# jxhe/vae-lagging-encoder

Measured on AMD Instinct MI355X. Metric: aggressive-loop seqs/sec, higher is better.
Workload: dtype bf16

## Files before the change

include/lvae.h:

```cpp
#ifndef LVAE_H
#define LVAE_H

#include <stdint.h>

#ifdef __cplusplus
extern "C" {
#endif

int lv_gemm_f32(int transA, int transB, int M, int N, int K, float alpha,
                const float* A, long lda, const float* B, long ldb, float* C, long ldc, int accumulate,
                const float* add1, long ld1, int mod1, const float* add2, long ld2, int mod2,
                float* ws , long ws_floats, void* stream);

int lv_gemm_bf16(int transA, int transB, int M, int N, int K, float alpha,
                 const float* A, long lda, const float* B, long ldb, float* C, long ldc, int accumulate,
                 const float* add1, long ld1, int mod1, const float* add2, long ld2, int mod2,
                 float* ws, long ws_floats, void* stream);

int lv_gemm_b16(int transA, int M, int N, int K, float alpha,
                const uint16_t* A, long lda, const uint16_t* B, long ldb, float* C, long ldc, int accumulate,
                const float* add1, long ld1, int mod1, const float* add2, long ld2, int mod2,
                float* ws, long ws_floats, void* stream);
int lv_gemm_b16_dual_supported(int M, int N, int K, long ws_floats);
int lv_gemm_b16_dual(int transA, int M, int N, int K, const uint16_t* A, long lda, const uint16_t* B, long ldb,
                     float* C1, long ldc1, int nsplit, float* C2, long ldc2, float* ws, long ws_floats, void* stream);
int lv_gemm_b16_pair_supported(int transA0, int M0, int N0, int K0, int transA1, int M1, int N1, int K1, long ws_floats);
int lv_gemm_b16_pair_pending(int* pending, void* stream);
int lv_gemm_b16_pair(int transA0, int M0, int N0, int K0, const uint16_t* A0, long lda0, const uint16_t* B0, long ldb0,
                     float* C0, long ldc0, int nsplit0, float* C0b, long ldc0b,
                     int transA1, int M1, int N1, int K1, const uint16_t* A1, long lda1, const uint16_t* B1, long ldb1,
                     float* C1, long ldc1, float* ws, long ws_floats, void* stream);
int lv_gemm_b16_keep(int M, int N, int K, const uint16_t* A, long lda, const uint16_t* B, long ldb, float* C,
                     const uint8_t* keep, float kscale, int Bsz, float* ws, long ws_floats, void* stream);
int lv_gemm_b16_sumsq_parts(int M, int N, int K, long ws_floats);
int lv_gemm_b16_sumsq(int transA, int M, int N, int K, const uint16_t* A, long lda, const uint16_t* B, long ldb, float* C, long ldc,
                      float* ws, long ws_floats, float* sq, int sq_only, void* stream);
int lv_gemm_b16_nll_parts(int N);
int lv_gemm_b16_tile(int tile, int transA, int M, int N, int K, float alpha,
                     const uint16_t* A, long lda, const uint16_t* B, long ldb, float* C, long ldc, int accumulate,
                     const float* add1, long ld1, int mod1, const float* add2, long ld2, int mod2,
                     float* ws, long ws_floats, void* stream);
int lv_gemm_b16_nll_tile(int tile, int M, int N, int K, const uint16_t* A, long lda, const uint16_t* B, long ldb, uint16_t* logits16,
                         long ldl16, const int64_t* ids, long ids_stride, int tgt_off, int Bsz, float* part, float* tgt_logit,
                         void* stream);
int lv_gemm_b16_nll(int M, int N, int K, const uint16_t* A, long lda, const uint16_t* B, long ldb, uint16_t* logits16, long ldl16,
                    const int64_t* ids, long ids_stride, int tgt_off, int Bsz, float* part, float* tgt_logit, void* stream);
int lv_softmax_nll_merge_f32(const float* part, int nparts, const float* tgt_logit, float* lse, float* nll, int R, void* stream);
int lv_softmax_nll_bwd_h16(const uint16_t* logits16, long ldl, const float* lse, const int64_t* ids, long ids_stride, int tgt_off,
                           const float* rowscale, uint16_t* dlogits, long ldo, int T, int B, int V, void* stream);
int lv_cvt_bf16_f32(const float* src, long lds, int R, int C, uint16_t* dst, long ldd, uint16_t* dstT, long ldt,
                    void* stream);
int lv_cvt_bf16_keep_f32(const float* src, long lds, int T, int Bsz, int C, const uint8_t* keep, float kscale,
                         uint16_t* dst, long ldd, uint16_t* dstT, long ldt, void* stream);
int lv_cvt_f32_bf16_scaled(const uint16_t* src, long n, float scale, float* dst, void* stream);
int lv_keep_scale_f32(float* x, const uint8_t* keep, float kscale, int T, int Bsz, int C, void* stream);

int lv_cvt_bf16_gates_f32(const float* src, long lds, int H, int C, uint16_t* dst, long ldd, uint16_t* dstT, long ldt,
                          void* stream);
int lv_cvt_bf16_lo_f32(const float* src, long lds, int R, int C, int gate_H, const int64_t* ids, long ids_stride, int Bsz, int V,
                       uint16_t* dst, long ldd, uint16_t* dstT, long ldt, void* stream);
int lv_cvt_h16_f32(const float* src, long lds, int R, int C, int gate_H, const int64_t* ids, long ids_stride, int Bsz, int V,
                   uint16_t* dst, long ldd, uint16_t* dstT, long ldt, void* stream);
int lv_gemm_h16(int M, int N, int K, float alpha, const uint16_t* A, long lda, const uint16_t* B, long ldb,
                float* C, long ldc, int accumulate, const float* add1, long ld1, int mod1,
                const float* add2, long ld2, int mod2, float* ws, long ws_floats, void* stream);
int lv_transpose_f32(const float* in, float* out, int rows, int cols, void* stream);
int lv_transpose_ld_f32(const float* in, long in_ld, float* out, long out_ld, int rows, int cols, void* stream);

int lv_lstm_fwd_f32(const float* gx, const float* whh, float* hs, float* cs, float* gates,
                    const uint8_t* dmask, float dscale, float* hdrop, float* ws, int T, int B, int H, void* stream);
int lv_lstm_fwd_bf16(const float* gx, const float* whh, float* hs, float* cs, float* gates,
                     const uint8_t* dmask, float dscale, float* hdrop, float* ws, int T, int B, int H, void* stream);
int lv_lstm_fwd_bf16_ug(const float* gx, const float* whh, float* hs, float* cs, float* gates,
                        const uint8_t* dmask, float dscale, float* hdrop, float* ws, int T, int B, int H, void* stream);
int lv_lstm_fwd_f32_ug(const float* gx, const float* whh, float* hs, float* cs, float* gates,
                       const uint8_t* dmask, float dscale, float* hdrop, float* ws, int T, int B, int H, void* stream);
long lv_lstm_persist16_wpk_floats(void);
long lv_lstm_persist16_xch_floats(void);
int lv_lstm_persist16_xch_clear(float* xch, void* stream);
long lv_lstm_persist16_saved_floats(int T, int R);
int lv_lstm_persist16_pack(const float* whh, float* wpk, int backward, int H, void* stream);
int lv_lstm_persist16_pack2(const float* whh, float* wpk_fwd, float* wpk_bwd, int H, void* stream);
int lv_lstm_persist16_pack2_h16(const float* whh, float* wpk_fwd, float* wpk_bwd, int H, void* stream);
int lv_lstm_fwd_bf16_persist16(const float* gx, const float* wpk, float* hs, float* cs, float* saved, float* xch, int* status,
                               int T, int B, int R, int flags, int H, void* stream);
int lv_lstm_bwd_bf16_persist16(const float* dh_ext, const float* dh_last, const float* wpk, const float* saved, const float* hs,
                               const float* cs, uint16_t* dG16, float* dGsum, float* xch, int* status, float* dh0, float* dc0,
                               int tanh_init, int T, int B, int R, int flags, int H, void* stream);
int lv_lstm_persist16_import_saved(const float* gates, const float* cs, float* saved, int T, int B, int R, int H, void* stream);
int lv_gate_interleave_f32(const float* a, const float* b, int R, int H, float* out, void* stream);
int lv_lstm_bwd_bf16(const float* dh_ext, const float* dh_last, const uint8_t* dmask, float dscale,
                     const float* whh, const float* gates, const float* hs, const float* cs,
                     float* dG, float* dGsum, float* ws, float* dh0, float* dc0, int tanh_init,
                     int T, int B, int H, void* stream);
int lv_lstm_bwd_bf16_img(const float* dh_ext, const float* dh_last, const uint8_t* dmask, float dscale,
                           const float* whh, const float* gates, const float* hs, const float* cs,
                           float* dG, uint16_t* dG16, float* dGsum, float* ws, float* dh0, float* dc0, int tanh_init,
                           int T, int B, int H, void* stream);
long lv_lstm_ws_floats(int B, int H);
int lv_lstm_bwd_ksplit(int H);
int lv_lstm_bwd_f32(const float* dh_ext, const float* dh_last, const uint8_t* dmask, float dscale,
                    const float* whh, const float* gates, const float* hs, const float* cs,
// ... 208 lines not shown
```

vae_lagging_encoder_amd/_lib.py:

```python
import ctypes
import os
import threading

from . import build as _build

_vp = ctypes.c_void_p
_i = ctypes.c_int
_l = ctypes.c_long
_f = ctypes.c_float
_d = ctypes.c_double
_u64 = ctypes.c_uint64

SIGNATURES = {
    "lv_gemm_f32": [_i, _i, _i, _i, _i, _f, _vp, _l, _vp, _l, _vp, _l, _i, _vp, _l, _i, _vp, _l, _i, _vp, _l, _vp],
    "lv_gemm_bf16": [_i, _i, _i, _i, _i, _f, _vp, _l, _vp, _l, _vp, _l, _i, _vp, _l, _i, _vp, _l, _i, _vp, _l, _vp],
    "lv_gemm_b16": [_i, _i, _i, _i, _f, _vp, _l, _vp, _l, _vp, _l, _i, _vp, _l, _i, _vp, _l, _i, _vp, _l, _vp],
    "lv_gemm_h16": [_i, _i, _i, _f, _vp, _l, _vp, _l, _vp, _l, _i, _vp, _l, _i, _vp, _l, _i, _vp, _l, _vp],
    "lv_gemm_b16_dual_supported": [_i, _i, _i, _l],
    "lv_gemm_b16_dual": [_i, _i, _i, _i, _vp, _l, _vp, _l, _vp, _l, _i, _vp, _l, _vp, _l, _vp],
    "lv_gemm_b16_pair_supported": [_i, _i, _i, _i, _i, _i, _i, _i, _l],
    "lv_gemm_b16_pair_pending": [_vp, _vp],
    "lv_gemm_b16_pair": [_i, _i, _i, _i, _vp, _l, _vp, _l, _vp, _l, _i, _vp, _l,
                         _i, _i, _i, _i, _vp, _l, _vp, _l, _vp, _l, _vp, _l, _vp],
    "lv_gemm_b16_keep": [_i, _i, _i, _vp, _l, _vp, _l, _vp, _vp, _f, _i, _vp, _l, _vp],
    "lv_gemm_b16_sumsq_parts": [_i, _i, _i, _l],
    "lv_gemm_b16_sumsq": [_i, _i, _i, _i, _vp, _l, _vp, _l, _vp, _l, _vp, _l, _vp, _i, _vp],
    "lv_gemm_b16_nll_parts": [_i],
    "lv_gemm_b16_tile": [_i, _i, _i, _i, _i, _f, _vp, _l, _vp, _l, _vp, _l, _i, _vp, _l, _i, _vp, _l, _i, _vp, _l, _vp],
    "lv_gemm_b16_nll_tile": [_i, _i, _i, _i, _vp, _l, _vp, _l, _vp, _l, _vp, _l, _i, _i, _vp, _vp, _vp],
    "lv_gemm_b16_nll": [_i, _i, _i, _vp, _l, _vp, _l, _vp, _l, _vp, _l, _i, _i, _vp, _vp, _vp],
    "lv_softmax_nll_merge_f32": [_vp, _i, _vp, _vp, _vp, _i, _vp],
    "lv_softmax_nll_bwd_h16": [_vp, _l, _vp, _vp, _l, _i, _vp, _vp, _l, _i, _i, _i, _vp],
    "lv_cvt_bf16_f32": [_vp, _l, _i, _i, _vp, _l, _vp, _l, _vp],
    "lv_cvt_bf16_keep_f32": [_vp, _l, _i, _i, _i, _vp, _f, _vp, _l, _vp, _l, _vp],
    "lv_cvt_f32_bf16_scaled": [_vp, _l, _f, _vp, _vp],
    "lv_keep_scale_f32": [_vp, _vp, _f, _i, _i, _i, _vp],
    "lv_cvt_bf16_gates_f32": [_vp, _l, _i, _i, _vp, _l, _vp, _l, _vp],
    "lv_cvt_bf16_lo_f32": [_vp, _l, _i, _i, _i, _vp, _l, _i, _i, _vp, _l, _vp, _l, _vp],
    "lv_cvt_h16_f32": [_vp, _l, _i, _i, _i, _vp, _l, _i, _i, _vp, _l, _vp, _l, _vp],
    "lv_gate_interleave_f32": [_vp, _vp, _i, _i, _vp, _vp],
    "lv_lstm_fwd_bf16_ug": [_vp, _vp, _vp, _vp, _vp, _vp, _f, _vp, _vp, _i, _i, _i, _vp],
    "lv_lstm_fwd_f32_ug": [_vp, _vp, _vp, _vp, _vp, _vp, _f, _vp, _vp, _i, _i, _i, _vp],
    "lv_loss_assemble_f32": [_vp, _vp, _vp, _vp, _vp, _vp, _vp, _vp, _vp, _i, _i, _vp],
    "lv_loss_assemble_rng_f32": [_vp, _vp, _vp, _vp, _vp, _vp, _vp, _vp, _vp, _i, _i, _vp, _u64, _vp],
    "lv_gx_expand_add_f32": [_vp, _vp, _vp, _i, _i, _i, _i, _vp],
    "lv_sample_sum_f32": [_vp, _vp, _i, _i, _i, _i, _vp],
    "lv_sample_sum_b16": [_vp, _l, _vp, _l, _i, _i, _i, _i, _vp],
    "lv_repeat_rows_i64": [_vp, _vp, _i, _i, _i, _vp],
    "lv_loss_assemble_ns_f32": [_vp, _vp, _vp, _vp, _vp, _vp, _vp, _vp, _vp, _i, _i, _i, _vp],
    "lv_loss_assemble_ns_rng_f32": [_vp, _vp, _vp, _vp, _vp, _vp, _vp, _vp, _vp, _i, _i, _i, _vp, _u64, _vp],
    "lv_enc_head_fwd_f32": [_vp, _vp, _vp, _vp, _vp, _vp, _i, _i, _i, _i, _vp],
    "lv_enc_head_bwd_f32": [_vp, _vp, _vp, _i, _vp, _vp, _vp, _vp, _vp, _vp, _i, _i, _i, _i, _vp],
    "lv_dec_tail_parts": [_i],
    "lv_dec_init_f32": [_vp, _vp, _vp, _l, _i, _vp, _vp, _vp, _vp, _vp, _i, _i, _i, _i, _vp],
    "lv_dec_tail_bwd_f32": [_vp, _vp, _vp, _vp, _l, _i, _vp, _vp, _l, _vp, _vp, _vp, _vp, _i, _i, _i, _vp],
    "lv_clip_norm2_f32": [_vp, _l, _vp, _l, _vp, _f, _vp, _vp, _vp, _vp],
    "lv_clip_norm2_txn_f32": [_vp, _l, _vp, _l, _vp, _f, _vp, _vp, _vp, _vp, _vp, _vp, _vp, _vp, _vp],
    "lv_clip_norm2_fold_txn_f32": [_vp, _l, _vp, _l, _vp, _vp, _i, _f, _vp, _vp, _vp, _vp, _vp, _vp, _vp, _vp, _vp],
    "lv_clip_coef_txn_f32": [_vp, _f, _vp, _vp, _vp, _vp, _vp, _vp, _vp, _vp],
    "lv_txn_guard_f32": [_vp, _vp, _vp, _vp],
    "lv_sgd_step_txn_f32": [_vp, _vp, _l, _vp, _vp, _i, _vp, _vp],
    "lv_scale_txn_f32": [_vp, _l, _vp, _vp, _vp],
    "lv_sgd_step_scale_txn_f32": [_vp, _vp, _l, _vp, _vp, _i, _vp, _l, _vp, _vp],
    "lv_rng_noise_step": [_vp, _l, _vp, _l, _f, _vp, _l, _f, _vp, _u64, _vp],
    "lv_lstm_persist16_wpk_floats": [],
    "lv_lstm_persist16_xch_floats": [],
    "lv_lstm_persist16_xch_clear": [_vp, _vp],
    "lv_lstm_persist16_saved_floats": [_i, _i],
    "lv_lstm_persist16_pack": [_vp, _vp, _i, _i, _vp],
    "lv_lstm_persist16_import_saved": [_vp, _vp, _vp, _i, _i, _i, _i, _vp],
    "lv_lstm_persist16_pack2": [_vp, _vp, _vp, _i, _vp],
    "lv_lstm_persist16_pack2_h16": [_vp, _vp, _vp, _i, _vp],
    "lv_lstm_fwd_bf16_persist16": [_vp, _vp, _vp, _vp, _vp, _vp, _vp, _i, _i, _i, _i, _i, _vp],
    "lv_lstm_bwd_bf16_persist16": [_vp, _vp, _vp, _vp, _vp, _vp, _vp, _vp, _vp, _vp, _vp, _vp, _i, _i, _i, _i, _i, _i, _vp],
    "lv_transpose_f32": [_vp, _vp, _i, _i, _vp],
    "lv_transpose_ld_f32": [_vp, _l, _vp, _l, _i, _i, _vp],
    "lv_lstm_bwd_ksplit": [_i],
    "lv_lstm_ws_floats": [_i, _i],
    "lv_lstm_fwd_f32": [_vp, _vp, _vp, _vp, _vp, _vp, _f, _vp, _vp, _i, _i, _i, _vp],
    "lv_lstm_bwd_f32": [_vp, _vp, _vp, _f, _vp, _vp, _vp, _vp, _vp, _vp, _vp, _vp, _vp, _i, _i, _i, _i, _vp],
    "lv_lstm_fwd_bf16": [_vp, _vp, _vp, _vp, _vp, _vp, _f, _vp, _vp, _i, _i, _i, _vp],
    "lv_lstm_bwd_bf16": [_vp, _vp, _vp, _f, _vp, _vp, _vp, _vp, _vp, _vp, _vp, _vp, _vp, _i, _i, _i, _i, _vp],
    "lv_lstm_bwd_bf16_img": [_vp, _vp, _vp, _f, _vp, _vp, _vp, _vp, _vp, _vp, _vp, _vp, _vp, _vp, _i, _i, _i, _i, _vp],
    "lv_embed_gather_f32": [_vp, _vp, _l, _vp, _f, _vp, _i, _i, _i, _i, _vp],
# ... 65 lines not shown
    "lv_mul_inplace_f32": [_vp, _vp, _l, _vp],
    "lv_bn_workspace_floats": [_i],
    "lv_pixelcnn_net_words": [],
    "lv_pixelcnn_block_words": [],
    "lv_pixelcnn_pixel_step_f32": [_vp, _i, _i, _i, _vp],
    "lv_conv32_tap_split": [_i],
    "lv_bn_eval_f32": [_vp, _vp, _vp, _vp, _vp, _f, _vp, _i, _vp, _vp, _vp, _l, _i, _vp],
    "lv_bn_fwd_f32": [_vp, _vp, _vp, _vp, _i, _vp, _vp, _vp, _vp, _vp, _f, _f, _vp, _l, _i, _vp],
    "lv_bn_bwd_f32": [_vp, _vp, _vp, _vp, _vp, _vp, _i, _vp, _vp, _vp, _vp, _i, _vp, _l, _i, _vp],
    "lv_bn_bwd2_f32": [_vp, _vp, _vp, _vp, _vp, _vp, _vp, _i, _vp, _vp, _vp, _vp, _i, _vp, _l, _i, _vp],
    "lv_bn_bwd4_f32": [_vp, _vp, _vp, _vp, _vp, _vp, _vp, _vp, _vp, _i, _vp, _vp, _vp, _vp, _i, _vp, _l, _i, _vp],
    "lv_sigmoid_bce_fwd_f32": [_vp, _vp, _vp, _i, _i, _f, _vp],
    "lv_sigmoid_bce_bwd_f32": [_vp, _vp, _vp, _vp, _i, _i, _f, _vp],
    "lv_dec_input_fwd_f32": [_vp, _vp, _vp, _i, _i, _i, _vp],
    "lv_dec_input_bwd_f32": [_vp, _vp, _i, _i, _i, _vp],
    "lv_dec_cond_ll_f32_supported": [_i, _i, _i, _i, _i],
    "lv_dec_cond_ll_f32_ws_floats": [_i, _i, _i, _i, _i],
    "lv_dec_cond_ll_f32": [_vp, _i, _i, _vp, _l, _i, _vp, _vp, _vp, _vp, _vp, _vp, _vp, _i, _i, _i, _i, _vp, _vp, _vp],
    "lv_grid_posterior_f32": [_vp, _vp, _l, _i, _i, _i, _vp, _vp, _vp],
    "lv_beam_supported": [_i, _i, _i],
    "lv_beam_ws_floats": [_i, _i, _i],
    "lv_beam_init_f32": [_vp, _vp, _vp, _vp, _vp, _vp, _vp, _vp, _vp, _vp, _i, _i, _i, _i, _i, _vp],
    "lv_beam_select_f32": [_vp, _l, _vp, _vp, _vp, _vp, _vp, _vp, _i, _i, _i, _vp],
    "lv_beam_advance_f32": [_vp, _vp, _vp, _vp, _vp, _vp, _vp, _vp, _vp, _vp, _vp, _vp, _vp, _i, _i, _i, _i, _i, _i, _i, _vp],
    "lv_beam_backtrace": [_vp, _vp, _vp, _vp, _vp, _vp, _vp, _vp, _i, _i, _i, _i, _vp],
}


_LONG_FNS = ("lv_lstm_ws_floats", "lv_conv1x1_wgrad_ws_floats", "lv_conv1x1_blocks", "lv_lstm_persist16_wpk_floats", "lv_lstm_persist16_xch_floats", "lv_lstm_persist16_saved_floats", "lv_conv32_wpack_floats",
             "lv_conv32_wgrad_ws_floats", "lv_dec_cond_ll_f32_ws_floats", "lv_beam_ws_floats")


class LvaeError(RuntimeError):
    pass


class Lib(object):

    def __init__(self, cdll, path):
        self.cdll = cdll
        self.path = path
        missing = []
        for name, argtypes in SIGNATURES.items():
            try:
                fn = getattr(cdll, name)
            except AttributeError:
                missing.append(name)
                continue
            fn.argtypes = argtypes
            fn.restype = ctypes.c_long if name in _LONG_FNS else ctypes.c_int
            setattr(self, "_raw_" + name, fn)
        if missing:
            raise LvaeError("%s does not export: %s" % (path, ", ".join(missing)))
        self._value_fns = {"lv_gemm_b16_dual_supported", "lv_gemm_b16_pair_supported", "lv_lstm_bwd_ksplit", "lv_dec_tail_parts", "lv_gemm_b16_nll_parts", "lv_gemm_b16_sumsq_parts", "lv_embed_scatter_sumsq_parts", "lv_conv32_wpack_floats",
                           "lv_conv32_wgrad_slabs", "lv_conv32_wgrad_ws_floats", "lv_conv32_wgrad_parts", "lv_conv1x1_wgrad_parts", "lv_conv32_blocks", "lv_conv1x1_blocks", "lv_conv1x1_wgrad_ws_floats", "lv_sumsq_workspace_floats", "lv_lstm_ws_floats", "lv_bn_workspace_floats",
                           "lv_lstm_persist16_wpk_floats", "lv_lstm_persist16_xch_floats", "lv_lstm_persist16_saved_floats",
                           "lv_pixelcnn_net_words", "lv_pixelcnn_block_words", "lv_conv32_tap_split", "lv_dec_cond_ll_f32_supported",
                           "lv_dec_cond_ll_f32_ws_floats", "lv_beam_supported", "lv_beam_ws_floats"}

    def __getattr__(self, name):
        if name.startswith("lv_"):
            raw = object.__getattribute__(self, "_raw_" + name)
            if name in object.__getattribute__(self, "_value_fns"):
                return raw

            def call(*args):
                rc = raw(*args)
                if rc != 0:
                    raise LvaeError("%s failed with status %d (%s)" % (
                        name, rc, "hipError_t" if rc > 0 else "argument check"))
            call.__name__ = name
            self.__dict__[name] = call
            return call
        raise AttributeError(name)


def bind(cdll, path="<cdll>"):
    return Lib(cdll, path)


_lock = threading.Lock()
_lib = None


def load():
    global _lib
    with _lock:
        if _lib is not None:
            return _lib
        path = _build.LIB_PATH
        if not os.path.exists(path):
            try:
                _build.build_hip()
            except Exception as e:
                raise LvaeError(
                    "HIP extension %s is missing and could not be built (%s). The MI355X path has no CPU "
                    "fallback: run `python -m vae_lagging_encoder_amd.build` where hipcc is available." % (path, e))
        try:
            cdll = ctypes.CDLL(path)
        except OSError as e:
            raise LvaeError("cannot load %s: %s" % (path, e))
        _lib = Lib(cdll, path)
        return _lib
```

vae_lagging_encoder_amd/csrc/lv_device.h:

```cpp
#pragma once

#ifdef LV_EMU
#include "hip_emu.h"
#define LV_LAUNCH(kern, grid, block, shmem, stream, ...) \
    lv_emu::launch((grid), (block), (shmem), [=]() { kern(__VA_ARGS__); })
#define LV_DYN_SHARED(name) char* name = lv_emu::dyn_smem()
static inline f32x4 lv_mfma_16x16x4(float a, float b, f32x4 c) { return lv_emu_mfma_16x16x4(a, b, c); }
static inline f32x16 lv_mfma_32x32x2(float a, float b, f32x16 c) { return lv_emu_mfma_32x32x2(a, b, c); }
#define LV_SCHED_BARRIER() do { } while (0)
static inline int lv_wave_uniform(int v) { return v; }
#define LV_LAUNCH_RESIDENT(kern, grid, block, shmem, stream, ...) \
    lv_emu::launch_concurrent((grid), (block), (shmem), [=]() { kern(__VA_ARGS__); })
#define LV_BLOCK_SHARED(T, name) T& name = *reinterpret_cast<T*>(lv_emu::block_shared(sizeof(T)))
static inline unsigned long long lv_agent_load_u64(const unsigned long long* p) {
    lv_emu::yield_all();
    return __atomic_load_n(p, __ATOMIC_RELAXED);
}
static inline void lv_agent_store_u64(unsigned long long* p, unsigned long long v) { __atomic_store_n(p, v, __ATOMIC_RELAXED); }
static inline void lv_xcd_store_u64(unsigned long long* p, unsigned long long v) { __atomic_store_n(p, v, __ATOMIC_RELAXED); }
static inline void lv_poll_backoff() { }
#define LV_WAIT_LDS() lv_emu::wave_sync()
template <class T> static inline void lv_store_nt(T v, T* p) { *p = v; }
static inline int lv_device_cus() { return 1 << 20; }
#define LV_SPIN_LIMIT (1 << 15)
static inline f32x16 lv_mfma_32x32x16_bf16(uint4 a, uint4 b, f32x16 c) { return lv_emu_mfma_32x32x16_bf16(a, b, c); }
static inline f32x4 lv_mfma_16x16x32_bf16(uint4 a, uint4 b, f32x4 c) { return lv_emu_mfma_16x16x32_bf16(a, b, c); }
static inline f32x4 lv_mfma_16x16x32_bf16_areg(uint4 a, uint4 b, f32x4 c) { return lv_emu_mfma_16x16x32_bf16(a, b, c); }
static inline f32x4 lv_mfma_16x16x32_bf16_areg_first(uint4 a, uint4 b) { return lv_emu_mfma_16x16x32_bf16(a, b, f32x4{0.f, 0.f, 0.f, 0.f}); }
#define LV_MFMA_DRAIN() do { } while (0)
static inline void LV_MFMA_RESULT(f32x4&) { }
static inline f32x4 lv_mfma_4x4x4_16b_bf16(uint2 a, uint2 b, f32x4 c) { return lv_emu_mfma_4x4x4_16b_bf16(a, b, c); }
static inline void lv_glds16(const void* g, void* lds_wave_base) { memcpy((char*)lds_wave_base + 16 * lv_emu::lane(), g, 16); }
static inline void lv_glds16_uncounted(const void* g, void* lds_wave_base) { lv_glds16(g, lds_wave_base); }
#define LV_WAIT_VMEM() do { } while (0)
#define LV_WAIT_VMEM_N(n) do { } while (0)
static inline void lv_store_wt_f4(float4* p, float4 v) { *p = v; }
static inline void lv_acquire_agent() { __atomic_thread_fence(__ATOMIC_ACQUIRE); }
static inline unsigned lv_agent_load_u32(const unsigned* p) { return __atomic_load_n(p, __ATOMIC_RELAXED); }
static inline void lv_sleep_short() { }
#define LV_ARRIVAL_POLLS 2
static inline unsigned atomicExch(unsigned* p, unsigned v) { return __atomic_exchange_n(p, v, __ATOMIC_RELAXED); }
#define LV_S_BARRIER() __syncthreads()
#define LV_SETPRIO(n) do { } while (0)
static inline uint2 lv_ds_read_tr16_b64(const void* lds_ptr) {
    auto& w = lv_emu::my_wave();
    const int l = lv_emu::lane();
    uint64_t blk;
    memcpy(&blk, lds_ptr, 8);
    w.u[l] = blk;
    lv_emu::wave_sync();
    uint16_t o[4];
    for (int j = 0; j < 4; ++j) {
        const uint64_t b = w.u[(l & ~15) + 4 * j + ((l & 15) >> 2)];
        o[j] = (uint16_t)(b >> (16 * (l & 3)));
    }
    lv_emu::wave_sync();
    uint2 r;
    memcpy(&r, o, 8);
    return r;
}
template <int SHIFT, int BANK> static inline float lv_row_shr_into(float old, float src) {
    auto& w = lv_emu::my_wave();
    const int l = lv_emu::lane();
    uint32_t b;
    memcpy(&b, &src, 4);
    w.u[l] = b;
    lv_emu::wave_sync();
    float out = old;
    if (((l & 15) >> 2) == BANK && (l & 15) >= SHIFT) { const uint32_t v = (uint32_t)w.u[l - SHIFT]; memcpy(&out, &v, 4); }
    lv_emu::wave_sync();
    return out;
}
static inline float lv_sat_f16(float x) { return x != x ? x : fminf(fmaxf(x, -65504.f), 65504.f); }
static inline uint16_t lv_f32_to_f16_bits(float x) {
    uint32_t u;
    memcpy(&u, &x, 4);
    const uint32_t sign = (u >> 16) & 0x8000u;
    u &= 0x7FFFFFFFu;
    if (u >= 0x7F800000u) return (uint16_t)(sign | (u > 0x7F800000u ? 0x7E00u : 0x7C00u));
    if (u >= 0x477FF000u) return (uint16_t)(sign | 0x7C00u);
    if (u < 0x33000001u) return (uint16_t)sign;
    if (u < 0x38800000u) {
        const int shift = 126 - (int)(u >> 23);
        const uint32_t mant = (u & 0x7FFFFFu) | 0x800000u;
        uint32_t h = mant >> shift;
        const uint32_t rem = mant & ((1u << shift) - 1u), half = 1u << (shift - 1);
        if (rem > half || (rem == half && (h & 1u))) ++h;
        return (uint16_t)(sign | h);
    }
    uint32_t h = ((u - 0x38000000u) >> 13);
    const uint32_t rem = u & 0x1FFFu;
    if (rem > 0x1000u || (rem == 0x1000u && (h & 1u))) ++h;
    return (uint16_t)(sign | h);
}
// ... 439 lines not shown
```

vae_lagging_encoder_amd/csrc/lv_gemm_b16.hip:

```cpp
#ifndef LV_B16_T256_DMA
#define LV_B16_T256_DMA 1
#endif
#if defined(LV_TRACE)
#define lv_trace_buf lv_trace_buf_gemm
#endif
#include "lv_device.h"
#if defined(LV_TRACE) && !defined(LV_EMU)
__device__ unsigned long long* lv_trace_buf = nullptr;
extern "C" int lv_trace_set_gemm(void* p) { return (int)hipMemcpyToSymbol(HIP_SYMBOL(lv_trace_buf), &p, sizeof(p)); }
#endif
#include <type_traits>

namespace {

#ifndef LV_B16_ABL
#define LV_B16_ABL 0
#endif
#ifndef LV_B16_SPLIT_TARGET
#define LV_B16_SPLIT_TARGET 512
#endif

constexpr int BK = 64;
constexpr int BT = 128;
constexpr int NCH = BK / 8;

#ifndef LV_NLL_ABL
#define LV_NLL_ABL 0
#endif
struct GemmQ {
    const uint16_t* A; const uint16_t* B; float* C;
    int M, N, K;
    long lda, ldb, ldc;
    float alpha;
    int accumulate;
    const float* add1; long ld1; int mod1;
    const float* add2; long ld2; int mod2;
    int tilesM, tilesN;
    int splits, kt_per_split;
    float* ws;
    uint16_t* C16; long ldc16;
    const int64_t* ids; long ids_stride; int tgt_off; int Bsz;
    float2* part; int nparts;
    float* tgt;
    const uint8_t* keep; float kscale; int keepT;
    float* sq; int sq_only;
    float* C2; long ldc2; int nsplit;
};

__device__ __forceinline__ uint4 load_chunk(const uint16_t* __restrict__ p, int valid) {
    if (valid >= 8) return *reinterpret_cast<const uint4*>(p);
    uint32_t h[8];
#pragma unroll
    for (int e = 0; e < 8; ++e) h[e] = e < valid ? (uint32_t)p[e] : 0u;
    uint4 q;
    q.x = h[0] | (h[1] << 16); q.y = h[2] | (h[3] << 16); q.z = h[4] | (h[5] << 16); q.w = h[6] | (h[7] << 16);
    return q;
}


struct KcPtr { const uint16_t* p[4]; };

__device__ __forceinline__ KcPtr kc_setup(const uint16_t* __restrict__ P, long ld, int rows, int r0, int t) {
    KcPtr q;
#pragma unroll
    for (int i = 0; i < 4; ++i) {
        const int f = t + 256 * i;
        int row = r0 + (f >> 3);
        if (row > rows - 1) row = rows - 1;
        q.p[i] = P + (long)row * ld + 8 * (f & 7);
    }
    return q;
}

template <bool FULL>
__device__ __forceinline__ void kc_load(const KcPtr& q, int k0, int K, int t, uint4 (&reg)[4]) {
#pragma unroll
    for (int i = 0; i < 4; ++i) {
        if (FULL) {
            reg[i] = *reinterpret_cast<const uint4*>(q.p[i] + k0);
        } else {
            const int k = k0 + 8 * ((t + 256 * i) & 7);
            reg[i] = k < K ? load_chunk(q.p[i] + k0, K - k) : make_uint4(0u, 0u, 0u, 0u);
        }
    }
}

__device__ __forceinline__ void store_kc(uint4 (*S)[BT], int t, const uint4 (&reg)[4]) {
#pragma unroll
    for (int i = 0; i < 4; ++i) {
        const int f = t + 256 * i;
        const int m = f >> 3, c = f & 7;
        S[c][m ^ (2 * c)] = reg[i];
    }
}

struct McPtr { const uint16_t* p; long ld; };

__device__ __forceinline__ McPtr mc_setup(const uint16_t* __restrict__ P, long ld, int r0, int t) {
    long col = r0 + 8 * (t & 15);
// ... 525 lines not shown
    for (int i = 0; i < 2; ++i)
#pragma unroll
        for (int j = 0; j < 2; ++j)
            store_frag_f32(p, acc[i][j], m0 + wm * 64 + i * 32 + 4 * (l >> 5), n0 + wn * 64 + j * 32 + (l & 31));
}

constexpr int BT2 = 256;
typedef uint4 LdsTile2[BT2][NCH];

struct Tail256 {
    int full;
    int tail;
    int tail_s;
    int kt_per_piece;
};

#ifndef LV_T256_G
#define LV_T256_G 4
#endif
__device__ __forceinline__ void t256_tile_of(const GemmQ& p, int s, int& tm, int& tn) {
    const int G = LV_T256_G;
    const int nig = G * p.tilesN;
    const int group = s / nig;
    const int first_m = group * G;
    const int gsz = (p.tilesM - first_m) < G ? (p.tilesM - first_m) : G;
    tm = first_m + (s % nig) % gsz;
    tn = (s % nig) / gsz;
}

struct T256Pick { int tile, kt0, kt1, piece, tm, tn; };
__device__ __forceinline__ T256Pick t256_pick(const GemmQ& p, const Tail256& q, int bid) {
    T256Pick k;
    const int nk_all = (p.K + BK - 1) / BK;
    k.piece = -1;
    if (bid < q.full) {
        const int xcd = bid % 8, per = q.full / 8;
        k.tile = xcd * per + bid / 8;
        k.kt0 = 0; k.kt1 = nk_all;
    } else {
        const int r = bid - q.full, nw = q.tail * q.tail_s;
        const int xcd = r % 8, qq = nw / 8, rem = nw % 8;
        const int idx = (xcd < rem ? xcd * (qq + 1) : rem * (qq + 1) + (xcd - rem) * qq) + r / 8;
        k.tile = q.full + idx % q.tail;
        k.piece = idx / q.tail;
        k.kt0 = k.piece * q.kt_per_piece;
        k.kt1 = k.kt0 + q.kt_per_piece;
        if (k.kt1 > nk_all) k.kt1 = nk_all;
        if (q.tail_s == 1) k.piece = -1;
    }
    t256_tile_of(p, k.tile, k.tm, k.tn);
    return k;
}

template <bool NLL>
__device__ __forceinline__ void t256_epilogue(const GemmQ& p, const Tail256& q, f32x16 (&acc)[4][2], LdsTile2& As0, LdsTile2& Bs0,
                                              LdsTile2& As1, LdsTile2& Bs1, int tile, int piece, int tn, int m0, int n0, int t, int l,
                                              int wm, int wn, int lh) {
    constexpr int NJ = 2;
    if constexpr (NLL) {
#if LV_NLL_ABL & 4
        return;
#endif
        auto rowptr = [&](int rr) -> char* {
            const int b = rr >> 6;
            char* base = b == 0 ? reinterpret_cast<char*>(&As0[0][0]) : b == 1 ? reinterpret_cast<char*>(&Bs0[0][0])
                       : b == 2 ? reinterpret_cast<char*>(&As1[0][0]) : reinterpret_cast<char*>(&Bs1[0][0]);
            return base + (rr & 63) * 512;
        };
        const int odd = l & 1;
#pragma unroll
        for (int i2 = 0; i2 < 4; ++i2) {
            char* const bufp = rowptr(wm * 128 + i2 * 32);
#pragma unroll
            for (int j = 0; j < 2; ++j) {
                const int clp = (wn * 64 + j * 32 + (l & 31)) & ~1;
                const int lane_off = (4 * lh + odd) * 512 + ((((clp >> 3) ^ (4 * lh) ^ odd) << 4) | ((clp & 7) << 1));
#pragma unroll
                for (int e = 0; e < 16; e += 2) {
                    const float mine0 = acc[i2][j][e], mine1 = acc[i2][j][e + 1];
                    const float got = lv_lane_xor1(odd ? mine0 : mine1);
                    const uint32_t pk = odd ? lv_pack_f16x2(got, mine1) : lv_pack_f16x2(mine0, got);
                    const int key = (e & 3) | (8 * ((e >> 2) & 1));
                    const int roff = ((e & 3) + 8 * (e >> 2)) * 512;
                    *reinterpret_cast<uint32_t*>(bufp + roff + (lane_off ^ (key << 4))) = pk;
                }
            }
        }
        __syncthreads();
#if !(LV_NLL_ABL & 1)
        {
            const int c = l & 31;
#pragma unroll 4
            for (int s16 = 0; s16 < 16; ++s16) {
                const int r2 = 16 * s16 + 2 * (t >> 6) + (l >> 5);
                const uint4 qv = *reinterpret_cast<const uint4*>(rowptr(r2) + ((c ^ (r2 & 15)) << 4));
                const int col0 = n0 + 8 * c;
                if (m0 + r2 < p.M && col0 + 8 <= p.ldc16) *reinterpret_cast<uint4*>(p.C16 + (long)(m0 + r2) * p.ldc16 + col0) = qv;
            }
        }
#endif
        const int rr = t & 255, half = t >> 8;
        const int row = m0 + rr;
        if (row < p.M) {
            const char* rowp = rowptr(rr);
            const int tt = row / p.Bsz, bb = row % p.Bsz;
            long tg = p.ids[(long)bb * p.ids_stride + tt + p.tgt_off];
            if (tg < 0) tg = 0;
            if (tg >= p.N) tg = p.N - 1;
#pragma unroll 1
            for (int pc = 0; pc < 2; ++pc) {
                const int cb = 128 * half + 64 * pc;
                const int c0 = n0 + cb;
                uint4 qv[8];
#pragma unroll
                for (int k = 0; k < 8; ++k) qv[k] = *reinterpret_cast<const uint4*>(rowp + ((((cb >> 3) + k) ^ (rr & 15)) << 4));
#if LV_NLL_ABL & 2
                if (qv[0].x == 0x12345678u) p.tgt[row] = 1.f;
                continue;
#endif
                float v[64];
#pragma unroll
                for (int k = 0; k < 8; ++k) {
                    const uint32_t wv[4] = {qv[k].x, qv[k].y, qv[k].z, qv[k].w};
#pragma unroll
                    for (int h2 = 0; h2 < 4; ++h2) {
                        v[8 * k + 2 * h2] = lv_f16_bits_to_f32((uint16_t)(wv[h2] & 0xFFFFu));
                        v[8 * k + 2 * h2 + 1] = lv_f16_bits_to_f32((uint16_t)(wv[h2] >> 16));
                    }
                }
                float mx, sm;
                nll_piece_stats(v, p.N - c0, mx, sm);
                p.part[(long)row * p.nparts + 4 * tn + 2 * half + pc] = make_float2(mx, sm);
                const int tl = (int)tg - c0;
                if (tl >= 0 && tl < 64) {
                    const int cl = cb + tl;
                    p.tgt[row] = lv_f16_bits_to_f32(*reinterpret_cast<const uint16_t*>(rowp + ((((cl >> 3) ^ (rr & 15)) << 4) | ((cl & 7) << 1))));
                }
            }
        }
        return;
    }
    if (piece >= 0) {
        if (p.sq && piece == 0 && l == 0) p.sq[tile * 8 + (t >> 6)] = 0.f;
        float* slab = p.ws + ((long)(tile - q.full) * q.tail_s + piece) * (BT2 * BT2);
#pragma unroll
        for (int i2 = 0; i2 < 4; ++i2)
#pragma unroll
            for (int j = 0; j < NJ; ++j) {
                const int col = wn * (32 * NJ) + j * 32 + (l & 31);
#pragma unroll
                for (int e = 0; e < 16; ++e) {
                    const int rr = wm * 128 + i2 * 32 + (e & 3) + 8 * (e >> 2) + 4 * (l >> 5);
                    slab[rr * BT2 + col] = acc[i2][j][e];
                }
            }
        return;
    }
    if (p.sq) {
        float ss = 0.f;
#pragma unroll
        for (int i2 = 0; i2 < 4; ++i2)
#pragma unroll
            for (int j = 0; j < NJ; ++j) {
                const int rbase = m0 + wm * 128 + i2 * 32 + 4 * (l >> 5), col = n0 + wn * (32 * NJ) + j * 32 + (l & 31);
#pragma unroll
                for (int e = 0; e < 16; ++e) {
                    const float v = p.alpha * acc[i2][j][e];
                    if (col < p.N && rbase + (e & 3) + 8 * (e >> 2) < p.M) ss += v * v;
                }
            }
        ss = lv_wave_sum(ss);
        if (l == 0) p.sq[tile * 8 + (t >> 6)] = ss;
        if (p.sq_only) return;
    }
#pragma unroll
    for (int i2 = 0; i2 < 4; ++i2)
#pragma unroll
        for (int j = 0; j < NJ; ++j)
            store_frag_f32(p, acc[i2][j], m0 + wm * 128 + i2 * 32 + 4 * (l >> 5), n0 + wn * (32 * NJ) + j * 32 + (l & 31));
}

template <bool NLL, bool TN, bool PP = false>
__global__ __launch_bounds__(512) void lv_gemm_b16_t256_kernel(GemmQ p, Tail256 q) {
    constexpr int WN = 4;
    constexpr int NJ = 2;
    constexpr int UN = 4;
    __shared__ __attribute__((aligned(1024))) LdsTile2 As0, Bs0;
    __shared__ __attribute__((aligned(1024))) LdsTile2 As1, Bs1;

    const int t = (int)threadIdx.x;
    const int l = t & 63, w = lv_wave_uniform(t >> 6);
    const int wm = w / WN, wn = w % WN;
    const int li = l & 31, lh = l >> 5;
    const int nfull = p.K / BK;

    const T256Pick pk = t256_pick(p, q, (int)blockIdx.x);
    const int kt0 = pk.kt0, kt1 = pk.kt1;
    const int m0 = pk.tm * BT2, n0 = pk.tn * BT2;

    f32x16 acc[4][NJ];
#pragma unroll
    for (int i = 0; i < 4; ++i)
#pragma unroll
        for (int j = 0; j < NJ; ++j)
#pragma unroll
            for (int e = 0; e < 16; ++e) acc[i][j][e] = 0.f;

    uint32_t oa[UN], ob[UN];
    int kch[UN];
#pragma unroll
    for (int i = 0; i < UN; ++i) {
        const int u = UN * w + i;
        const int row = 8 * u + (l >> 3);
#if LV_B16_PP_ABL & 128
        const int c = (l & 7);
#else
        const int c = (l & 7) ^ ((row >> 1) & 7);
#endif
        kch[i] = 8 * c;
#if LV_B16_PP_ABL & 64
        int ra = row, rb = row;
#else
        int ra = m0 + row, rb = n0 + row;
#endif
        if (ra > p.M - 1) ra = p.M - 1;
        if (rb > p.N - 1) rb = p.N - 1;
        oa[i] = (uint32_t)((long)ra * p.lda + kch[i]);
        ob[i] = (uint32_t)((long)rb * p.ldb + kch[i]);
        if constexpr (TN) {
            const int krow = 2 * u + (l >> 5);
            long mc = m0 / 8 + ((l & 31) ^ (4 * (krow & 3)));
            if (mc > p.lda / 8 - 1) mc = p.lda / 8 - 1;
            oa[i] = (uint32_t)((long)krow * p.lda + 8 * mc);
        }
    }
// ... 344 lines not shown
        mfma_close(true);
#pragma unroll
        for (int ks = 0; ks < 4; ++ks) { fa[ks][0] = a_frag(Ac, ks, 2); fa[ks][1] = a_frag(Ac, ks, 3); }
        LV_SCHED_BARRIER();
        stage_half(kn2, 2, Ac, Bc);
        seg_close(false);
        mma_quadrant(fa, fb1, 1, 1);
        mfma_close(false);
        stage_half(kn2, 3, Ac, Bc);
        seg_close(true);
        mma_quadrant(fa, fb0, 1, 0);
        mfma_close(true);
    };

    const int nmain = (kt1 < nfull ? kt1 : nfull) - kt0;
    if (kt1 > kt0 + nmain) {
        stage_ragged(kt1 - 1, As0, Bs0);
        __syncthreads();
#pragma unroll
        for (int ks = 0; ks < 4; ++ks) {
            uint4 ra[4], rb[2];
#pragma unroll
            for (int i2 = 0; i2 < 4; ++i2) ra[i2] = a_frag(As0, ks, i2);
#pragma unroll
            for (int j = 0; j < 2; ++j) rb[j] = b_frag(Bs0, ks, j);
#pragma unroll
            for (int i2 = 0; i2 < 4; ++i2)
#pragma unroll
                for (int j = 0; j < 2; ++j) acc[i2][j] = lv_mfma_32x32x16_bf16(ra[i2], rb[j], acc[i2][j]);
        }
        __syncthreads();
    }
    if (nmain > 0) {
        const int klast = kt0 + nmain - 1;
        auto tile_at = [&](int i) { return kt0 + i < klast ? kt0 + i : klast; };
        stage_half(tile_at(0), 0, As0, Bs0); stage_half(tile_at(0), 2, As0, Bs0); stage_half(tile_at(0), 3, As0, Bs0);
        stage_half(tile_at(0), 1, As0, Bs0);
        stage_half(tile_at(1), 0, As1, Bs1); stage_half(tile_at(1), 2, As1, Bs1); stage_half(tile_at(1), 3, As1, Bs1);
        LV_Q_WAIT();
        __syncthreads();
        if (wm == 1) LV_S_BARRIER();
        for (int i = 0; i < nmain; i += 2) {
            q_tile(As0, Bs0, As1, Bs1, tile_at(i + 1), tile_at(i + 2));
            if (i + 1 >= nmain) break;
            q_tile(As1, Bs1, As0, Bs0, tile_at(i + 2), tile_at(i + 3));
        }
        if (wm == 0) LV_S_BARRIER();
        LV_WAIT_VMEM();
        __syncthreads();
    }
#undef LV_Q_WAIT
}

template <bool NLL, bool TN>
__global__ __launch_bounds__(512) void lv_gemm_b16_t256q_kernel(GemmQ p, Tail256 q) {
    __shared__ __attribute__((aligned(1024))) LdsTile2 As0, Bs0;
    __shared__ __attribute__((aligned(1024))) LdsTile2 As1, Bs1;

    const T256Pick pk = t256_pick(p, q, (int)blockIdx.x);
    const int m0 = pk.tm * BT2, n0 = pk.tn * BT2;
    const int t = (int)threadIdx.x;
    const int l = t & 63, w = lv_wave_uniform(t >> 6);

    f32x16 acc[4][2];
    t256q_run<TN>(p, m0, n0, pk.kt0, pk.kt1, acc, As0, Bs0, As1, Bs1, l, w);
    t256_epilogue<NLL>(p, q, acc, As0, Bs0, As1, Bs1, pk.tile, pk.piece, pk.tn, m0, n0, t, l, w >> 2, w & 3, l >> 5);
}

#ifndef LV_SK_ABL
#define LV_SK_ABL 0
#endif
#ifndef LV_SK_SPIN
#define LV_SK_SPIN LV_ARRIVAL_POLLS
#endif
#ifndef LV_SK_SKEW
#define LV_SK_SKEW 3
#endif
#ifndef LV_SK_ROWS0
#define LV_SK_ROWS0 0
#endif
constexpr int SK_SLOTS = 32;
constexpr int SK_TILES = 1024;
__device__ unsigned lv_sk_arrivals[SK_SLOTS * SK_TILES];

struct SkProb {
    GemmQ q;
    int rows;
    int nk;
    long units;
    float* slabs;
    int cnt0;
    int skew, pieces, plen;
};
struct GemmG { SkProb pr[2]; };

__device__ __forceinline__ long sk_start(const SkProb& P, int nwg, int s) {
    const long b = (long)s * P.units / nwg;
    return (P.skew > 0 && s % P.pieces != 0) ? b - P.skew : b;
}
__device__ __forceinline__ int sk_owner(const SkProb& P, int nwg, long u) {
    if (P.skew > 0) {
        const int tile = (int)(u / P.nk), k = (int)(u - (long)tile * P.nk);
        int j = k / P.plen;
        if (j + 1 < P.pieces && k >= (j + 1) * P.plen - P.skew) ++j;
        return tile * P.pieces + j;
    }
    return (int)(((u + 1) * nwg - 1) / P.units);
// ... 115 lines not shown
                    sk_add_slab(acc, reinterpret_cast<const float4*>(P.slabs + (2L * c + (tile != (int)(cu0 / P.nk))) * (BT2 * BT2)) + t);
                }
            }
            done = summed;
        }
#if LV_SK_ABL & 2
        if (done && acc[0][0][0] == 1.2345e-30f) sk_store_tile(P.q, acc, m0, n0, l, w);
#else
        if (done) sk_store_tile(P.q, acc, m0, n0, l, w);
#endif
    }
}

__global__ __launch_bounds__(256) void sk_pending_kernel(int* out) {
    int n = 0;
    for (int i = (int)threadIdx.x; i < SK_SLOTS * SK_TILES; i += 256) n += lv_sk_arrivals[i] != 0u;
    n = lv_wave_sum(n);
    __shared__ int part[4];
    if ((threadIdx.x & 63) == 0) part[threadIdx.x >> 6] = n;
    __syncthreads();
    if (threadIdx.x == 0) *out = part[0] + part[1] + part[2] + part[3];
}

template <bool TN0, bool TN1>
__global__ __launch_bounds__(512) void lv_gemm_b16_t256g_kernel(GemmG g) {
    __shared__ __attribute__((aligned(1024))) LdsTile2 As0, Bs0;
    __shared__ __attribute__((aligned(1024))) LdsTile2 As1, Bs1;
    const int t = (int)threadIdx.x;
    const int l = t & 63, w = lv_wave_uniform(t >> 6);
    const int bid = (int)blockIdx.x, xcd = bid % 8, row = bid / 8;
    if (row < g.pr[0].rows) sk_work<TN0>(g.pr[0], xcd * g.pr[0].rows + row, As0, Bs0, As1, Bs1, t, l, w);
    else sk_work<TN1>(g.pr[1], xcd * g.pr[1].rows + (row - g.pr[0].rows), As0, Bs0, As1, Bs1, t, l, w);
}

#ifndef LV_TR_ROWS
#define LV_TR_ROWS 8
#endif
constexpr int TR_ROWS = LV_TR_ROWS, TR_WGS = BT2 / TR_ROWS;
__global__ __launch_bounds__(256) void tail_reduce_t256_kernel(GemmQ p, Tail256 q) {
    const int tile = q.full + (int)blockIdx.x / TR_WGS;
    int tm, tn;
    t256_tile_of(p, tile, tm, tn);
    const float* slab = p.ws + (long)(tile - q.full) * q.tail_s * (BT2 * BT2);
    const int t = (int)threadIdx.x;
    const int c4 = (t & 63) * 4;
    float ss = 0.f;
    const bool fast = !p.add1 && !p.add2 && !p.accumulate && p.ldc % 4 == 0 && p.N % 4 == 0 && (((uintptr_t)p.C) & 15) == 0 &&
                      (((uintptr_t)p.keep) & 3) == 0;
#pragma unroll
    for (int it = 0; it < TR_ROWS / 4; ++it) {
        const int rr = ((int)blockIdx.x % TR_WGS) * TR_ROWS + 4 * it + (t >> 6);
        const int row = tm * BT2 + rr;
        if (row >= p.M) continue;
        float4 sacc = make_float4(0.f, 0.f, 0.f, 0.f);
        for (int k0 = 0; k0 < q.tail_s; k0 += 4) {
            float4 pv[4];
#pragma unroll
            for (int u = 0; u < 4; ++u)
                pv[u] = *reinterpret_cast<const float4*>(slab + (long)(k0 + u < q.tail_s ? k0 + u : k0) * (BT2 * BT2) + rr * BT2 + c4);
#pragma unroll
            for (int u = 0; u < 4; ++u)
                if (k0 + u < q.tail_s) { sacc.x += pv[u].x; sacc.y += pv[u].y; sacc.z += pv[u].z; sacc.w += pv[u].w; }
        }
        const float sv[4] = {sacc.x, sacc.y, sacc.z, sacc.w};
        if (fast && tn * BT2 + c4 + 3 < p.N) {
            const int col = tn * BT2 + c4;
            float4 o = make_float4(p.alpha * sv[0], p.alpha * sv[1], p.alpha * sv[2], p.alpha * sv[3]);
            if (p.keep) {
                const uint32_t mk = *reinterpret_cast<const uint32_t*>(p.keep + ((long)(row % p.Bsz) * p.keepT + row / p.Bsz) * p.N + col);
                o.x = (mk & 0xFFu) ? o.x * p.kscale : 0.f;
                o.y = (mk & 0xFF00u) ? o.y * p.kscale : 0.f;
                o.z = (mk & 0xFF0000u) ? o.z * p.kscale : 0.f;
                o.w = (mk & 0xFF000000u) ? o.w * p.kscale : 0.f;
            }
            ss += (o.x * o.x + o.y * o.y) + (o.z * o.z + o.w * o.w);
            if (!p.sq_only) *reinterpret_cast<float4*>(p.C + (long)row * p.ldc + col) = o;
            continue;
        }
#pragma unroll
        for (int e = 0; e < 4; ++e) {
            const int col = tn * BT2 + c4 + e;
            if (col >= p.N) continue;
            float v = p.alpha * sv[e];
            if (p.add1) v += p.add1[(long)(row % p.mod1) * p.ld1 + col];
            if (p.add2) v += p.add2[(long)(row % p.mod2) * p.ld2 + col];
            float* c = p.C + (long)row * p.ldc + col;
            if (p.accumulate) v += *c;
            if (p.keep) v *= p.keep[((long)(row % p.Bsz) * p.keepT + row / p.Bsz) * p.N + col] ? p.kscale : 0.f;
            ss += v * v;
            if (!p.sq_only) *c = v;
        }
    }
    if (p.sq) {
        ss = lv_wave_sum(ss);
        if ((t & 63) == 0) p.sq[(long)p.tilesM * p.tilesN * 8 + (long)blockIdx.x * 4 + (t >> 6)] = ss;
    }
}

template <int NF>
__device__ __forceinline__ float sum_pieces(const float* first, long stride, int n) {
    float s = 0.f;
    for (int k0 = 0; k0 < n; k0 += NF) {
        float pv[NF];
#pragma unroll
        for (int u = 0; u < NF; ++u) pv[u] = first[(long)(k0 + u < n ? k0 + u : 0) * stride];
#pragma unroll
        for (int u = 0; u < NF; ++u)
            if (k0 + u < n) s += pv[u];
    }
    return s;
}

__global__ __launch_bounds__(256) void splitk_reduce_b16_v4_kernel(GemmQ p) {
    const long idx = ((long)blockIdx.x * 256 + threadIdx.x) * 4;
    const long MN = (long)p.M * p.N;
    if (idx >= MN) return;
    const int row = (int)(idx / p.N), col = (int)(idx % p.N);
    float4 s = make_float4(0.f, 0.f, 0.f, 0.f);
    for (int k0 = 0; k0 < p.splits; k0 += 4) {
        float4 pv[4];
#pragma unroll
        for (int u = 0; u < 4; ++u) pv[u] = *reinterpret_cast<const float4*>(p.ws + (long)(k0 + u < p.splits ? k0 + u : k0) * MN + idx);
#pragma unroll
        for (int u = 0; u < 4; ++u)
            if (k0 + u < p.splits) { s.x += pv[u].x; s.y += pv[u].y; s.z += pv[u].z; s.w += pv[u].w; }
    }
    float4 o = make_float4(p.alpha * s.x, p.alpha * s.y, p.alpha * s.z, p.alpha * s.w);
    if (p.keep) {
        const uint32_t mk = *reinterpret_cast<const uint32_t*>(p.keep + ((long)(row % p.Bsz) * p.keepT + row / p.Bsz) * p.N + col);
        o.x = (mk & 0xFFu) ? o.x * p.kscale : 0.f;
        o.y = (mk & 0xFF00u) ? o.y * p.kscale : 0.f;
        o.z = (mk & 0xFF0000u) ? o.z * p.kscale : 0.f;
        o.w = (mk & 0xFF000000u) ? o.w * p.kscale : 0.f;
    }
    if (p.nsplit > 0 && col >= p.nsplit) *reinterpret_cast<float4*>(p.C2 + (long)row * p.ldc2 + (col - p.nsplit)) = o;
    else *reinterpret_cast<float4*>(p.C + (long)row * p.ldc + col) = o;
}

__global__ __launch_bounds__(256) void splitk_reduce_b16_kernel(GemmQ p) {
    const long idx = (long)blockIdx.x * 256 + threadIdx.x;
    const long MN = (long)p.M * p.N;
    if (idx >= MN) return;
    const int row = (int)(idx / p.N), col = (int)(idx % p.N);
    float s = 0.f;
    if (p.splits <= 2) s = sum_pieces<2>(p.ws + idx, MN, p.splits);
    else if (p.splits <= 4) s = sum_pieces<4>(p.ws + idx, MN, p.splits);
    else s = sum_pieces<8>(p.ws + idx, MN, p.splits);
    float v = p.alpha * s;
    if (p.add1) v += p.add1[(long)(row % p.mod1) * p.ld1 + col];
    if (p.add2) v += p.add2[(long)(row % p.mod2) * p.ld2 + col];
    float* c = (p.nsplit > 0 && col >= p.nsplit) ? p.C2 + (long)row * p.ldc2 + (col - p.nsplit) : p.C + (long)row * p.ldc + col;
    if (p.accumulate) v += *c;
    if (p.keep) v *= p.keep[((long)(row % p.Bsz) * p.keepT + row / p.Bsz) * p.N + col] ? p.kscale : 0.f;
    *c = v;
}

__global__ __launch_bounds__(256) void cvt_b16_kernel(const float* __restrict__ src, long lds_, int R, int C,
                                                      uint16_t* __restrict__ dst, long ldd, uint16_t* __restrict__ dstT, long ldt,
                                                      int gate_H, const uint8_t* __restrict__ keep, float kscale, int Bsz,
                                                      const int64_t* __restrict__ gids, long gstride, int gV, int lo) {
    __shared__ uint16_t tile[64][66];
    const int t = (int)threadIdx.x;
    const int r0 = (int)blockIdx.y * 64, c0 = (int)blockIdx.x * 64;
    const int lane = t & 63, q = t >> 6;
    const bool tb = keep || gids;
    const int Tt = tb ? R / Bsz : 1;
    int bb = tb ? (r0 + q) % Bsz : 0, tt = tb ? (r0 + q) / Bsz : 0;
    const int gc = c0 + lane, gcc = gc < C ? gc : C - 1;
#pragma unroll
    for (int i0 = 0; i0 < 16; i0 += 8) {
        int grs[8], bbs[8], tts[8];
        long sr[8];
#pragma unroll
        for (int u = 0; u < 8; ++u) {
            grs[u] = r0 + q + 4 * (i0 + u);
            bbs[u] = bb; tts[u] = tt;
            if (tb) {
                bb += 4;
                while (bb >= Bsz) { bb -= Bsz; ++tt; }
            }
            sr[u] = grs[u] < R ? grs[u] : R - 1;
        }
        if (gids) {
#pragma unroll
            for (int u = 0; u < 8; ++u) sr[u] = gids[(long)bbs[u] * gstride + (grs[u] < R ? tts[u] : 0)];
#pragma unroll
            for (int u = 0; u < 8; ++u) sr[u] = sr[u] < 0 ? 0 : (sr[u] >= gV ? gV - 1 : sr[u]);
        }
        float v[8];
        uint8_t kp[8];
#pragma unroll
        for (int u = 0; u < 8; ++u) v[u] = src[sr[u] * lds_ + gcc];
        if (keep) {
#pragma unroll
            for (int u = 0; u < 8; ++u) kp[u] = keep[((long)bbs[u] * Tt + (grs[u] < R ? tts[u] : 0)) * C + gcc];
        }
#pragma unroll
        for (int u = 0; u < 8; ++u) {
            const int gr = grs[u];
            uint16_t b = 0;
            if (gr < R && gc < C) {
                float x = v[u];
                if (keep) {
                    if (gids) x = kp[u] ? x * kscale : 0.f;
                    else x *= kp[u] ? kscale : 0.f;
                }
                b = (uint16_t)lv_f32_to_bf16_bits(x);
                if (lo == 1) b = (uint16_t)lv_f32_to_bf16_bits(x - lv_bf16_bits_to_f32(b));
                if (dst) {
                    const long dr = gate_H > 0 ? (long)(gr % gate_H) * 4 + gr / gate_H : gr;
                    dst[dr * ldd + gc] = lo == 2 ? lv_f32_to_f16_bits(lv_sat_f16(x)) : b;
                }
            }
            tile[q + 4 * (i0 + u)][lane] = b;
        }
    }
    if (!dstT) return;
    __syncthreads();
#pragma unroll 4
    for (int i = 0; i < 16; ++i) {
        const int c = q + 4 * i;
        const int gc = c0 + c, gr = r0 + lane;
        if (gc < C && gr < R) dstT[(long)gc * ldt + gr] = tile[lane][c];
    }
}


__global__ __launch_bounds__(256) void cvt_b16_v4_kernel(const float* __restrict__ src, long lds_, int R, int C,
                                                         uint16_t* __restrict__ dst, long ldd, uint16_t* __restrict__ dstT, long ldt,
                                                         int gate_H, const uint8_t* __restrict__ keep, float kscale, int Bsz,
                                                         const int64_t* __restrict__ gids, long gstride, int gV, int lo) {
    __shared__ __attribute__((aligned(8))) uint16_t tile[64][68];
    const int t = (int)threadIdx.x;
    const int r0 = (int)blockIdx.y * 64, c0 = (int)blockIdx.x * 64;
    const int q = t >> 4, cl = t & 15;
    const bool tb = keep || gids;
    const int Tt = tb ? R / Bsz : 1;
    int bb = tb ? (r0 + q) % Bsz : 0, tt = tb ? (r0 + q) / Bsz : 0;
    const int gc = c0 + 4 * cl;
    const int gcc = gc < C ? gc : C - 4;
    int grs[4], bbs[4], tts[4];
    long sr[4];
#pragma unroll
    for (int u = 0; u < 4; ++u) {
        grs[u] = r0 + q + 16 * u;
        bbs[u] = bb; tts[u] = tt;
        if (tb) {
            bb += 16;
            while (bb >= Bsz) { bb -= Bsz; ++tt; }
        }
        sr[u] = grs[u] < R ? grs[u] : R - 1;
    }
    if (gids) {
#pragma unroll
        for (int u = 0; u < 4; ++u) sr[u] = gids[(long)bbs[u] * gstride + (grs[u] < R ? tts[u] : 0)];
#pragma unroll
        for (int u = 0; u < 4; ++u) sr[u] = sr[u] < 0 ? 0 : (sr[u] >= gV ? gV - 1 : sr[u]);
    }
    float4 v[4];
    uint32_t kp[4] = {0u, 0u, 0u, 0u};
#pragma unroll
    for (int u = 0; u < 4; ++u) v[u] = *reinterpret_cast<const float4*>(src + sr[u] * lds_ + gcc);
    if (keep) {
#pragma unroll
        for (int u = 0; u < 4; ++u)
            kp[u] = *reinterpret_cast<const uint32_t*>(keep + ((long)bbs[u] * Tt + (grs[u] < R ? tts[u] : 0)) * C + gcc);
    }
#pragma unroll
    for (int u = 0; u < 4; ++u) {
        const int gr = grs[u];
        uint16_t b[4] = {0, 0, 0, 0}, d[4] = {0, 0, 0, 0};
        const bool in = gr < R && gc < C;
        if (in) {
            const float xs[4] = {v[u].x, v[u].y, v[u].z, v[u].w};
#pragma unroll
            for (int e = 0; e < 4; ++e) {
                float x = xs[e];
                if (keep) {
                    const bool k = (kp[u] >> (8 * e)) & 0xFFu;
                    if (gids) x = k ? x * kscale : 0.f;
                    else x *= k ? kscale : 0.f;
                }
                b[e] = (uint16_t)lv_f32_to_bf16_bits(x);
                if (lo == 1) b[e] = (uint16_t)lv_f32_to_bf16_bits(x - lv_bf16_bits_to_f32(b[e]));
                d[e] = lo == 2 ? lv_f32_to_f16_bits(lv_sat_f16(x)) : b[e];
            }
            if (dst) {
                const long dr = gate_H > 0 ? (long)(gr % gate_H) * 4 + gr / gate_H : gr;
                *reinterpret_cast<uint2*>(dst + dr * ldd + gc) = make_uint2((uint32_t)d[0] | ((uint32_t)d[1] << 16), (uint32_t)d[2] | ((uint32_t)d[3] << 16));
            }
        }
        *reinterpret_cast<uint2*>(&tile[q + 16 * u][4 * cl]) = make_uint2((uint32_t)b[0] | ((uint32_t)b[1] << 16), (uint32_t)b[2] | ((uint32_t)b[3] << 16));
    }
    if (!dstT) return;
    __syncthreads();
    const int rl = t & 15, gr = r0 + 4 * rl;
#pragma unroll
    for (int i = 0; i < 4; ++i) {
        const int c = q + 16 * i, gct = c0 + c;
        const uint16_t e0 = tile[4 * rl][c], e1 = tile[4 * rl + 1][c], e2 = tile[4 * rl + 2][c], e3 = tile[4 * rl + 3][c];
        if (gct < C) {
            uint16_t* o = dstT + (long)gct * ldt + gr;
            if (gr + 3 < R) *reinterpret_cast<uint2*>(o) = make_uint2((uint32_t)e0 | ((uint32_t)e1 << 16), (uint32_t)e2 | ((uint32_t)e3 << 16));
            else {
                if (gr < R) o[0] = e0;
                if (gr + 1 < R) o[1] = e1;
                if (gr + 2 < R) o[2] = e2;
            }
        }
    }
}

static void cvt_launch(void* stream, const float* src, long lds, int R, int C, uint16_t* dst, long ldd, uint16_t* dstT, long ldt, int gate_H,
                       const uint8_t* keep, float kscale, int Bsz, const int64_t* gids, long gstride, int gV, int lo) {
    const dim3 grid((unsigned)lv_cdiv(C, 64), (unsigned)lv_cdiv(R, 64)), block(256);
    const bool v4 = C >= 4 && C % 4 == 0 && lds % 4 == 0 && (((uintptr_t)src) & 15) == 0 &&
                    (!dst || (ldd % 4 == 0 && (((uintptr_t)dst) & 7) == 0)) && (!dstT || (ldt % 4 == 0 && (((uintptr_t)dstT) & 7) == 0)) &&
                    (!keep || (((uintptr_t)keep) & 3) == 0);
    if (v4) LV_LAUNCH(cvt_b16_v4_kernel, grid, block, 0, stream, src, lds, R, C, dst, ldd, dstT, ldt, gate_H, keep, kscale, Bsz, gids, gstride, gV, lo);
    else LV_LAUNCH(cvt_b16_kernel, grid, block, 0, stream, src, lds, R, C, dst, ldd, dstT, ldt, gate_H, keep, kscale, Bsz, gids, gstride, gV, lo);
}

}

static bool t256_wanted(int tile, int M, int N, int K) {
    if (tile) return tile >= 256;
    return 2.0 * M * N * K >= 1.0e11 && M >= 1024 && N >= 1024 && K >= 1024;
}
#ifndef LV_B16_SCHED_DEFAULT
#define LV_B16_SCHED_DEFAULT -1
#endif
static int t256_sched(int tile, int kt_per_wg) {
    if (tile >= 256) return tile - 256;
    return LV_B16_SCHED_DEFAULT >= 0 ? LV_B16_SCHED_DEFAULT : (kt_per_wg >= 24 ? 2 : 1);
}

static Tail256 t256_plan(long tiles, int nk, long ws_floats) {
    Tail256 q;
    q.full = (int)(tiles / 256 * 256);
    q.tail_s = 1;
    q.kt_per_piece = nk;
    const long tail = tiles - q.full;
    q.tail = (int)tail;
    if (tail == 0) return q;
    double best = (double)nk * 2.0;
    for (int s = 2; s <= 16; ++s) {
        if (nk / s < 4 || tail * s * (long)(BT2 * BT2) > ws_floats) break;
        const double cost = (double)lv_cdiv(tail * s, 256) * lv_cdiv(nk, s) * 2.0 + (s + 1) * tail * 0.058;
        if (cost < best) { best = cost; q.tail_s = s; }
    }
    q.kt_per_piece = lv_cdiv(nk, q.tail_s);
    q.tail_s = lv_cdiv(nk, q.kt_per_piece);
    return q;
}

extern "C" int lv_keep_scale_f32(float* x, const uint8_t* keep, float kscale, int T, int Bsz, int C, void* stream);

static int gemm_b16_launch(int tile, int transA, int M, int N, int K, float alpha,
                           const uint16_t* A, long lda, const uint16_t* B, long ldb,
                           float* C, long ldc, int accumulate,
                           const float* add1, long ld1, int mod1,
                           const float* add2, long ld2, int mod2,
                           float* ws, long ws_floats, void* stream, const uint8_t* keep, float kscale, int Bsz,
                           float* sq = nullptr, int sq_only = 0, int f16 = 0, float* C2 = nullptr, long ldc2 = 0, int nsplit = 0) {
    if (tile != 0 && tile != 128 && (tile < 256 || tile > 258)) return LV_ERR_ARG;
    if (f16) {
        if (transA || keep || sq || !LV_B16_GLDS) return LV_ERR_UNSUPPORTED;
        tile = 128;
    }
    if (M < 0 || N < 0 || K < 0) return LV_ERR_SHAPE;
    if (M == 0 || N == 0) return LV_OK;
    if (!A || !B || !C) return LV_ERR_ARG;
    if ((add1 && mod1 <= 0) || (add2 && mod2 <= 0)) return LV_ERR_ARG;
    if (lda < (transA ? M : K) || ldb < K || ldc < (C2 && nsplit > 0 ? nsplit : N)) return LV_ERR_SHAPE;
    if (ldb % 8 != 0 || (((uintptr_t)B) & 15) != 0) return LV_ERR_ALIGN;
    if (lda % 8 != 0 || (((uintptr_t)A) & 15) != 0) return LV_ERR_ALIGN;
    GemmQ p{};
    p.A = A; p.B = B; p.C = C; p.M = M; p.N = N; p.K = K;
    p.lda = lda; p.ldb = ldb; p.ldc = ldc; p.alpha = alpha; p.accumulate = accumulate;
    p.add1 = add1; p.ld1 = ld1; p.mod1 = mod1 > 0 ? mod1 : 1;
    p.add2 = add2; p.ld2 = ld2; p.mod2 = mod2 > 0 ? mod2 : 1;
    p.ws = ws;
    p.keep = nullptr; p.kscale = 1.f; p.keepT = 1; p.Bsz = Bsz > 0 ? Bsz : 1;
    p.sq = sq; p.sq_only = sq ? sq_only : 0;
    p.C2 = C2; p.ldc2 = ldc2; p.nsplit = C2 ? nsplit : 0;
    if (p.nsplit > 0) {
        if (p.nsplit >= N || ldc < p.nsplit || ldc2 < N - p.nsplit || add1 || add2 || accumulate || keep || sq || f16) return LV_ERR_ARG;
        if (t256_wanted(tile, M, N, K) || !ws) return LV_ERR_UNSUPPORTED;
    }
    if (sq && (!t256_wanted(tile, M, N, K) || accumulate || add1 || add2 || keep)) return LV_ERR_ARG;
    bool keep_pending = keep != nullptr;
    const int nk = lv_cdiv(K > 0 ? K : 1, BK);
    if (t256_wanted(tile, M, N, K)) {
        p.tilesM = lv_cdiv(M, BT2); p.tilesN = lv_cdiv(N, BT2);
        p.splits = 1; p.kt_per_split = nk;
        const Tail256 q = t256_plan((long)p.tilesM * p.tilesN, nk, ws ? ws_floats : 0);
        const long tail = (long)p.tilesM * p.tilesN - q.full;
        if (keep && q.full == 0 && q.tail_s > 1) { p.keep = keep; p.kscale = kscale; p.keepT = M / p.Bsz; keep_pending = false; }
        dim3 grid((unsigned)(q.full + tail * q.tail_s)), block(512);
        const int sched = t256_sched(tile, q.tail_s > 1 && q.full == 0 ? q.kt_per_piece : nk);
        if (sched == 2) {
            if (transA) LV_LAUNCH((lv_gemm_b16_t256q_kernel<false, true>), grid, block, 0, stream, p, q);
            else LV_LAUNCH((lv_gemm_b16_t256q_kernel<false, false>), grid, block, 0, stream, p, q);
        } else if (sched == 1) {
            if (transA) LV_LAUNCH((lv_gemm_b16_t256_kernel<false, true, true>), grid, block, 0, stream, p, q);
            else LV_LAUNCH((lv_gemm_b16_t256_kernel<false, false, true>), grid, block, 0, stream, p, q);
        } else if (transA) LV_LAUNCH((lv_gemm_b16_t256_kernel<false, true>), grid, block, 0, stream, p, q);
        else LV_LAUNCH((lv_gemm_b16_t256_kernel<false, false>), grid, block, 0, stream, p, q);
        if (q.tail_s > 1) LV_LAUNCH(tail_reduce_t256_kernel, dim3((unsigned)(tail * TR_WGS)), dim3(256), 0, stream, p, q);
        LV_CHECK_LAUNCH();
        if (keep_pending) return lv_keep_scale_f32(C, keep, kscale, M / p.Bsz, p.Bsz, N, stream);
        return LV_OK;
    }
    p.tilesM = lv_cdiv(M, BT); p.tilesN = lv_cdiv(N, BT);
    const long tiles = (long)p.tilesM * p.tilesN;
    int splits = 1;
    if (ws && tiles < 512 && nk >= 8) {
        long sp = lv_cdiv(LV_B16_SPLIT_TARGET, tiles);
        if (sp > nk / 4) sp = nk / 4;
        if (sp > 64) sp = 64;
        const long cap = ws_floats / ((long)M * N);
        if (sp > cap) sp = cap;
        if (sp > 1) splits = (int)sp;
    }
    if (p.nsplit > 0 && splits < 2) {
        if (nk < 2 || ws_floats < 2L * M * N) return LV_ERR_UNSUPPORTED;
        splits = 2;
    }
    if (p.nsplit > 0) {
        while (lv_cdiv(nk, splits) > 32 && splits < 64 && ws_floats >= (long)(splits + 1) * M * N) ++splits;
    }
    p.kt_per_split = lv_cdiv(nk, splits);
    splits = lv_cdiv(nk, p.kt_per_split);
    p.splits = splits;
    if (keep && splits > 1) { p.keep = keep; p.kscale = kscale; p.keepT = M / p.Bsz; keep_pending = false; }
    dim3 grid((unsigned)tiles, (unsigned)splits), block(256);
    if (transA && LV_B16_GLDS == 1 && p.kt_per_split > 32) LV_LAUNCH((lv_gemm_b16_nt_glds_kernel<false, false, true>), grid, block, 0, stream, p);
    else if (transA && LV_B16_GLDS) LV_LAUNCH((lv_gemm_b16_nt_glds_kernel<true, false, true>), grid, block, 0, stream, p);
    else if (transA) LV_LAUNCH((lv_gemm_b16_kernel<false>), grid, block, 0, stream, p);
    else if (f16 && p.kt_per_split > 32) LV_LAUNCH((lv_gemm_b16_nt_glds_kernel<false, false, false, true>), grid, block, 0, stream, p);
    else if (f16) LV_LAUNCH((lv_gemm_b16_nt_glds_kernel<true, false, false, true>), grid, block, 0, stream, p);
    else if (LV_B16_GLDS == 1 && p.kt_per_split > 32) LV_LAUNCH(lv_gemm_b16_nt_glds_kernel<false>, grid, block, 0, stream, p);
    else if (LV_B16_GLDS) LV_LAUNCH(lv_gemm_b16_nt_glds_kernel<true>, grid, block, 0, stream, p);
    else LV_LAUNCH((lv_gemm_b16_kernel<true>), grid, block, 0, stream, p);
    if (splits > 1) {
        const bool v4 = !add1 && !add2 && !accumulate && N % 4 == 0 && ldc % 4 == 0 && (((uintptr_t)C | (uintptr_t)ws) & 15) == 0 &&
                        (((uintptr_t)p.keep) & 3) == 0 &&
                        (p.nsplit == 0 || (p.nsplit % 4 == 0 && ldc2 % 4 == 0 && (((uintptr_t)C2) & 15) == 0));
        if (v4) LV_LAUNCH(splitk_reduce_b16_v4_kernel, dim3((unsigned)lv_cdiv((long)M * N / 4, 256)), dim3(256), 0, stream, p);
        else LV_LAUNCH(splitk_reduce_b16_kernel, dim3((unsigned)lv_cdiv((long)M * N, 256)), dim3(256), 0, stream, p);
    }
    LV_CHECK_LAUNCH();
    if (keep_pending) return lv_keep_scale_f32(C, keep, kscale, M / p.Bsz, p.Bsz, N, stream);
    return LV_OK;
}

static int sk_rows0(long U0, int nk0, long U1) {
    if (U1 <= 0) return 32;
    int best = 0;
    double bestc = 0.;
    for (int r0 = 1; r0 < 32; ++r0) {
        const long n0 = 8L * r0, n1 = 8L * (32 - r0);
        const long L0 = lv_cdiv(U0, n0), L1 = lv_cdiv(U1, n1);
        double c = (double)(L0 > L1 ? L0 : L1);
        if (U0 % n0 != 0 || nk0 % L0 != 0) c *= 1.1;
        if (!best || c < bestc) { best = r0; bestc = c; }
    }
    return best;
}
static bool sk_fits32(int transA, int M, int N, int K, long lda, long ldb) {
    const long ea = (long)(transA ? K : M) * lda + 64, eb = (long)N * ldb + 64;
    return ea < (1L << 32) && eb < (1L << 32) && (transA ? K : M) < (1 << 30);
}
static long sk_ws_floats() { return 2L * 256 * BT2 * BT2; }

static bool sk_possible(int transA1, int M0, int N0, int K0, int M1, int N1, int K1, long ws_floats) {
    if (!LV_B16_GLDS) return false;
    if (M0 <= 0 || N0 <= 0 || K0 <= 0 || M1 < 0 || N1 < 0 || K1 < 0) return false;
    const bool two = M1 > 0 && N1 > 0 && K1 > 0;
    if (transA1 != 0 && two) return false;
    const long t0 = (long)lv_cdiv(M0, BT2) * lv_cdiv(N0, BT2), t1 = two ? (long)lv_cdiv(M1, BT2) * lv_cdiv(N1, BT2) : 0;
    return t0 + t1 <= SK_TILES && ws_floats >= sk_ws_floats();
}
extern "C" int lv_gemm_b16_pair_supported(int transA0, int M0, int N0, int K0, int transA1, int M1, int N1, int K1, long ws_floats) {
    (void)transA0;
    if (!sk_possible(transA1, M0, N0, K0, M1, N1, K1, ws_floats) || M1 <= 0 || N1 <= 0 || K1 <= 0) return 0;
    const long U = (long)lv_cdiv(M0, BT2) * lv_cdiv(N0, BT2) * lv_cdiv(K0, BK) + (long)lv_cdiv(M1, BT2) * lv_cdiv(N1, BT2) * lv_cdiv(K1, BK);
    return U >= 256L * 12;
}

extern "C" int lv_gemm_b16_pair(int transA0, int M0, int N0, int K0, const uint16_t* A0, long lda0, const uint16_t* B0, long ldb0,
                                float* C0, long ldc0, int nsplit0, float* C0b, long ldc0b,
                                int transA1, int M1, int N1, int K1, const uint16_t* A1, long lda1, const uint16_t* B1, long ldb1,
                                float* C1, long ldc1, float* ws, long ws_floats, void* stream) {
    if (!sk_possible(transA1, M0, N0, K0, M1, N1, K1, ws_floats)) return LV_ERR_UNSUPPORTED;
    const bool two = M1 > 0 && N1 > 0 && K1 > 0;
    if (!A0 || !B0 || !C0 || !ws || (two && (!A1 || !B1 || !C1))) return LV_ERR_ARG;
    if (nsplit0 < 0 || (nsplit0 > 0 && (!C0b || nsplit0 >= N0 || ldc0b < N0 - nsplit0))) return LV_ERR_ARG;
    if (lda0 < (transA0 ? M0 : K0) || ldb0 < K0 || ldc0 < (nsplit0 > 0 ? nsplit0 : N0)) return LV_ERR_SHAPE;
    if (two && (lda1 < K1 || ldb1 < K1 || ldc1 < N1)) return LV_ERR_SHAPE;
    if (lda0 % 8 != 0 || ldb0 % 8 != 0 || ((((uintptr_t)A0) | ((uintptr_t)B0)) & 15) != 0) return LV_ERR_ALIGN;
    if (two && (lda1 % 8 != 0 || ldb1 % 8 != 0 || ((((uintptr_t)A1) | ((uintptr_t)B1)) & 15) != 0)) return LV_ERR_ALIGN;
    if ((((uintptr_t)ws) & 15) != 0) return LV_ERR_ALIGN;
    if (!sk_fits32(transA0, M0, N0, K0, lda0, ldb0) || (two && !sk_fits32(0, M1, N1, K1, lda1, ldb1))) return LV_ERR_UNSUPPORTED;
    static unsigned next_slot = 0;
// ... 14 lines not shown
    for (int j = 0; j < 2; ++j) {
        SkProb& P = g.pr[j];
        const long n = 8L * P.rows;
        if (LV_SK_SKEW <= 0 || n == 0 || P.units % n != 0) continue;
        const long L = P.units / n;
        if (L < 8 || P.nk % L != 0 || P.nk / L < 2) continue;
        P.pieces = (int)(P.nk / L); P.plen = (int)L;
        P.skew = LV_SK_SKEW < L / 8 ? LV_SK_SKEW : (int)(L / 8);
    }
    g.pr[0].slabs = ws;
    g.pr[1].slabs = ws + 2L * 8 * g.pr[0].rows * (BT2 * BT2);
    g.pr[0].cnt0 = (int)(slot * SK_TILES);
    g.pr[1].cnt0 = g.pr[0].cnt0 + g.pr[0].q.tilesM * g.pr[0].q.tilesN;
    if (transA0) LV_LAUNCH((lv_gemm_b16_t256g_kernel<true, false>), dim3(256), dim3(512), 0, stream, g);
    else LV_LAUNCH((lv_gemm_b16_t256g_kernel<false, false>), dim3(256), dim3(512), 0, stream, g);
    LV_CHECK_LAUNCH();
    return LV_OK;
}

extern "C" int lv_gemm_b16_pair_pending(int* pending, void* stream) {
    if (!pending) return LV_ERR_ARG;
    LV_LAUNCH(sk_pending_kernel, dim3(1), dim3(256), 0, stream, pending);
    LV_CHECK_LAUNCH();
    return LV_OK;
}

extern "C" int lv_gemm_b16_tile(int tile, int transA, int M, int N, int K, float alpha,
                                const uint16_t* A, long lda, const uint16_t* B, long ldb,
                                float* C, long ldc, int accumulate,
                                const float* add1, long ld1, int mod1,
                                const float* add2, long ld2, int mod2,
                                float* ws, long ws_floats, void* stream) {
    return gemm_b16_launch(tile, transA, M, N, K, alpha, A, lda, B, ldb, C, ldc, accumulate, add1, ld1, mod1, add2, ld2, mod2, ws, ws_floats,
                           stream, nullptr, 1.f, 1);
}

extern "C" int lv_gemm_b16_dual_supported(int M, int N, int K, long ws_floats) {
    if (M <= 0 || N <= 0 || K <= 0 || t256_wanted(0, M, N, K)) return 0;
    return lv_cdiv(K, BK) >= 2 && ws_floats >= 2L * M * N;
}
extern "C" int lv_gemm_b16_dual(int transA, int M, int N, int K, const uint16_t* A, long lda, const uint16_t* B, long ldb,
                                float* C1, long ldc1, int nsplit, float* C2, long ldc2, float* ws, long ws_floats, void* stream) {
    if (!C2 || nsplit <= 0) return LV_ERR_ARG;
    return gemm_b16_launch(0, transA, M, N, K, 1.f, A, lda, B, ldb, C1, ldc1, 0, nullptr, 0, 1, nullptr, 0, 1, ws, ws_floats, stream,
                           nullptr, 1.f, 1, nullptr, 0, 0, C2, ldc2, nsplit);
}

extern "C" int lv_gemm_b16_keep(int M, int N, int K, const uint16_t* A, long lda, const uint16_t* B, long ldb, float* C,
                                const uint8_t* keep, float kscale, int Bsz, float* ws, long ws_floats, void* stream) {
    if (!keep || Bsz <= 0 || M % Bsz != 0) return LV_ERR_ARG;
    return gemm_b16_launch(0, 0, M, N, K, 1.f, A, lda, B, ldb, C, N, 0, nullptr, 0, 1, nullptr, 0, 1, ws, ws_floats, stream, keep, kscale, Bsz);
}

extern "C" int lv_gemm_b16_sumsq_parts(int M, int N, int K, long ws_floats) {
    if (M <= 0 || N <= 0 || K <= 0 || !t256_wanted(0, M, N, K)) return 0;
    const long tiles = (long)lv_cdiv(M, BT2) * lv_cdiv(N, BT2);
    const Tail256 q = t256_plan(tiles, lv_cdiv(K, BK), ws_floats);
    return (int)(tiles * 8 + (q.tail_s > 1 ? (long)q.tail * TR_WGS * 4 : 0));
}

extern "C" int lv_gemm_b16_sumsq(int transA, int M, int N, int K, const uint16_t* A, long lda, const uint16_t* B, long ldb,
                                 float* C, long ldc, float* ws, long ws_floats, float* sq, int sq_only, void* stream) {
    if (!sq || (!ws && ws_floats > 0)) return LV_ERR_ARG;
    return gemm_b16_launch(0, transA, M, N, K, 1.f, A, lda, B, ldb, C, ldc, 0, nullptr, 0, 1, nullptr, 0, 1, ws, ws_floats, stream,
                           nullptr, 1.f, 1, sq, sq_only);
}

extern "C" int lv_gemm_b16(int transA, int M, int N, int K, float alpha,
                           const uint16_t* A, long lda, const uint16_t* B, long ldb,
                           float* C, long ldc, int accumulate,
                           const float* add1, long ld1, int mod1,
                           const float* add2, long ld2, int mod2,
                           float* ws, long ws_floats, void* stream) {
    return lv_gemm_b16_tile(0, transA, M, N, K, alpha, A, lda, B, ldb, C, ldc, accumulate, add1, ld1, mod1, add2, ld2, mod2, ws,
                            ws_floats, stream);
}

extern "C" int lv_gemm_h16(int M, int N, int K, float alpha, const uint16_t* A, long lda, const uint16_t* B, long ldb,
                           float* C, long ldc, int accumulate, const float* add1, long ld1, int mod1,
                           const float* add2, long ld2, int mod2, float* ws, long ws_floats, void* stream) {
    return gemm_b16_launch(128, 0, M, N, K, alpha, A, lda, B, ldb, C, ldc, accumulate, add1, ld1, mod1, add2, ld2, mod2, ws, ws_floats,
                           stream, nullptr, 1.f, 1, nullptr, 0, 1);
}

extern "C" int lv_cvt_bf16_f32(const float* src, long lds, int R, int C, uint16_t* dst, long ldd, uint16_t* dstT, long ldt,
                               void* stream) {
    if (!src || (!dst && !dstT)) return LV_ERR_ARG;
    if (R < 0 || C < 0 || lds < C || (dst && ldd < C) || (dstT && ldt < R)) return LV_ERR_SHAPE;
    if (R == 0 || C == 0) return LV_OK;
    cvt_launch(stream, src, lds, R, C,
              dst, ldd, dstT, ldt, 0, (const uint8_t*)nullptr, 1.f, 1, (const int64_t*)nullptr, 0L, 0, 0);
    LV_CHECK_LAUNCH();
    return LV_OK;
}

extern "C" int lv_cvt_bf16_keep_f32(const float* src, long lds, int T, int Bsz, int C, const uint8_t* keep, float kscale,
                                    uint16_t* dst, long ldd, uint16_t* dstT, long ldt, void* stream) {
    if (!src || !keep || (!dst && !dstT)) return LV_ERR_ARG;
    const long R = (long)T * Bsz;
    if (T < 0 || Bsz <= 0 || C < 0 || lds < C || (dst && ldd < C) || (dstT && ldt < R)) return LV_ERR_SHAPE;
    if (R == 0 || C == 0) return LV_OK;
    cvt_launch(stream, src, lds, (int)R, C,
              dst, ldd, dstT, ldt, 0, keep, kscale, Bsz, (const int64_t*)nullptr, 0L, 0, 0);
    LV_CHECK_LAUNCH();
    return LV_OK;
}

extern "C" int lv_embed_gather_b16(const float* emb, const int64_t* ids, long ids_stride, const uint8_t* keep, float kscale,
                                   int T, int Bsz, int C, int V, uint16_t* dst, long ldd, uint16_t* dstT, long ldt, void* stream) {
    if (!emb || !ids || (!dst && !dstT)) return LV_ERR_ARG;
    const long R = (long)T * Bsz;
    if (T < 0 || Bsz <= 0 || C < 0 || V <= 0 || (dst && ldd < C) || (dstT && ldt < R)) return LV_ERR_SHAPE;
    if (R == 0 || C == 0) return LV_OK;
    cvt_launch(stream, emb, (long)C, (int)R, C,
              dst, ldd, dstT, ldt, 0, keep, kscale, Bsz, ids, ids_stride, V, 0);
    LV_CHECK_LAUNCH();
    return LV_OK;
}

extern "C" int lv_cvt_bf16_gates_f32(const float* src, long lds, int H, int C, uint16_t* dst, long ldd, uint16_t* dstT, long ldt,
                                     void* stream) {
    if (!src || (!dst && !dstT)) return LV_ERR_ARG;
    if (H <= 0 || C < 0 || lds < C || (dst && ldd < C) || (dstT && ldt < 4 * H)) return LV_ERR_SHAPE;
    if (C == 0) return LV_OK;
    cvt_launch(stream, src, lds, 4 * H, C,
              dst, ldd, dstT, ldt, H, (const uint8_t*)nullptr, 1.f, 1, (const int64_t*)nullptr, 0L, 0, 0);
    LV_CHECK_LAUNCH();
    return LV_OK;
}


extern "C" int lv_cvt_bf16_lo_f32(const float* src, long lds, int R, int C, int gate_H, const int64_t* ids, long ids_stride, int Bsz,
                                  int V, uint16_t* dst, long ldd, uint16_t* dstT, long ldt, void* stream) {
    if (!src || (!dst && !dstT)) return LV_ERR_ARG;
    if (R < 0 || C < 0 || lds < C || (dst && ldd < C) || (dstT && ldt < R)) return LV_ERR_SHAPE;
    if (gate_H > 0 && (R != 4 * gate_H || ids)) return LV_ERR_ARG;
    if (ids && (Bsz <= 0 || V <= 0 || R % Bsz != 0)) return LV_ERR_SHAPE;
    if (R == 0 || C == 0) return LV_OK;
    cvt_launch(stream, src, lds, R, C,
              dst, ldd, dstT, ldt, gate_H > 0 ? gate_H : 0, (const uint8_t*)nullptr, 1.f, ids ? Bsz : 1, ids, ids_stride, ids ? V : 0, 1);
    LV_CHECK_LAUNCH();
    return LV_OK;
}

extern "C" int lv_cvt_h16_f32(const float* src, long lds, int R, int C, int gate_H, const int64_t* ids, long ids_stride, int Bsz,
                              int V, uint16_t* dst, long ldd, uint16_t* dstT, long ldt, void* stream) {
    if (!src || (!dst && !dstT)) return LV_ERR_ARG;
    if (R < 0 || C < 0 || lds < C || (dst && ldd < C) || (dstT && ldt < R)) return LV_ERR_SHAPE;
    if (gate_H > 0 && (R != 4 * gate_H || ids)) return LV_ERR_ARG;
    if (ids && (Bsz <= 0 || V <= 0 || R % Bsz != 0)) return LV_ERR_SHAPE;
    if (R == 0 || C == 0) return LV_OK;
    cvt_launch(stream, src, lds, R, C,
              dst, ldd, dstT, ldt, gate_H > 0 ? gate_H : 0, (const uint8_t*)nullptr, 1.f, ids ? Bsz : 1, ids, ids_stride, ids ? V : 0, 2);
    LV_CHECK_LAUNCH();
    return LV_OK;
}

extern "C" int lv_gemm_b16_nll_parts(int N) { return 4 * lv_cdiv(N, BT2); }

extern "C" int lv_gemm_b16_nll_tile(int tile, int M, int N, int K, const uint16_t* A, long lda, const uint16_t* B, long ldb,
                                    uint16_t* logits16, long ldl16, const int64_t* ids, long ids_stride, int tgt_off, int Bsz,
                                    float* part, float* tgt_logit, void* stream) {
    if (tile != 0 && tile != 128 && (tile < 256 || tile > 258)) return LV_ERR_ARG;
    if (M < 0 || N <= 0 || K <= 0 || Bsz <= 0) return LV_ERR_SHAPE;
    if (M == 0) return LV_OK;
    if (!A || !B || !logits16 || !ids || !part || !tgt_logit) return LV_ERR_ARG;
    if (lda < K || ldb < K || ldl16 < N) return LV_ERR_SHAPE;
    if (lda % 8 != 0 || ldb % 8 != 0 || ldl16 % 8 != 0 || (((uintptr_t)A) & 15) != 0 || (((uintptr_t)B) & 15) != 0 ||
        (((uintptr_t)logits16) & 15) != 0 || (((uintptr_t)part) & 7) != 0)
        return LV_ERR_ALIGN;
    GemmQ p{};
    p.A = A; p.B = B; p.C = nullptr; p.M = M; p.N = N; p.K = K;
    p.lda = lda; p.ldb = ldb; p.ldc = 0; p.alpha = 1.f; p.accumulate = 0;
    p.add1 = nullptr; p.add2 = nullptr; p.mod1 = p.mod2 = 1; p.ws = nullptr;
    p.splits = 1; p.kt_per_split = lv_cdiv(K, BK);
    p.C16 = logits16; p.ldc16 = ldl16; p.ids = ids; p.ids_stride = ids_stride; p.tgt_off = tgt_off; p.Bsz = Bsz;
    p.part = reinterpret_cast<float2*>(part); p.nparts = lv_gemm_b16_nll_parts(N); p.tgt = tgt_logit;
    if (t256_wanted(tile, M, N, K)) {
        p.tilesM = lv_cdiv(M, BT2); p.tilesN = lv_cdiv(N, BT2);
        Tail256 q;
        const long tiles = (long)p.tilesM * p.tilesN;
        q.full = (int)(tiles / 256 * 256); q.tail = (int)(tiles - q.full); q.tail_s = 1; q.kt_per_piece = p.kt_per_split;
        const int sched = t256_sched(tile, p.kt_per_split);
        if (sched == 2) LV_LAUNCH((lv_gemm_b16_t256q_kernel<true, false>), dim3((unsigned)tiles), dim3(512), 0, stream, p, q);
        else if (sched == 1) LV_LAUNCH((lv_gemm_b16_t256_kernel<true, false, true>), dim3((unsigned)tiles), dim3(512), 0, stream, p, q);
        else LV_LAUNCH((lv_gemm_b16_t256_kernel<true, false>), dim3((unsigned)tiles), dim3(512), 0, stream, p, q);
        LV_CHECK_LAUNCH();
        return LV_OK;
    }
    p.tilesM = lv_cdiv(M, BT); p.tilesN = lv_cdiv(N, BT);
    dim3 grid((unsigned)((long)p.tilesM * p.tilesN), 1), block(256);
    LV_LAUNCH((lv_gemm_b16_nt_glds_kernel<true, true>), grid, block, 0, stream, p);
    LV_CHECK_LAUNCH();
    return LV_OK;
}

extern "C" int lv_gemm_b16_nll(int M, int N, int K, const uint16_t* A, long lda, const uint16_t* B, long ldb,
                               uint16_t* logits16, long ldl16, const int64_t* ids, long ids_stride, int tgt_off, int Bsz,
                               float* part, float* tgt_logit, void* stream) {
    return lv_gemm_b16_nll_tile(0, M, N, K, A, lda, B, ldb, logits16, ldl16, ids, ids_stride, tgt_off, Bsz, part, tgt_logit, stream);
}
```

vae_lagging_encoder_amd/csrc/lv_loss.hip:

```cpp
#include "lv_device.h"

namespace {

template <int G>
__global__ __launch_bounds__(256) void reparam_kl_fwd_kernel(const float* __restrict__ mulv, const float* __restrict__ eps,
                                                             float* __restrict__ z, float* __restrict__ kl,
                                                             int B, int ns, int nz) {
    const int tid = (int)threadIdx.x;
    const int row = ((int)blockIdx.x * 256 + tid) / G;
    const int j0 = tid % G;
    const bool ok = row < B;
    const float* mu = mulv + (long)(ok ? row : 0) * 2 * nz;
    const float* lv = mu + nz;
    float part = 0.f;
    for (int j = j0; j < nz; j += G) {
        if (!ok) break;
        const float m = mu[j], l = lv[j];
        const float sd = expf(0.5f * l);
        part += (m * m + expf(l)) - l - 1.f;
        for (int s = 0; s < ns; ++s) {
            const long zi = ((long)row * ns + s) * nz + j;
            z[zi] = m + eps[zi] * sd;
        }
    }
// ... 111 lines not shown
    uint16_t* orow = out + (long)r * ldo;
    const int t = r / B, b = r % B;
    long tg = ids[(long)b * ids_stride + t + tgt_off];
    if (tg < 0) tg = 0;
    if (tg >= V) tg = V - 1;
    const float L = lse[r], sc = rowscale[b];
    const bool vec = (ldl % 4 == 0) && ((((uintptr_t)logits) & 15) == 0) && (ldo % 4 == 0) && ((((uintptr_t)out) & 7) == 0);
    const int itg = (int)tg;
    int done = 0;
    if (vec) {
        const int V4 = V & ~3;
        for (int k = tid * 4; k < V4; k += 1024) {
            const float4 v = *reinterpret_cast<const float4*>(row + k);
            const float g0 = (expf(v.x - L) - (k == itg ? 1.f : 0.f)) * sc;
            const float g1 = (expf(v.y - L) - (k + 1 == itg ? 1.f : 0.f)) * sc;
            const float g2 = (expf(v.z - L) - (k + 2 == itg ? 1.f : 0.f)) * sc;
            const float g3 = (expf(v.w - L) - (k + 3 == itg ? 1.f : 0.f)) * sc;
            *reinterpret_cast<uint2*>(orow + k) = make_uint2(lv_pack_bf16x2(g0, g1), lv_pack_bf16x2(g2, g3));
        }
        done = V4;
    }
    for (int k = done + tid; k < V; k += 256)
        orow[k] = (uint16_t)lv_f32_to_bf16_bits((expf(row[k] - L) - (k == itg ? 1.f : 0.f)) * sc);
    for (long k = V + tid; k < ldo; k += 256) orow[k] = 0;
}

__global__ __launch_bounds__(256) void softmax_nll_merge_kernel(const float2* __restrict__ part, int nparts,
                                                                const float* __restrict__ tgt, float* __restrict__ lse,
                                                                float* __restrict__ nll, int R) {
    const int r = (int)blockIdx.x * 4 + ((int)threadIdx.x >> 6);
    const int l = (int)threadIdx.x & 63;
    if (r >= R) return;
    float m = -INFINITY, s = 0.f;
    for (int i0 = l; i0 < nparts; i0 += 512) {
        float2 q[8];
#pragma unroll
        for (int u = 0; u < 8; ++u) q[u] = part[(long)r * nparts + (i0 + 64 * u < nparts ? i0 + 64 * u : nparts - 1)];
#pragma unroll
        for (int u = 0; u < 8; ++u)
            if (i0 + 64 * u < nparts) ms_merge(m, s, q[u].x, q[u].y);
    }
#pragma unroll
    for (int d = 32; d >= 1; d >>= 1) {
        const float m2 = __shfl_xor(m, d, 64), s2 = __shfl_xor(s, d, 64);
        ms_merge(m, s, m2, s2);
    }
    if (l == 0) {
        const float L = m + logf(s);
        lse[r] = L;
        nll[r] = L - tgt[r];
    }
}

__global__ __launch_bounds__(256) void softmax_nll_bwd_h16_kernel(const uint16_t* __restrict__ logits16, long ldl,
                                                                  const float* __restrict__ lse, const int64_t* __restrict__ ids,
                                                                  long ids_stride, int tgt_off, const float* __restrict__ rowscale,
                                                                  uint16_t* __restrict__ out, long ldo, int T, int B, int V) {
    const int r = (int)blockIdx.x;
    const int tid = (int)threadIdx.x;
    const uint16_t* row = logits16 + (long)r * ldl;
    uint16_t* orow = out + (long)r * ldo;
    const int t = r / B, b = r % B;
    long tg = ids[(long)b * ids_stride + t + tgt_off];
    if (tg < 0) tg = 0;
    if (tg >= V) tg = V - 1;
    const float L = lse[r], sc = rowscale[b];
    const int itg = (int)tg;
    const bool vec = (ldl % 8 == 0) && ((((uintptr_t)logits16) & 15) == 0) && (ldo % 8 == 0) && ((((uintptr_t)out) & 15) == 0);
    int done = 0;
    if (vec) {
        const int V8 = V & ~7;
        for (int k = tid * 8; k < V8; k += 2048) {
            const uint4 q = *reinterpret_cast<const uint4*>(row + k);
            const uint32_t wv[4] = {q.x, q.y, q.z, q.w};
            uint32_t o[4];
#pragma unroll
            for (int h = 0; h < 4; ++h) {
                const float x0 = lv_f16_bits_to_f32((uint16_t)(wv[h] & 0xFFFFu)), x1 = lv_f16_bits_to_f32((uint16_t)(wv[h] >> 16));
                const float g0 = (lv_exp_fast(x0 - L) - (k + 2 * h == itg ? 1.f : 0.f)) * sc;
                const float g1 = (lv_exp_fast(x1 - L) - (k + 2 * h + 1 == itg ? 1.f : 0.f)) * sc;
                o[h] = lv_pack_bf16x2(g0, g1);
            }
            *reinterpret_cast<uint4*>(orow + k) = make_uint4(o[0], o[1], o[2], o[3]);
        }
        done = V8;
    }
    for (int k = done + tid; k < V; k += 256)
        orow[k] = (uint16_t)lv_f32_to_bf16_bits((lv_exp_fast(lv_f16_bits_to_f32(row[k]) - L) - (k == itg ? 1.f : 0.f)) * sc);
    for (long k = V + tid; k < ldo; k += 256) orow[k] = 0;
}

__global__ __launch_bounds__(256) void vae_loss_kernel(const float* __restrict__ nll, const float* __restrict__ kl,
                                                       const float* __restrict__ klw, float* __restrict__ loss,
                                                       float* __restrict__ rec, int T, int B) {
    const int b = (int)blockIdx.x * 4 + ((int)threadIdx.x >> 6);
    const int l = (int)threadIdx.x & 63;
    if (b >= B) return;
    float s = 0.f;
    for (int t = l; t < T; t += 64) s += nll[(long)t * B + b];
    s = lv_wave_sum(s);
    if (l == 0) {
        rec[b] = s;
        loss[b] = s + klw[0] * kl[b];
    }
}

// ... 163 lines not shown
extern "C" int lv_colsum_f32(const float* in, long ld, int R, int C, float* out, float* out2, void* stream) {
    if (!in || !out || R < 0 || C <= 0 || ld < C) return LV_ERR_ARG;
    LV_LAUNCH(colsum_kernel, dim3((unsigned)lv_cdiv(C, 256)), dim3(256), 0, stream, in, ld, R, C, out, out2);
    LV_CHECK_LAUNCH();
    return LV_OK;
}

extern "C" int lv_add_f32(const float* a, const float* b, float* out, long n, void* stream) {
    if (!a || !b || !out || n < 0) return LV_ERR_ARG;
    if (n == 0) return LV_OK;
    if ((n & 3) == 0 && ((((uintptr_t)a) | ((uintptr_t)b) | ((uintptr_t)out)) & 15) == 0) {
        LV_LAUNCH(add_v4_kernel, dim3((unsigned)lv_cdiv(n / 4, 256)), dim3(256), 0, stream, a, b, out, n / 4);
        LV_CHECK_LAUNCH();
        return LV_OK;
    }
    LV_LAUNCH(add_kernel, dim3((unsigned)lv_cdiv(n, 256)), dim3(256), 0, stream, a, b, out, n);
    LV_CHECK_LAUNCH();
    return LV_OK;
}

extern "C" int lv_loss_assemble_f32(const float* nll, const float* kl, const float* kl_weight_dev, const float* g_loss,
                                    float* loss, float* rec, float* rowscale, float* dkl, float* acc, int T, int B,
                                    void* stream) {
    if (!nll || !kl || !kl_weight_dev || !g_loss || !loss || !rec || !rowscale || !dkl || !acc) return LV_ERR_ARG;
    if (T < 0 || B <= 0) return LV_ERR_SHAPE;
    LV_LAUNCH(loss_assemble_kernel, dim3(1), dim3(64 * LA_WAVES), 0, stream, nll, kl, kl_weight_dev, g_loss, loss, rec, rowscale,
              dkl, acc, T, B, (unsigned long long*)nullptr, 0ULL);
    LV_CHECK_LAUNCH();
    return LV_OK;
}

extern "C" int lv_loss_assemble_rng_f32(const float* nll, const float* kl, const float* kl_weight_dev, const float* g_loss,
                                        float* loss, float* rec, float* rowscale, float* dkl, float* acc, int T, int B,
                                        uint64_t* rng_state, uint64_t rng_inc, void* stream) {
    if (!nll || !kl || !kl_weight_dev || !g_loss || !loss || !rec || !rowscale || !dkl || !acc || !rng_state) return LV_ERR_ARG;
    if (T < 0 || B <= 0) return LV_ERR_SHAPE;
    LV_LAUNCH(loss_assemble_kernel, dim3(1), dim3(64 * LA_WAVES), 0, stream, nll, kl, kl_weight_dev, g_loss, loss, rec, rowscale,
              dkl, acc, T, B, reinterpret_cast<unsigned long long*>(rng_state), (unsigned long long)rng_inc);
    LV_CHECK_LAUNCH();
    return LV_OK;
}

extern "C" int lv_softmax_nll_merge_f32(const float* part, int nparts, const float* tgt_logit, float* lse, float* nll, int R,
                                        void* stream) {
    if (!part || !tgt_logit || !lse || !nll) return LV_ERR_ARG;
    if (R < 0 || nparts <= 0) return LV_ERR_SHAPE;
    if (R == 0) return LV_OK;
    LV_LAUNCH(softmax_nll_merge_kernel, dim3((unsigned)lv_cdiv(R, 4)), dim3(256), 0, stream, reinterpret_cast<const float2*>(part),
              nparts, tgt_logit, lse, nll, R);
    LV_CHECK_LAUNCH();
    return LV_OK;
}

extern "C" int lv_softmax_nll_bwd_h16(const uint16_t* logits16, long ldl, const float* lse, const int64_t* ids, long ids_stride,
                                      int tgt_off, const float* rowscale, uint16_t* dlogits, long ldo, int T, int B, int V,
                                      void* stream) {
    if (!logits16 || !ids || !lse || !rowscale || !dlogits) return LV_ERR_ARG;
    if (T < 0 || B <= 0 || V <= 0 || ldl < V || ldo < V) return LV_ERR_SHAPE;
    if (T == 0) return LV_OK;
    LV_LAUNCH(softmax_nll_bwd_h16_kernel, dim3((unsigned)(T * B)), dim3(256), 0, stream, logits16, ldl, lse, ids, ids_stride,
              tgt_off, rowscale, dlogits, ldo, T, B, V);
    LV_CHECK_LAUNCH();
    return LV_OK;
}
```

vae_lagging_encoder_amd/engine.py:

```python
import ctypes
import os

import torch

from . import _lib

def backend_for(device):
    device = torch.device(device)
    if device.type == "cuda":
        return _lib.load()
    raise _lib.LvaeError(
        "vae_lagging_encoder_amd runs on MI355X (ROCm 'cuda' tensors) through its HIP extension; got a %s tensor. "
        "There is no CPU fallback." % device.type)


def stream_ptr(device):
    device = torch.device(device)
    if device.type == "cuda":
        return ctypes.c_void_p(torch.cuda.current_stream(device).cuda_stream)
    return None


def P(t, offset_elems=0):
    if t is None:
# ... 123 lines not shown
                budget_bytes = 8 << 30
        self.budget = budget_bytes

    def get(self, key, builder):
        ws = self.cache.get(key)
        if ws is not None:
            self.cache.move_to_end(key)
            self.hits += 1
            return ws
        self.misses += 1
        ws = builder()
        nb = _tensor_bytes(ws)
        self.cache[key] = ws
        self.nbytes[key] = nb
        self.total += nb
        self._trim(key)
        return ws

    def grew(self, key, nbytes):
        if key in self.nbytes:
            self.nbytes[key] += nbytes
            self.total += nbytes
            self._trim(key)

    def _trim(self, key):
        if not self.evictable:
            return
        told = False
        while self.total > self.budget and len(self.cache) > 8:
            k = next(iter(self.cache))
            if k == key:
                break
            if not told and self.before_evict is not None:
                self.before_evict()
                told = True
            del self.cache[k]
            self.total -= self.nbytes.pop(k)
            self.evictions += 1

    def f32(self, *shape):
        return torch.empty(*shape, dtype=torch.float32, device=self.device)

    def i16(self, *shape):
        return torch.empty(*shape, dtype=torch.int16, device=self.device)

    def i32(self, *shape):
        return torch.empty(*shape, dtype=torch.int32, device=self.device)


class _NS(object):
    pass


class _DecWS(_NS):

    @property
    def logits(self):
        if self._logits is None:
            self._logits = self._alloc()
            self._grew(self._logits.numel() * self._logits.element_size())
        return self._logits


PROFILE = None
PROFILE_PREFIX = None


class _prof(object):
    def __init__(self, name, work, launches=1):
        self.name, self.work, self.launches = name, work, launches
        self.on = PROFILE is not None and (PROFILE_PREFIX is None or name.startswith(PROFILE_PREFIX))

    def __enter__(self):
        if self.on:
            self.e0 = torch.cuda.Event(enable_timing=True)
            self.e1 = torch.cuda.Event(enable_timing=True)
            self.e0.record()

    def __exit__(self, *a):
        if self.on:
            self.e1.record()
            PROFILE.setdefault(self.name, []).append((self.e0, self.e1, self.work, self.launches))


_GEMM_WS = {}
_PERSISTENT_DEFAULT = True


def _gemm_ws(lib, s):
    dev = torch.device("cuda", torch.cuda.current_device()) if s is not None else torch.device("cpu")
    ws = _GEMM_WS.get(dev)
    if ws is None:
        ws = torch.empty(1 << 26 if dev.type == "cuda" else 1 << 20, dtype=torch.float32, device=dev)
        _GEMM_WS[dev] = ws
    return ws


def _gemm(lib, s, tA, tB, M, N, K, A, lda, B, ldb, C, ldc, alpha=1.0, acc=0, add1=None, ld1=0, mod1=1,
          add2=None, ld2=0, mod2=1, prec="f32", ws=None):
    if ws is None:
        ws = _gemm_ws(lib, s)
    fn = lib.lv_gemm_bf16 if prec == "bf16" else lib.lv_gemm_f32
    with _prof("gemm_" + prec, 2.0 * M * N * K):
        fn(tA, tB, M, N, K, alpha, A, lda, B, ldb, C, ldc, acc, add1, ld1, mod1, add2, ld2, mod2, P(ws), ws.numel(), s)


# ... 25 lines not shown
            t.record_stream(self.stream)
        with torch.cuda.stream(self.stream):
            fn(self.stream.cuda_stream)
            self.done = torch.cuda.Event()
            self.done.record(self.stream)

    def join(self, device):
        if self.done is not None:
            torch.cuda.current_stream(torch.device(device)).wait_event(self.done)
            self.done = None


class _TokenSortCache(object):
    LIMIT = 8192

    def __init__(self):
        import collections
        self.map = collections.OrderedDict()

    def _entries(self, key_tensor, create):
        i = id(key_tensor)
        ent = self.map.get(i)
        if ent is not None and ent[0]() is key_tensor:
            self.map.move_to_end(i)
            return ent[1]
        if not create:
            return None
        import weakref
        while len(self.map) >= self.LIMIT:
            self.map.popitem(last=False)
        self.map[i] = (weakref.ref(key_tensor, lambda _r, i=i, m=self.map: m.pop(i, None)), {})
        return self.map[i][1]

    def get(self, key_tensor, tag):
        ent = self._entries(key_tensor, False)
        hit = ent.get(tag) if ent is not None else None
        return hit[1:] if hit is not None and hit[0] == key_tensor._version else None

    def put(self, key_tensor, tag, srows, stok):
        self._entries(key_tensor, True)[tag] = (key_tensor._version, srows, stok)

    def invalidate(self, key_tensor=None):
        if key_tensor is None:
            self.map.clear()
        else:
            self.map.pop(id(key_tensor), None)


def reset_persistent_status(eng):
    if eng.status is not None:
        eng.status.zero_()


PERSIST_RUNGS = ("persistent, XCD-local hand-off", "persistent, write-through hand-off", "launch-per-timestep kernels")


def persist_rung(eng):
    if not eng.persistent:
        return 2
    return 0 if (eng.persist_flags & 1) else 1


def demote_persistent(eng):
    r = persist_rung(eng)
    if r == 0:
        eng.persist_flags &= ~1
    elif r == 1:
        eng.persistent = False
    else:
        raise _lib.LvaeError("a persistent-launch timeout was reported although the engine runs the launch-per-timestep kernels")
    reset_persistent_status(eng)
    eng.ladder_gen = getattr(eng, "ladder_gen", 0) + 1
    return r + 1


def status_ptr(eng):
    return P(eng.status) if eng.status is not None else None


_PERSIST_H = 1024
_PERSIST_MAX_B = 128


def _persist_rows(eng, B):
    rows = getattr(eng, "persist_rows", None)
    if rows is not None and 8 * rows >= B and 1 <= rows <= 16:
        return int(rows)
    return (B + 7) // 8


def _saved_floats(eng, T, B, H):
    n = T * B * 4 * H
    if H == _PERSIST_H and eng.precision == "bf16" and eng.persistent and B <= _PERSIST_MAX_B:
        n = max(n, eng.lib.lv_lstm_persist16_saved_floats(T, _persist_rows(eng, B)))
    return n


def _persistent_ok(eng, img, B, H, device, max_b):
    return (eng.precision == "bf16" and img is not None and eng.persistent and H == _PERSIST_H and B <= max_b
            and torch.device(device).type == "cuda" and torch.cuda.get_device_properties(device).multi_processor_count >= 256)


def weights_version(eng):
    return (sum(p._version for p in eng.flat.params), eng.wgen)


# ... 494 lines not shown
            _gemm(lib, s, 1, 0, nz2, H, B, P(w.dmulv), nz2, P(w.hs, T * B * H), H, P(gv["linear.weight"]), H)
        elif head is not None:
            eps, dz, parts, dkl = head
            lib.lv_enc_head_bwd_f32(P(w.mulv), P(eps), P(dz), parts, P(dkl), P(w.hs, T * B * H), P(v["linear.weight"]), P(w.dmulv),
                                    P(w.dhT), P(gv["linear.weight"]), B, H, eps.shape[1], nz2 // 2, s)
        else:
            dmulv = dmulv.contiguous()
            _gemm(lib, s, 0, 0, B, H, nz2, P(dmulv), nz2, P(v["linear.weight"]), H, P(w.dhT), H)
            _gemm(lib, s, 1, 0, nz2, H, B, P(dmulv), nz2, P(w.hs, T * B * H), H, P(gv["linear.weight"]), H)
        img = self._b16(B, T)
        with _prof("lstm_bwd_enc", float(T), 1 if _persistent_ok(self, img, B, H, x.device, _PERSIST_BWD_MAX_B) else 2 * T):
            _lstm_backward(self, lib, s, img, w, None, P(w.dhT), None, 1.0, P(v["lstm.weight_hh_l0"]), None, None, 0, T, B, H, x.device)
        if after_bptt is not None:
            after_bptt()
        def embed_grad():
            self._aux.join(x.device)
            if self.fold and "embed" in self.fold:
                sq, only = self.fold["embed"]
                lib.lv_embed_scatter_full_sumsq_f32(P(w.dX), None, 1.0, P(self._sort[0]), P(self._sort[1]), T, B, P(gv["embed.weight"]), ni,
                                                    V, -1, P(sq), int(only), s)
            else:
                lib.lv_embed_scatter_full_f32(P(w.dX), None, 1.0, P(self._sort[0]), P(self._sort[1]), T, B, P(gv["embed.weight"]), ni, V, -1, s)
            if after_embed is not None:
                after_embed()
        if img is not None:
            img.backward(lib, s, None, P(w.hs), P(self._wimg.WT), P(w.dX), P(gv["lstm.weight_ih_l0"]), ni, P(gv["lstm.weight_hh_l0"]),
                         between=embed_grad)
        else:
            _gemm(lib, s, 0, 0, T * B, ni, 4 * H, P(w.dG), 4 * H, P(v["lstm.weight_ih_l0"]), ni, P(w.dX), ni, prec=self.precision)
            embed_grad()
            _wgrad(lib, s, 4 * H, ni, T * B, P(w.dG), 4 * H, P(w.X), ni, P(gv["lstm.weight_ih_l0"]), ni, self.precision)
            _wgrad(lib, s, 4 * H, H, T * B, P(w.dG), 4 * H, P(w.hs), H, P(gv["lstm.weight_hh_l0"]), H, self.precision)
        lib.lv_colsum_f32(P(w.dGsum), 4 * H, B, 4 * H, P(gv["lstm.bias_ih_l0"]), P(gv["lstm.bias_hh_l0"]), s)


class LSTMDecoderEngine(object):

    def __init__(self, module):
        self.m = module
        self.flat = None
        self.wsc = None
        self.ws_evictable = True
        self.gen = 0
        self.precision = "f32"
        self.overlap = None
        self.native16 = True
        self.persistent = _PERSISTENT_DEFAULT
        self.persist_rows = None
        self.persist_flags = 1
        self.status = None
        self.fold = None
        self.cache_weight_images = True
        self.fused_nll = True
        self.wgen = 0
        self._wimg = None
        self._side = None
        self._side_ws = None
        self._pending = None
        self._aux = _AuxStream()
        self._sorts = _TokenSortCache()

    def _quiesce_side_streams(self):
        dev = self.flat.device if self.flat is not None else None
        if dev is not None and dev.type == "cuda":
            for st in (self._aux.stream, self._side):
                if st is not None:
                    torch.cuda.current_stream(dev).wait_stream(st)

    def _fork(self, device):
        import contextlib
        if not (torch.device(device).type == "cuda" and self._overlap_on()):
            return contextlib.nullcontext(), None
        if self._side is None:
            self._side = torch.cuda.Stream(device)
            self._side_ws = torch.empty(1 << 26, dtype=torch.float32, device=device)
        ev = torch.cuda.Event()
        ev.record(torch.cuda.current_stream(device))
        self._side.wait_event(ev)
        return torch.cuda.stream(self._side), self._side_ws

    def _overlap_on(self):
        if self.overlap is not None:
            return bool(self.overlap)
        return self.precision == "f32"

    def _mark_pending(self, device):
        if self._side is not None and torch.device(device).type == "cuda" and self._overlap_on():
            ev = torch.cuda.Event()
            ev.record(self._side)
            self._pending = ev

    def join(self):
        if self._pending is not None:
            torch.cuda.current_stream().wait_event(self._pending)
            self._pending = None

    def ensure(self, device):
        device = torch.device(device)
        if self.flat is None or self.flat.device != device or not self.flat.bound():
            m = self.m
            named = [("embed.weight", m.embed.weight), ("trans_linear.weight", m.trans_linear.weight),
                     ("lstm.weight_ih_l0", m.lstm.weight_ih_l0), ("lstm.weight_hh_l0", m.lstm.weight_hh_l0),
                     ("lstm.bias_ih_l0", m.lstm.bias_ih_l0), ("lstm.bias_hh_l0", m.lstm.bias_hh_l0),
                     ("pred_linear.weight", m.pred_linear.weight)]
            self.flat = FlatBuffer(named, device)
            self.flat.flat_grads = getattr(self, "_flat_grads_pref", True)
# ... 28 lines not shown
            w._grew = lambda nb: c.grew(key, nb)
            w.X = c.f32(Td * Bs, ni)
            if ns > 1:
                w.Gxw = c.f32(Td * Bs, 4 * H)
                w.dGs = c.f32(Td * Bs, 4 * H)
                w.x_rep = torch.empty(Bd, Td + 1, dtype=torch.int64, device=c.device)
                w.Zp_um = c.f32(Bd, 4 * H)
            w.Zp = c.f32(Bd, 4 * H)
            w.Gx = c.f32(Td * Bd, 4 * H)
            w.hs = c.f32(Td + 1, Bd, H)
            w.cs = c.f32(Td + 1, Bd, H)
            w.gates = c.f32(_saved_floats(self, Td, Bd, H))
            w.O = c.f32(Td * Bd, H)
            w._logits = None
            w.lse = c.f32(Td * Bd)
            w.nll = c.f32(Td * Bd)
            w.rec = c.f32(Bd)
            w.dO = c.f32(Td * Bd, H)
            w.dG = c.f32(Td * Bd, 4 * H)
            w.dGsum = c.f32(Bd, 4 * H)
            w.lstm_ws = c.f32(self.lib.lv_lstm_ws_floats(Bd, H))
            w.dc0 = c.f32(Bd, H)
            w.dX = c.f32(Td * Bs, ni)
            w.dz = c.f32(Bd, nz)
            w.dz_parts = self.lib.lv_dec_tail_parts(H)
            w.dzp = c.f32(w.dz_parts, Bd, nz)
            w.srows = c.i32(Td * Bs)
            w.stok = c.i32(Td * Bs)
            w.stmp = c.i32(2 * Td * Bs)
            w.zero1 = torch.zeros(1, dtype=torch.float32, device=c.device)
            w.klz = torch.zeros(Bd, dtype=torch.float32, device=c.device)
            w.loss = c.f32(Bd)
            return w
        return c.get(key, build)

    def fold_parts(self, B, Td, ns=1):
        out = {"embed": self.lib.lv_embed_scatter_sumsq_parts(Td, B)}
        V, ni, H, nz = self.dims()
        if self._b16(B * ns, Td, ns) is not None:
            dev = self.flat.device
            on_side = torch.device(dev).type == "cuda" and self._overlap_on()
            ws_n = (1 << 26) if on_side else _gemm_ws(self.lib, stream_ptr(dev)).numel()
            n = self.lib.lv_gemm_b16_sumsq_parts(V, H, Td * B * ns, ws_n)
            if n > 0:
                out["pred"] = n
        return out

    def _b16(self, Bd, Td, ns=1):
        V, ni, H, nz = self.dims()
        if self.precision != "bf16" or not self.native16 or H % 8 != 0:
            return None
        c = self.wsc

        def build():
            b = _NS()
            b.ldr = _round_up(Td * Bd, 8)
            b.ldv = _round_up(V, 32)
            b.O = c.i16(Td * Bd, H)
            b.OT = c.i16(H, b.ldr)
            b.dl = c.i16(Td * Bd, b.ldv)
            b.l16 = c.i16(Td * Bd, b.ldv)
            b.nparts = self.lib.lv_gemm_b16_nll_parts(V)
            b.part = c.f32(Td * Bd, 2 * b.nparts)
            b.tgt = c.f32(Td * Bd)
            return b
        return c.get(("b16", Bd, Td) if ns == 1 else ("b16", Bd // ns, ns, Td), build)

    def refresh_weight_images(self, B, device):
        V, ni, H, nz = self.dims()
        use_pred = self.precision == "bf16" and self.native16 and H % 8 == 0
        use_lstm = _LstmImages.usable(self.precision, self.native16, ni, H)
        if not (use_pred or use_lstm):
            return None
        self.ensure(device)
        persist = use_lstm and self.persistent and H == _PERSIST_H and B <= _PERSIST_MAX_B and \
            torch.device(device).type == "cuda" and torch.cuda.get_device_properties(device).multi_processor_count >= 256
        return _weight_images(self, self.lib, stream_ptr(device), device, persist, lstm=use_lstm, pred=use_pred)

    def _lstm_images(self, Bd, Td, ns=1):
        V, ni, H, nz = self.dims()
        if not _LstmImages.usable(self.precision, self.native16, ni, H):
            return None
        if ns > 1:
            return self.wsc.get(("b16lstm", Bd // ns, ns, Td), lambda: _LstmImagesMS(self.wsc, Td, Bd // ns, ns, ni, H))
        return self.wsc.get(("b16lstm", Bd, Td), lambda: _LstmImages(self.wsc, Td * Bd, ni, H, key=("b16lstm", Bd, Td)))

    def forward(self, x, z, mask_in, mask_out, p_in, p_out, want_rec=True, x_key=None):
        assert x.dtype == torch.int64 and x.dim() == 2
        x = x.contiguous()
        B, T = x.shape
        Td = T - 1
        if z.dim() != 3 or z.shape[0] != B or z.shape[1] < 1:
            raise _lib.LvaeError("the HIP decoder path takes z of shape [B, nsamples, nz]; got %s for a batch of %d" % (tuple(z.shape), B))
        ns = int(z.shape[1])
        Bd = B * ns
        z2 = z.reshape(Bd, -1).contiguous()
        f = self.ensure(x.device)
        lib, s = self.lib, stream_ptr(x.device)
        V, ni, H, nz = self.dims()
        w = self._ws(Bd, Td, ns)
        v = f.views
        sc_in = 1.0 / (1.0 - p_in) if mask_in is not None else 1.0
        sc_out = 1.0 / (1.0 - p_out) if mask_out is not None else 1.0
        if mask_in is not None:
            assert mask_in.dtype == torch.uint8 and tuple(mask_in.shape) == (B, Td, ni) and mask_in.is_contiguous()
        if mask_out is not None:
            assert mask_out.dtype == torch.uint8 and tuple(mask_out.shape) == (Bd, Td, H) and mask_out.is_contiguous()
        gather = (P(v["embed.weight"]), P(x), T, P(mask_in), sc_in, Td, B, V)
        img = self._lstm_images(Bd, Td, ns)
        if img is None:
            lib.lv_embed_gather_f32(P(v["embed.weight"]), P(x), T, P(mask_in), sc_in, P(w.X), Td, B, ni, V, s)
        self._sort = _sorted_tokens(self, lib, s, x, x_key, T, Td, B, V, w)
        ids = x
        if ns > 1:
            lib.lv_repeat_rows_i64(P(x), P(w.x_rep), B, T, ns, s)
            ids = w.x_rep
        wih = v["lstm.weight_ih_l0"]
        fused = fused_ends_ok(Bd, nz)
        if fused:
            lib.lv_dec_init_f32(P(z2), P(v["trans_linear.weight"]), P(wih), ni + nz, ni, P(v["lstm.bias_ih_l0"]),
                                P(v["lstm.bias_hh_l0"]), P(w.cs), P(w.hs), P(w.Zp), 1 if img is not None else 0, Bd, H, nz, s)
        else:
            _gemm(lib, s, 0, 1, Bd, H, nz, P(z2), nz, P(v["trans_linear.weight"]), nz, P(w.cs), H)
            lib.lv_tanh_f32(P(w.cs), P(w.hs), Bd * H, s)
            _gemm(lib, s, 0, 1, Bd, 4 * H, nz, P(z2), nz, P(wih, ni), ni + nz, P(w.Zp), 4 * H,
                  add1=P(v["lstm.bias_ih_l0"]), ld1=0, mod1=1, add2=P(v["lstm.bias_hh_l0"]), ld2=0, mod2=1)
        if ns > 1:
            zp = w.Zp
            if img is not None and not fused:
                lib.lv_gate_interleave_f32(P(w.Zp), None, Bd, H, P(w.Zp_um), s)
                zp = w.Zp_um
            if img is not None:
                wi = self.refresh_weight_images(Bd, x.device)
                img.forward(lib, s, P(wi.W), P(w.Gxw), gather)
            else:
                _gemm(lib, s, 0, 1, Td * B, 4 * H, ni, P(w.X), ni, P(wih), ni + nz, P(w.Gxw), 4 * H, prec=self.precision)
            lib.lv_gx_expand_add_f32(P(w.Gxw), P(zp), P(w.Gx), Td, B, ns, 4 * H, s)
        elif img is not None:
            wi = self.refresh_weight_images(B, x.device)
            if fused:
                img.forward(lib, s, None, P(wi.W), P(w.Gx), None, None, B, self.wsc, addend_um=P(w.Zp), gather=gather)
            else:
                img.forward(lib, s, None, P(wi.W), P(w.Gx), P(w.Zp), None, B, self.wsc, gather=gather)
        else:
            _gemm(lib, s, 0, 1, Td * B, 4 * H, ni, P(w.X), ni, P(wih), ni + nz, P(w.Gx), 4 * H,
                  add1=P(w.Zp), ld1=4 * H, mod1=B, prec=self.precision)
        b16 = self._b16(Bd, Td, ns)
        late_mask = b16 is not None and _persistent_ok(self, img, Bd, H, x.device, _PERSIST_MAX_B)
        with _prof("lstm_fwd_dec", float(Td), 1 if _persistent_ok(self, img, Bd, H, x.device, _PERSIST_MAX_B) else Td):
            if late_mask:
                _lstm_forward(self, lib, s, img, w, P(w.Gx), P(v["lstm.weight_hh_l0"]), None, 1.0, None, Td, Bd, H, x.device)
            else:
                _lstm_forward(self, lib, s, img, w, P(w.Gx), P(v["lstm.weight_hh_l0"]), P(mask_out), sc_out, P(w.O), Td, Bd, H, x.device)
        if b16 is not None:
            if late_mask and mask_out is not None:
                lib.lv_cvt_bf16_keep_f32(P(w.hs, Bd * H), H, Td, Bd, H, P(mask_out), sc_out, P(b16.O), H, P(b16.OT), b16.ldr, s)
            elif late_mask:
                lib.lv_cvt_bf16_f32(P(w.hs, Bd * H), H, Td * Bd, H, P(b16.O), H, P(b16.OT), b16.ldr, s)
            else:
                lib.lv_cvt_bf16_f32(P(w.O), H, Td * Bd, H, P(b16.O), H, P(b16.OT), b16.ldr, s)
            wi = self.refresh_weight_images(Bd, x.device)
            if self.fused_nll:
                with _prof("gemm_bf16", 2.0 * Td * Bd * V * H):
                    lib.lv_gemm_b16_nll(Td * Bd, V, H, P(b16.O), H, P(wi.pred), H, P(b16.l16), b16.ldv, P(ids), T, 1, Bd,
                                        P(b16.part), P(b16.tgt), s)
                lib.lv_softmax_nll_merge_f32(P(b16.part), b16.nparts, P(b16.tgt), P(w.lse), P(w.nll), Td * Bd, s)
            else:
                _gemm16(lib, s, 0, Td * Bd, V, H, P(b16.O), H, P(wi.pred), H, P(w.logits), w.ldl)
        else:
            _gemm(lib, s, 0, 1, Td * Bd, V, H, P(w.O), H, P(v["pred_linear.weight"]), H, P(w.logits), w.ldl, prec=self.precision)
        if not (b16 is not None and self.fused_nll):
            lib.lv_softmax_nll_fwd_f32(P(w.logits), w.ldl, P(ids), T, 1, P(w.lse), P(w.nll), Td, Bd, V, s)
        if want_rec:
            lib.lv_vae_loss_f32(P(w.nll), P(w.klz), P(w.zero1), P(w.loss), P(w.rec), Td, Bd, s)
        self.gen += 1
        self.last = (x, z2, mask_in, mask_out, sc_in, sc_out, B, T, self.gen)
        self.last_ns = ns
        return w.rec

    def cond_ll_supported(self, T):
        V, ni, H, nz = self.dims()
        return bool(self.lib.lv_dec_cond_ll_f32_supported(V, ni, H, nz, int(T)))

    def cond_ll(self, x, z):
        device = x.device
        if z.device != device:
            raise _lib.LvaeError("cond_ll: z is on %s, x on %s" % (z.device, device))
        self.ensure(device)
        V, ni, H, nz = self.dims()
        v = self.flat.views
        B, T = x.shape
        if x.dtype != torch.int64 or z.dim() not in (2, 3) or z.shape[-1] != nz or (z.dim() == 3 and z.shape[0] != B):
            raise ValueError("cond_ll: x int64 [B][T] and z [K][%d] or [B][K][%d] expected, got %s %s and %s"
                             % (nz, nz, x.dtype, tuple(x.shape), tuple(z.shape)))
        x = x.contiguous()
        z = z.contiguous().float()
        K = z.shape[-2]
        z_stride = 0 if z.dim() == 2 else K * nz
        ws = torch.empty(self.lib.lv_dec_cond_ll_f32_ws_floats(V, H, nz, B, T), dtype=torch.float32, device=device)
        out = torch.empty(B, K, dtype=torch.float32, device=device)
        self.lib.lv_dec_cond_ll_f32(P(x), B, T, P(z), z_stride, K, P(v["embed.weight"]), P(v["trans_linear.weight"]),
                                    P(v["lstm.weight_ih_l0"]), P(v["lstm.weight_hh_l0"]), P(v["lstm.bias_ih_l0"]),
                                    P(v["lstm.bias_hh_l0"]), P(v["pred_linear.weight"]), V, ni, H, nz, P(ws), P(out),
                                    stream_ptr(device))
        return out

    def backward(self, drec, gen=None, partial_dz=False):
        x, z2, mask_in, mask_out, sc_in, sc_out, B, T, g = self.last
        if gen is not None and gen != g:
            raise _lib.LvaeError("decoder activations were overwritten by a later forward(); the HIP engine keeps "
                                 "one in-flight step per module")
        ns = self.last_ns
        Bd, Td = B * ns, T - 1
        f = self.flat
        lib, s = self.lib, stream_ptr(x.device)
        V, ni, H, nz = self.dims()
        w = self._ws(Bd, Td, ns)
        v, gv = f.views, f.gviews
        drec = drec.contiguous()
        if drec.numel() != Bd:
            raise _lib.LvaeError("backward takes drec per decoder row (%d values for %d samples per sentence), got %d" % (Bd, ns, drec.numel()))
        ids = x if ns == 1 else w.x_rep
        wih = v["lstm.weight_ih_l0"]
        gwih = gv["lstm.weight_ih_l0"]
        dev = x.device
        b16 = self._b16(Bd, Td, ns)
        if b16 is not None and self.fused_nll:
            lib.lv_softmax_nll_bwd_h16(P(b16.l16), b16.ldv, P(w.lse), P(ids), T, 1, P(drec), P(b16.dl), b16.ldv, Td, Bd, V, s)
        elif b16 is not None:
            lib.lv_softmax_nll_bwd_b16(P(w.logits), w.ldl, P(w.lse), P(ids), T, 1, P(drec), P(b16.dl), b16.ldv, Td, Bd, V, s)
        else:
            lib.lv_softmax_nll_bwd_f32(P(w.logits), w.ldl, P(w.lse), P(ids), T, 1, P(drec), Td, Bd, V, s)
        ctx, sws = self._fork(dev)
        with ctx:
            if b16 is not None and self.fold and "pred" in self.fold:
                sq, only = self.fold["pred"]
                gws = sws if sws is not None else _gemm_ws(lib, s)
                if lib.lv_gemm_b16_sumsq_parts(V, H, Td * Bd, gws.numel()) != sq.numel():
                    raise RuntimeError("norm folding: the plan's partial count does not match this launch's tile plan")
                with _prof("gemm_bf16", 2.0 * V * H * Td * Bd):
                    lib.lv_gemm_b16_sumsq(1, V, H, Td * Bd, P(b16.dl), b16.ldv, P(b16.OT), b16.ldr, P(gv["pred_linear.weight"]), H,
                                          P(gws), gws.numel(), P(sq), int(only), stream_ptr(dev))
            elif b16 is not None:
                _gemm16(lib, stream_ptr(dev), 1, V, H, Td * Bd, P(b16.dl), b16.ldv, P(b16.OT), b16.ldr,
                        P(gv["pred_linear.weight"]), H, ws=sws)
            else:
                _wgrad(lib, stream_ptr(dev), V, H, Td * Bd, P(w.logits), w.ldl, P(w.O), H, P(gv["pred_linear.weight"]), H,
                       self.precision, ws=sws)
        img = self._lstm_images(Bd, Td, ns)
        late_mask = _persistent_ok(self, img, Bd, H, dev, _PERSIST_BWD_MAX_B)
        if b16 is not None and late_mask and mask_out is not None:
            gws = _gemm_ws(lib, s)
            with _prof("gemm_bf16", 2.0 * Td * Bd * H * V):
                lib.lv_gemm_b16_keep(Td * Bd, H, V, P(b16.dl), b16.ldv, P(self._wimg.predT), b16.ldv, P(w.dO), P(mask_out), sc_out, Bd,
                                     P(gws), gws.numel(), s)
        else:
            if b16 is not None:
                _gemm16(lib, s, 0, Td * Bd, H, V, P(b16.dl), b16.ldv, P(self._wimg.predT), b16.ldv, P(w.dO), H)
            else:
                _gemm(lib, s, 0, 0, Td * Bd, H, V, P(w.logits), w.ldl, P(v["pred_linear.weight"]), H, P(w.dO), H, prec=self.precision)
            if late_mask and mask_out is not None:
                lib.lv_keep_scale_f32(P(w.dO), P(mask_out), sc_out, Td, Bd, H, s)
        with _prof("lstm_bwd_dec", float(Td), 1 if late_mask else 2 * Td):
            _lstm_backward(self, lib, s, img, w, P(w.dO), None, None if late_mask else P(mask_out), 1.0 if late_mask else sc_out,
                           P(v["lstm.weight_hh_l0"]), None, P(w.dc0), 1, Td, Bd, H, dev)
        ctx, sws = self._fork(dev)
        with ctx:
            s2 = stream_ptr(dev)
            if img is not None:
                img.backward(lib, s2, None, P(w.hs), P(self._wimg.WT), P(w.dX), P(gwih), ni + nz, P(gv["lstm.weight_hh_l0"]), ws=sws)
            else:
                dG = w.dG
                if ns > 1:
                    lib.lv_sample_sum_f32(P(w.dG), P(w.dGs), Td, B, ns, 4 * H, s2)
                    dG = w.dGs
                _gemm(lib, s2, 0, 0, Td * B, ni, 4 * H, P(dG), 4 * H, P(wih), ni + nz, P(w.dX), ni, prec=self.precision, ws=sws)
                _wgrad(lib, s2, 4 * H, ni, Td * B, P(dG), 4 * H, P(w.X), ni, P(gwih), ni + nz, self.precision, ws=sws)
                _wgrad(lib, s2, 4 * H, H, Td * Bd, P(w.dG), 4 * H, P(w.hs), H, P(gv["lstm.weight_hh_l0"]), H,
                       self.precision, ws=sws)
            self._aux.join(dev)
            if self.fold and "embed" in self.fold:
                sq, only = self.fold["embed"]
                lib.lv_embed_scatter_full_sumsq_f32(P(w.dX), P(mask_in), sc_in, P(self._sort[0]), P(self._sort[1]), Td, B,
                                                    P(gv["embed.weight"]), ni, V, V - 1, P(sq), int(only), s2)
            else:
                lib.lv_embed_scatter_full_f32(P(w.dX), P(mask_in), sc_in, P(self._sort[0]), P(self._sort[1]), Td, B, P(gv["embed.weight"]), ni,
                                              V, V - 1, s2)
        self._mark_pending(dev)
        if not fused_ends_ok(Bd, nz):
            _gemm(lib, s, 1, 0, 4 * H, nz, Bd, P(w.dGsum), 4 * H, P(z2), nz, P(gwih, ni), ni + nz)
            lib.lv_colsum_f32(P(w.dGsum), 4 * H, Bd, 4 * H, P(gv["lstm.bias_ih_l0"]), P(gv["lstm.bias_hh_l0"]), s)
            _gemm(lib, s, 0, 0, Bd, nz, 4 * H, P(w.dGsum), 4 * H, P(wih, ni), ni + nz, P(w.dz), nz)
            _gemm(lib, s, 0, 0, Bd, nz, H, P(w.dc0), H, P(v["trans_linear.weight"]), nz, P(w.dz), nz, acc=1)
            _gemm(lib, s, 1, 0, H, nz, Bd, P(w.dc0), H, P(z2), nz, P(gv["trans_linear.weight"]), nz)
            return (w.dz, 1) if partial_dz else w.dz
        lib.lv_dec_tail_bwd_f32(P(w.dGsum), P(w.dc0), P(z2), P(wih), ni + nz, ni, P(v["trans_linear.weight"]), P(gwih), ni + nz,
                                P(gv["trans_linear.weight"]), P(gv["lstm.bias_ih_l0"]), P(gv["lstm.bias_hh_l0"]), P(w.dzp),
                                Bd, H, nz, s)
        if partial_dz:
            return w.dzp, w.dz_parts
        lib.lv_colsum_f32(P(w.dzp), Bd * nz, w.dz_parts, Bd * nz, P(w.dz), None, s)
        return w.dz


# ... 244 lines not shown
```

vae_lagging_encoder_amd/trainer.py:

```python
import collections
import ctypes

import numpy as np
import contextlib
import gc
import torch

from . import engine as _eng
from .engine import P



@contextlib.contextmanager
def _capture_graph(graph, stream):
    was_enabled = gc.isenabled()
    gc.disable()
    try:
        with torch.cuda.graph(graph, stream=stream):
            yield
    finally:
        if was_enabled:
            gc.enable()

class _Static(object):
# ... 85 lines not shown
        self._klw_host = 0.0
        self._journal = []
        self._committed_base = 0.0
        self.on_demote = _log_demotion
        self.recoveries = 0
        self.norm_ws = torch.empty(self.lib.lv_sumsq_workspace_floats(), dtype=torch.float32, device=d)
        self.rng_state = torch.tensor([_rank_seed(seed, grad_sync), 0], dtype=torch.int64, device=d)
        self.static = collections.OrderedDict()
        for e in (self.enc, self.dec):
            e.ws_evictable = e.ws_evictable and not self.use_graph
            if e.wsc is not None:
                e.wsc.evictable = e.ws_evictable

    def _s(self, i):
        return P(self.scal, i)

    def set_lr(self, lr):
        self.scal[1] = lr

    ADAM_STEP = {"enc": 13, "dec": 14}

    def reset_optimizer(self, lr, betas=None):
        self.commit()
        self.scal[1] = lr
        if self.optimizer != "adam":
            return
        if betas is not None and (float(betas[0]), float(betas[1])) != self.betas:
            self.betas = (float(betas[0]), float(betas[1]))
            for st in self.static.values():
                st.graphs = {}
        self.scal[13:15] = 0
        for k in ("enc", "dec"):
            self.adam_m[k].zero_()
            self.adam_v[k].zero_()

    def adam_steps(self):
        v = self.scal[13:15].cpu().tolist()
        return int(v[0]), int(v[1])

    JOURNAL_MAX = 64

    def read_stats(self):
        v = self._settle(self.scal.cpu().tolist())
        return dict(loss_sum=v[5], rec_sum=v[6], kl_sum=v[7], norm=v[4], coef=v[3])

    def commit(self):
        self._settle(self.scal.cpu().tolist())
        return max(_eng.persist_rung(self.enc), _eng.persist_rung(self.dec))

    def _settle(self, v):
        while v[8] != 0.0:
            done = int(round(v[9] - self._committed_base))
            redo = self._journal[done:]
            if all(_eng.persist_rung(e) == 2 for e in (self.enc, self.dec)):
                raise _eng._lib.LvaeError("a step was voided although both engines run the launch-per-timestep kernels (status words "
                                          "%s / %s)" % (self.enc.status.tolist(), self.dec.status.tolist()))
            for e in (self.enc, self.dec):
                if _eng.persist_rung(e) < 2:
                    _eng.demote_persistent(e)
                else:
                    _eng.reset_persistent_status(e)
            self.recoveries += 1
            for st in self.static.values():
                st.graphs = {}
            self.scal[8:13] = 0
            self._committed_base = 0.0
            self._journal = []
            if self.on_demote is not None:
                self.on_demote(max(_eng.persist_rung(self.enc), _eng.persist_rung(self.dec)))
            for x, klw, noise, update in redo:
                self._queue_step(x, klw, noise, update)
                self._journal.append((x, klw, noise, update))
            v = self.scal.cpu().tolist()
        self._committed_base = v[9]
        self._journal = []
        if v[9] >= 4194304.0:
            self.scal[9] = 0
            self._committed_base = 0.0
        return v

    def reset_stats(self):
        self.scal[5:8] = 0

    def prepare_batches(self, batches):
        if self.use_graph:
            return
        lib = self.lib
        for x in batches:
            if not (x.is_contiguous() and x.device == self.device and x.dtype == torch.int64 and x.dim() == 2):
                continue
            B, T = x.shape
            s = _eng.stream_ptr(self.device)
            for eng, Tu in ((self.enc, T), (self.dec, T - 1)):
                if Tu <= 0 or eng._sorts.get(x, (Tu, B)) is not None:
                    continue
                V = eng.dims()[0]
                srows, stok = eng.wsc.i32(Tu * B), eng.wsc.i32(Tu * B)
                tmp = eng.wsc.i32(2 * Tu * B)
                lib.lv_token_sort(P(x), T, Tu, B, V, P(srows), P(stok), P(tmp), s)
                eng._sorts.put(x, (Tu, B), srows, stok)

    def enable_row_exchange(self, batches, mode="auto"):
        gs = self.grad_sync
        if gs is None or not gs.active:
            return False
        if self.micro_batches != 1 or self.use_graph:
            raise ValueError("the row-list exchange runs with micro_batches = 1 in eager mode")
        self.prepare_batches(batches)
        V, ni = self.enc.dims()[:2]
        uniq = []
        self._row_index = {}
        for j, x in enumerate(batches):
            B, T = x.shape
            _, stok = self.enc._sorts.get(x, (T, B))
            uniq.append(torch.unique_consecutive(stok).to(torch.int64))
            self._row_index[id(x)] = j
        self._row_keep = list(batches)
        ef = self.enc.flat
        return gs.prepare_rows(uniq, V, ni, ef.offsets[ef.names[1]], mode=mode)

    def invalidate_batch(self, x=None):
        self.enc._sorts.invalidate(x)
        self.dec._sorts.invalidate(x)

    def _static_for(self, B, T, parts=1):
        key = (B, T) if parts == 1 else (B, T, parts)
        st = self.static.get(key)
        if st is not None:
            self.static.move_to_end(key)
        else:
            d = self.device
            V, ni, H, nz = self.dec.dims()
# ... 237 lines not shown
                df.use_slot(i)
                if gs is not None:
                    gs.set_slot(i)
                self._fwd_bwd(st, draw)
                if dp:
                    gs.sync_issue(ef, df, update)
            dec_ss = None
            if dp:
                for i in range(m):
                    ef.use_slot(i)
                    df.use_slot(i)
                    gs.set_slot(i)
                    gs.sync_collect(ef, df, update)
                dec_ss = gs.sync_norm(df, update, tuple(range(m)))
        finally:
            ef.use_slot(0)
            df.use_slot(0)
            if gs is not None:
                gs.set_slot(0)
        for f in (ef, df):
            for i in range(1, m):
                lib.lv_add_f32(P(f._slots[0][0]), P(f._slots[i][0]), P(f._slots[0][0]), f._slots[0][0].numel(), s)
        self._clip_and_step(update, dec_ss)
        if update in ("encoder", "both"):
            self.enc.wgen += 1
        if update in ("decoder", "both"):
            self.dec.wgen += 1

    def _queue_step(self, x, kl_weight, noise, update):
        if self.micro_batches > 1:
            return self._queue_micro(x, kl_weight, noise, update, self.micro_batches)
        B, T = x.shape
        for e in (self.enc, self.dec):
            if e.flat.detached:
                e.flat.attach_grads()
        st = self._static_for(B, T)
        if self.use_graph or not (x.is_contiguous() and x.device == self.device and x.dtype == torch.int64):
            st.x.copy_(x)
            st.xin = st.x
        else:
            st.xin = x
        st.x_key = x
        if self._klw_host != float(kl_weight):
            self.scal[0] = float(kl_weight)
            self._klw_host = float(kl_weight)
        draw = noise is None
        if not draw:
            eps, m_in, m_out = noise
            st.eps.copy_(eps.reshape(st.eps.shape))
            if m_in is not None:
                st.m_in.copy_(m_in)
            if m_out is not None:
                st.m_out.copy_(m_out)
        try:
            if not self.use_graph:
                self._run(st, update, draw)
                return
            self.enc.refresh_weight_images(B, self.device)
            self.dec.refresh_weight_images(B, self.device)
            gens = (getattr(self.enc, "ladder_gen", 0), getattr(self.dec, "ladder_gen", 0))
            key = (update, draw, self.vae.training) + gens
            g = st.graphs.get(key)
            if g is None:
                for k in [k for k in st.graphs if k[3:] != gens]:
                    del st.graphs[k]
                self._run(st, update, draw)
                torch.cuda.synchronize(self.device)
                g = self._capture(st, update, draw)
                st.graphs[key] = g
                return
            for part in g:
                part()
        finally:
            if update in ("encoder", "both"):
                self.enc.wgen += 1
            if update in ("decoder", "both"):
                self.dec.wgen += 1

    def _check_noise(self, x, noise):
        B, T = x.shape
        V, ni, H, nz = self.dec.dims()
        ns = self.nsamples
        want = ((B, ns, nz), (B, T - 1, ni), (B * ns, T - 1, H))
        for name, got, shape in zip(("eps", "mask_in", "mask_out"), noise, want):
            if got is not None and tuple(got.shape) != shape:
                raise ValueError("nsamples = %d: %s must have shape %s, got %s" % (ns, name, shape, tuple(got.shape)))

    def _capture(self, st, update, draw):
        parts = []
        self._update = update
        self._plan_fold(st, update)
        stream = torch.cuda.Stream(self.device)
        stream.wait_stream(torch.cuda.current_stream(self.device))

        def cap(fn):
            gr = torch.cuda.CUDAGraph()
            self._capturing = True
            try:
                with _capture_graph(gr, stream):
                    fn()
            finally:
                self._capturing = False
            return gr.replay
        if self.grad_sync is None:
            parts.append(cap(lambda: (self._fwd_bwd(st, draw), self._clip_and_step(update))))
        else:
            self._update = update
            parts.append(cap(lambda: self._fwd_bwd(st, draw)))
            ss = self.grad_sync.ss_handle(self.dec.flat, update)
            parts.append(lambda: self.grad_sync.sync(self.enc.flat, self.dec.flat, update))
            parts.append(cap(lambda: self._clip_and_step(update, ss)))
        return parts

    def inner_loop(self, batches, first, kl_weight, np_rng=None, max_iter=100, window=15, fixed_k=None, noise_fn=None, next_batch=None):
        rng = np_rng if np_rng is not None else np.random
        sub_iter = 1
        x = first
        burn_num_words = 0
        burn_pre_loss = 1e4
        self.reset_stats()
        steps = 0
        while sub_iter < max_iter:
            B, T = x.shape
            burn_num_words += (T - 1) * B
            self.step(x, kl_weight, noise=None if noise_fn is None else noise_fn(x), update="encoder")
            steps += 1
# ... 198 lines not shown
```

Before: 11340.

## Add exp-image NLL route folding softmax rescale into backward GEMM

Adds a new fused NLL path. The logits GEMM epilogue stores exp(logits) as bf16 and accumulates row sums, instead of storing fp16 logits and running a separate softmax backward. The merge kernel computes lse and the per-row scale factors kappa, rz and corr. The backward dlogits GEMM then applies the row scale and subtracts the target-weight correction in its tail, and the OT conversion is folded into a rescaled transpose, which removes the separate softmax-backward pass over the V-wide logits. The trade-offs are possible exp overflow, handled through a status word that falls back to the logits route and replays the step, and extra host-side routing logic.

```diff
diff --git a/include/lvae.h b/include/lvae.h
--- a/include/lvae.h
+++ b/include/lvae.h
@@ -48,6 +48,24 @@
 int lv_softmax_nll_merge_f32(const float* part, int nparts, const float* tgt_logit, float* lse, float* nll, int R, void* stream);
 int lv_softmax_nll_bwd_h16(const uint16_t* logits16, long ldl, const float* lse, const int64_t* ids, long ids_stride, int tgt_off,
                            const float* rowscale, uint16_t* dlogits, long ldo, int T, int B, int V, void* stream);
+int lv_gemm_b16_nll_exp_supported(int M, int N, int K);
+int lv_gemm_b16_nll_exp_tile(int tile, int M, int N, int K, const uint16_t* A, long lda, const uint16_t* B, long ldb, uint16_t* expimg,
+                             long lde, float* part, void* stream);
+int lv_gemm_b16_nll_exp(int M, int N, int K, const uint16_t* A, long lda, const uint16_t* B, long ldb, uint16_t* expimg, long lde,
+                        float* part, void* stream);
+int lv_softmax_nll_merge_exp_f32(const float* part, int nparts, const uint16_t* A, long lda, const uint16_t* W, long ldw, int K,
+                                 const int64_t* ids, long ids_stride, int tgt_off, int Bsz, uint16_t* expimg, long lde, int V,
+                                 float* lse, float* nll, float* kappa, float* rz, float* corr, int* status, int R, void* stream);
+int lv_gemm_b16_keep_rs(int M, int N, int K, const uint16_t* A, long lda, const uint16_t* B, long ldb, float* C,
+                        const uint8_t* keep, float kscale, int Bsz, const float* rz, const float* drec, const float* corr,
+                        const float* W, long ldw, const int64_t* ids, long ids_stride, int tgt_off,
+                        float* ws, long ws_floats, void* stream);
+int lv_gemm_b16_keep_rs_tile(int tile, int M, int N, int K, const uint16_t* A, long lda, const uint16_t* B, long ldb, float* C,
+                             const uint8_t* keep, float kscale, int Bsz, const float* rz, const float* drec, const float* corr,
+                             const float* W, long ldw, const int64_t* ids, long ids_stride, int tgt_off,
+                             float* ws, long ws_floats, void* stream);
+int lv_cvt_bf16_keep_rs_f32(const float* src, long lds, int T, int Bsz, int C, const uint8_t* keep, float kscale,
+                            const float* kappa, const float* drec, uint16_t* dstT, long ldt, void* stream);
 int lv_cvt_bf16_f32(const float* src, long lds, int R, int C, uint16_t* dst, long ldd, uint16_t* dstT, long ldt,
                     void* stream);
 int lv_cvt_bf16_keep_f32(const float* src, long lds, int T, int Bsz, int C, const uint8_t* keep, float kscale,
diff --git a/vae_lagging_encoder_amd/_lib.py b/vae_lagging_encoder_amd/_lib.py
--- a/vae_lagging_encoder_amd/_lib.py
+++ b/vae_lagging_encoder_amd/_lib.py
@@ -30,6 +30,13 @@
     "lv_gemm_b16_nll_tile": [_i, _i, _i, _i, _vp, _l, _vp, _l, _vp, _l, _vp, _l, _i, _i, _vp, _vp, _vp],
     "lv_gemm_b16_nll": [_i, _i, _i, _vp, _l, _vp, _l, _vp, _l, _vp, _l, _i, _i, _vp, _vp, _vp],
     "lv_softmax_nll_merge_f32": [_vp, _i, _vp, _vp, _vp, _i, _vp],
+    "lv_gemm_b16_nll_exp_supported": [_i, _i, _i],
+    "lv_gemm_b16_nll_exp_tile": [_i, _i, _i, _i, _vp, _l, _vp, _l, _vp, _l, _vp, _vp],
+    "lv_gemm_b16_nll_exp": [_i, _i, _i, _vp, _l, _vp, _l, _vp, _l, _vp, _vp],
+    "lv_softmax_nll_merge_exp_f32": [_vp, _i, _vp, _l, _vp, _l, _i, _vp, _l, _i, _i, _vp, _l, _i, _vp, _vp, _vp, _vp, _vp, _vp, _i, _vp],
+    "lv_gemm_b16_keep_rs": [_i, _i, _i, _vp, _l, _vp, _l, _vp, _vp, _f, _i, _vp, _vp, _vp, _vp, _l, _vp, _l, _i, _vp, _l, _vp],
+    "lv_gemm_b16_keep_rs_tile": [_i, _i, _i, _i, _vp, _l, _vp, _l, _vp, _vp, _f, _i, _vp, _vp, _vp, _vp, _l, _vp, _l, _i, _vp, _l, _vp],
+    "lv_cvt_bf16_keep_rs_f32": [_vp, _l, _i, _i, _i, _vp, _f, _vp, _vp, _vp, _l, _vp],
     "lv_softmax_nll_bwd_h16": [_vp, _l, _vp, _vp, _l, _i, _vp, _vp, _l, _i, _i, _i, _vp],
     "lv_cvt_bf16_f32": [_vp, _l, _i, _i, _vp, _l, _vp, _l, _vp],
     "lv_cvt_bf16_keep_f32": [_vp, _l, _i, _i, _i, _vp, _f, _vp, _l, _vp, _l, _vp],
@@ -201,7 +208,7 @@
             setattr(self, "_raw_" + name, fn)
         if missing:
             raise LvaeError("%s does not export: %s" % (path, ", ".join(missing)))
-        self._value_fns = {"lv_gemm_b16_dual_supported", "lv_gemm_b16_pair_supported", "lv_lstm_bwd_ksplit", "lv_dec_tail_parts", "lv_gemm_b16_nll_parts", "lv_gemm_b16_sumsq_parts", "lv_embed_scatter_sumsq_parts", "lv_conv32_wpack_floats",
+        self._value_fns = {"lv_gemm_b16_dual_supported", "lv_gemm_b16_nll_exp_supported", "lv_gemm_b16_pair_supported", "lv_lstm_bwd_ksplit", "lv_dec_tail_parts", "lv_gemm_b16_nll_parts", "lv_gemm_b16_sumsq_parts", "lv_embed_scatter_sumsq_parts", "lv_conv32_wpack_floats",
                            "lv_conv32_wgrad_slabs", "lv_conv32_wgrad_ws_floats", "lv_conv32_wgrad_parts", "lv_conv1x1_wgrad_parts", "lv_conv32_blocks", "lv_conv1x1_blocks", "lv_conv1x1_wgrad_ws_floats", "lv_sumsq_workspace_floats", "lv_lstm_ws_floats", "lv_bn_workspace_floats",
                            "lv_lstm_persist16_wpk_floats", "lv_lstm_persist16_xch_floats", "lv_lstm_persist16_saved_floats",
                            "lv_pixelcnn_net_words", "lv_pixelcnn_block_words", "lv_conv32_tap_split", "lv_dec_cond_ll_f32_supported",
diff --git a/vae_lagging_encoder_amd/csrc/lv_device.h b/vae_lagging_encoder_amd/csrc/lv_device.h
--- a/vae_lagging_encoder_amd/csrc/lv_device.h
+++ b/vae_lagging_encoder_amd/csrc/lv_device.h
@@ -40,6 +40,7 @@
 static inline void lv_sleep_short() { }
 #define LV_ARRIVAL_POLLS 2
 static inline unsigned atomicExch(unsigned* p, unsigned v) { return __atomic_exchange_n(p, v, __ATOMIC_RELAXED); }
+static inline int atomicCAS(int* p, int cmp, int v) { __atomic_compare_exchange_n(p, &cmp, v, false, __ATOMIC_RELAXED, __ATOMIC_RELAXED); return cmp; }
 #define LV_S_BARRIER() __syncthreads()
 #define LV_SETPRIO(n) do { } while (0)
 static inline uint2 lv_ds_read_tr16_b64(const void* lds_ptr) {
diff --git a/vae_lagging_encoder_amd/csrc/lv_gemm_b16.hip b/vae_lagging_encoder_amd/csrc/lv_gemm_b16.hip
--- a/vae_lagging_encoder_amd/csrc/lv_gemm_b16.hip
+++ b/vae_lagging_encoder_amd/csrc/lv_gemm_b16.hip
@@ -45,6 +45,7 @@
     const uint8_t* keep; float kscale; int keepT;
     float* sq; int sq_only;
     float* C2; long ldc2; int nsplit;
+    const float* rs_rz; const float* rs_drec; const float* rs_corr; const float* rs_W; long rs_ldw;
 };
 
 __device__ __forceinline__ uint4 load_chunk(const uint16_t* __restrict__ p, int valid) {
@@ -676,7 +677,13 @@
     return k;
 }
 
-template <bool NLL>
+template <int BIT>
+__device__ __forceinline__ float fold_lanes(float x, float y, int l) {
+    const float xs = __shfl_xor(x, BIT, 64), ys = __shfl_xor(y, BIT, 64);
+    return (l & BIT) ? ys + y : x + xs;
+}
+
+template <int NLL>
 __device__ __forceinline__ void t256_epilogue(const GemmQ& p, const Tail256& q, f32x16 (&acc)[4][2], LdsTile2& As0, LdsTile2& Bs0,
                                               LdsTile2& As1, LdsTile2& Bs1, int tile, int piece, int tn, int m0, int n0, int t, int l,
                                               int wm, int wn, int lh) {
@@ -691,23 +698,50 @@
                        : b == 2 ? reinterpret_cast<char*>(&As1[0][0]) : reinterpret_cast<char*>(&Bs1[0][0]);
             return base + (rr & 63) * 512;
         };
+        constexpr bool EXP = NLL == 2;
         const int odd = l & 1;
 #pragma unroll
         for (int i2 = 0; i2 < 4; ++i2) {
             char* const bufp = rowptr(wm * 128 + i2 * 32);
+            float rs[16];
+#pragma unroll
+            for (int e = 0; e < 16; ++e) rs[e] = 0.f;
 #pragma unroll
             for (int j = 0; j < 2; ++j) {
                 const int clp = (wn * 64 + j * 32 + (l & 31)) & ~1;
                 const int lane_off = (4 * lh + odd) * 512 + ((((clp >> 3) ^ (4 * lh) ^ odd) << 4) | ((clp & 7) << 1));
+                const bool inN = n0 + wn * 64 + j * 32 + (l & 31) < p.N;
 #pragma unroll
                 for (int e = 0; e < 16; e += 2) {
-                    const float mine0 = acc[i2][j][e], mine1 = acc[i2][j][e + 1];
+                    float mine0 = acc[i2][j][e], mine1 = acc[i2][j][e + 1];
+                    if constexpr (EXP) {
+                        mine0 = inN ? lv_exp_fast(mine0) : 0.f;
+                        mine1 = inN ? lv_exp_fast(mine1) : 0.f;
+                        rs[e] += mine0;
+                        rs[e + 1] += mine1;
+                    }
                     const float got = lv_lane_xor1(odd ? mine0 : mine1);
-                    const uint32_t pk = odd ? lv_pack_f16x2(got, mine1) : lv_pack_f16x2(mine0, got);
+                    uint32_t pk;
+                    if constexpr (EXP) pk = odd ? lv_pack_bf16x2(got, mine1) : lv_pack_bf16x2(mine0, got);
+                    else pk = odd ? lv_pack_f16x2(got, mine1) : lv_pack_f16x2(mine0, got);
                     const int key = (e & 3) | (8 * ((e >> 2) & 1));
                     const int roff = ((e & 3) + 8 * (e >> 2)) * 512;
                     *reinterpret_cast<uint32_t*>(bufp + roff + (lane_off ^ (key << 4))) = pk;
                 }
+            }
+            if constexpr (EXP) {
+                float a8[8], a4[4], a2[2];
+#pragma unroll
+                for (int k = 0; k < 8; ++k) a8[k] = lv_fold16(rs[k], rs[k + 8]);
+#pragma unroll
+                for (int k = 0; k < 4; ++k) a4[k] = lv_fold8(a8[k], a8[k + 4]);
+#pragma unroll
+                for (int k = 0; k < 2; ++k) a2[k] = fold_lanes<4>(a4[k], a4[k + 2], l);
+                float a1 = fold_lanes<2>(a2[0], a2[1], l);
+                a1 += lv_lane_xor1(a1);
+                const int eo = ((l >> 1) & 1) | (((l >> 2) & 1) << 1) | (((l >> 3) & 1) << 2) | (((l >> 4) & 1) << 3);
+                const int prow = m0 + wm * 128 + i2 * 32 + (eo & 3) + 8 * (eo >> 2) + 4 * lh;
+                if (!odd && prow < p.M) p.part[(long)prow * p.nparts + 4 * tn + wn] = make_float2(0.f, a1);
             }
         }
         __syncthreads();
@@ -723,6 +757,7 @@
             }
         }
 #endif
+        if constexpr (EXP) return;
         const int rr = t & 255, half = t >> 8;
         const int row = m0 + rr;
         if (row < p.M) {
@@ -804,7 +839,7 @@
             store_frag_f32(p, acc[i2][j], m0 + wm * 128 + i2 * 32 + 4 * (l >> 5), n0 + wn * (32 * NJ) + j * 32 + (l & 31));
 }
 
-template <bool NLL, bool TN, bool PP = false>
+template <int NLL, bool TN, bool PP = false>
 __global__ __launch_bounds__(512) void lv_gemm_b16_t256_kernel(GemmQ p, Tail256 q) {
     constexpr int WN = 4;
     constexpr int NJ = 2;
@@ -1255,7 +1290,7 @@
 #undef LV_Q_WAIT
 }
 
-template <bool NLL, bool TN>
+template <int NLL, bool TN>
 __global__ __launch_bounds__(512) void lv_gemm_b16_t256q_kernel(GemmQ p, Tail256 q) {
     __shared__ __attribute__((aligned(1024))) LdsTile2 As0, Bs0;
     __shared__ __attribute__((aligned(1024))) LdsTile2 As1, Bs1;
@@ -1477,6 +1512,16 @@
         const int rr = ((int)blockIdx.x % TR_WGS) * TR_ROWS + 4 * it + (t >> 6);
         const int row = tm * BT2 + rr;
         if (row >= p.M) continue;
+        float rf = 1.f, cw = 0.f, wv[4] = {0.f, 0.f, 0.f, 0.f};
+        if (p.rs_rz) {
+            long tg = p.ids[(long)(row % p.Bsz) * p.ids_stride + row / p.Bsz + p.tgt_off];
+            tg = tg < 0 ? 0 : (tg >= p.K ? p.K - 1 : tg);
+            rf = p.rs_drec[row % p.Bsz] * p.rs_rz[row];
+            cw = p.rs_drec[row % p.Bsz] * p.rs_corr[row];
+            const float* wrow = p.rs_W + tg * p.rs_ldw;
+#pragma unroll
+            for (int e = 0; e < 4; ++e) wv[e] = wrow[tn * BT2 + c4 + e < p.N ? tn * BT2 + c4 + e : p.N - 1];
+        }
         float4 sacc = make_float4(0.f, 0.f, 0.f, 0.f);
         for (int k0 = 0; k0 < q.tail_s; k0 += 4) {
             float4 pv[4];
@@ -1491,6 +1536,10 @@
         if (fast && tn * BT2 + c4 + 3 < p.N) {
             const int col = tn * BT2 + c4;
             float4 o = make_float4(p.alpha * sv[0], p.alpha * sv[1], p.alpha * sv[2], p.alpha * sv[3]);
+            if (p.rs_rz) {
+                o.x = o.x * rf + cw * wv[0]; o.y = o.y * rf + cw * wv[1];
+                o.z = o.z * rf + cw * wv[2]; o.w = o.w * rf + cw * wv[3];
+            }
             if (p.keep) {
                 const uint32_t mk = *reinterpret_cast<const uint32_t*>(p.keep + ((long)(row % p.Bsz) * p.keepT + row / p.Bsz) * p.N + col);
                 o.x = (mk & 0xFFu) ? o.x * p.kscale : 0.f;
@@ -1511,6 +1560,7 @@
             if (p.add2) v += p.add2[(long)(row % p.mod2) * p.ld2 + col];
             float* c = p.C + (long)row * p.ldc + col;
             if (p.accumulate) v += *c;
+            if (p.rs_rz) v = v * rf + cw * wv[e];
             if (p.keep) v *= p.keep[((long)(row % p.Bsz) * p.keepT + row / p.Bsz) * p.N + col] ? p.kscale : 0.f;
             ss += v * v;
             if (!p.sq_only) *c = v;
@@ -1583,12 +1633,13 @@
 __global__ __launch_bounds__(256) void cvt_b16_kernel(const float* __restrict__ src, long lds_, int R, int C,
                                                       uint16_t* __restrict__ dst, long ldd, uint16_t* __restrict__ dstT, long ldt,
                                                       int gate_H, const uint8_t* __restrict__ keep, float kscale, int Bsz,
-                                                      const int64_t* __restrict__ gids, long gstride, int gV, int lo) {
+                                                      const int64_t* __restrict__ gids, long gstride, int gV, int lo,
+                                                      const float* __restrict__ rs_kappa, const float* __restrict__ rs_drec) {
     __shared__ uint16_t tile[64][66];
     const int t = (int)threadIdx.x;
     const int r0 = (int)blockIdx.y * 64, c0 = (int)blockIdx.x * 64;
     const int lane = t & 63, q = t >> 6;
-    const bool tb = keep || gids;
+    const bool tb = keep || gids || rs_kappa;
     const int Tt = tb ? R / Bsz : 1;
     int bb = tb ? (r0 + q) % Bsz : 0, tt = tb ? (r0 + q) / Bsz : 0;
     const int gc = c0 + lane, gcc = gc < C ? gc : C - 1;
@@ -1612,10 +1663,14 @@
 #pragma unroll
             for (int u = 0; u < 8; ++u) sr[u] = sr[u] < 0 ? 0 : (sr[u] >= gV ? gV - 1 : sr[u]);
         }
-        float v[8];
+        float v[8], rf[8];
         uint8_t kp[8];
 #pragma unroll
         for (int u = 0; u < 8; ++u) v[u] = src[sr[u] * lds_ + gcc];
+        if (rs_kappa) {
+#pragma unroll
+            for (int u = 0; u < 8; ++u) rf[u] = rs_drec[bbs[u]] * rs_kappa[sr[u]];
+        }
         if (keep) {
 #pragma unroll
             for (int u = 0; u < 8; ++u) kp[u] = keep[((long)bbs[u] * Tt + (grs[u] < R ? tts[u] : 0)) * C + gcc];
@@ -1630,6 +1685,7 @@
                     if (gids) x = kp[u] ? x * kscale : 0.f;
                     else x *= kp[u] ? kscale : 0.f;
                 }
+                if (rs_kappa) x *= rf[u];
                 b = (uint16_t)lv_f32_to_bf16_bits(x);
                 if (lo == 1) b = (uint16_t)lv_f32_to_bf16_bits(x - lv_bf16_bits_to_f32(b));
                 if (dst) {
@@ -1654,12 +1710,13 @@
 __global__ __launch_bounds__(256) void cvt_b16_v4_kernel(const float* __restrict__ src, long lds_, int R, int C,
                                                          uint16_t* __restrict__ dst, long ldd, uint16_t* __restrict__ dstT, long ldt,
                                                          int gate_H, const uint8_t* __restrict__ keep, float kscale, int Bsz,
-                                                         const int64_t* __restrict__ gids, long gstride, int gV, int lo) {
+                                                         const int64_t* __restrict__ gids, long gstride, int gV, int lo,
+                                                      const float* __restrict__ rs_kappa, const float* __restrict__ rs_drec) {
     __shared__ __attribute__((aligned(8))) uint16_t tile[64][68];
     const int t = (int)threadIdx.x;
     const int r0 = (int)blockIdx.y * 64, c0 = (int)blockIdx.x * 64;
     const int q = t >> 4, cl = t & 15;
-    const bool tb = keep || gids;
+    const bool tb = keep || gids || rs_kappa;
     const int Tt = tb ? R / Bsz : 1;
     int bb = tb ? (r0 + q) % Bsz : 0, tt = tb ? (r0 + q) / Bsz : 0;
     const int gc = c0 + 4 * cl;
@@ -1684,8 +1741,13 @@
     }
     float4 v[4];
     uint32_t kp[4] = {0u, 0u, 0u, 0u};
+    float rf[4] = {1.f, 1.f, 1.f, 1.f};
 #pragma unroll
     for (int u = 0; u < 4; ++u) v[u] = *reinterpret_cast<const float4*>(src + sr[u] * lds_ + gcc);
+    if (rs_kappa) {
+#pragma unroll
+        for (int u = 0; u < 4; ++u) rf[u] = rs_drec[bbs[u]] * rs_kappa[sr[u]];
+    }
     if (keep) {
 #pragma unroll
         for (int u = 0; u < 4; ++u)
@@ -1706,6 +1768,7 @@
                     if (gids) x = k ? x * kscale : 0.f;
                     else x *= k ? kscale : 0.f;
                 }
+                if (rs_kappa) x *= rf[u];
                 b[e] = (uint16_t)lv_f32_to_bf16_bits(x);
                 if (lo == 1) b[e] = (uint16_t)lv_f32_to_bf16_bits(x - lv_bf16_bits_to_f32(b[e]));
                 d[e] = lo == 2 ? lv_f32_to_f16_bits(lv_sat_f16(x)) : b[e];
@@ -1737,13 +1800,14 @@
 }
 
 static void cvt_launch(void* stream, const float* src, long lds, int R, int C, uint16_t* dst, long ldd, uint16_t* dstT, long ldt, int gate_H,
-                       const uint8_t* keep, float kscale, int Bsz, const int64_t* gids, long gstride, int gV, int lo) {
+                       const uint8_t* keep, float kscale, int Bsz, const int64_t* gids, long gstride, int gV, int lo,
+                       const float* rs_kappa = nullptr, const float* rs_drec = nullptr) {
     const dim3 grid((unsigned)lv_cdiv(C, 64), (unsigned)lv_cdiv(R, 64)), block(256);
     const bool v4 = C >= 4 && C % 4 == 0 && lds % 4 == 0 && (((uintptr_t)src) & 15) == 0 &&
                     (!dst || (ldd % 4 == 0 && (((uintptr_t)dst) & 7) == 0)) && (!dstT || (ldt % 4 == 0 && (((uintptr_t)dstT) & 7) == 0)) &&
                     (!keep || (((uintptr_t)keep) & 3) == 0);
-    if (v4) LV_LAUNCH(cvt_b16_v4_kernel, grid, block, 0, stream, src, lds, R, C, dst, ldd, dstT, ldt, gate_H, keep, kscale, Bsz, gids, gstride, gV, lo);
-    else LV_LAUNCH(cvt_b16_kernel, grid, block, 0, stream, src, lds, R, C, dst, ldd, dstT, ldt, gate_H, keep, kscale, Bsz, gids, gstride, gV, lo);
+    if (v4) LV_LAUNCH(cvt_b16_v4_kernel, grid, block, 0, stream, src, lds, R, C, dst, ldd, dstT, ldt, gate_H, keep, kscale, Bsz, gids, gstride, gV, lo, rs_kappa, rs_drec);
+    else LV_LAUNCH(cvt_b16_kernel, grid, block, 0, stream, src, lds, R, C, dst, ldd, dstT, ldt, gate_H, keep, kscale, Bsz, gids, gstride, gV, lo, rs_kappa, rs_drec);
 }
 
 }
@@ -1781,14 +1845,50 @@
 
 extern "C" int lv_keep_scale_f32(float* x, const uint8_t* keep, float kscale, int T, int Bsz, int C, void* stream);
 
+namespace {
+__global__ __launch_bounds__(256) void row_keep_scale_kernel(float* __restrict__ C, const uint8_t* __restrict__ keep, float kscale,
+                                                             const float* __restrict__ rz, const float* __restrict__ drec,
+                                                             const float* __restrict__ corr, const float* __restrict__ W, long ldw,
+                                                             const int64_t* __restrict__ ids, long ids_stride, int tgt_off, int V,
+                                                             int M, int N, int Bsz) {
+    const int row = (int)blockIdx.x;
+    const int b = row % Bsz, tt = row / Bsz;
+    const float rf = drec[b] * rz[row];
+    long tg = ids[(long)b * ids_stride + tt + tgt_off];
+    tg = tg < 0 ? 0 : (tg >= V ? V - 1 : tg);
+    const float cw = drec[b] * corr[row];
+    const float* wrow = W + tg * ldw;
+    float* c = C + (long)row * N;
+    const uint8_t* k = keep ? keep + ((long)b * (M / Bsz) + tt) * N : nullptr;
+    for (int col = (int)threadIdx.x; col < N; col += 256) {
+        float v = c[col] * rf + cw * wrow[col];
+        if (k) v *= k[col] ? kscale : 0.f;
+        c[col] = v;
+    }
+}
+}
+struct RowScale {
+    const float* rz; const float* drec; const float* corr; const float* W; long ldw;
+    const int64_t* ids; long ids_stride; int tgt_off;
+};
+static int row_keep_scale_launch(float* C, const uint8_t* keep, float kscale, const RowScale& r, int M, int N, int V, int Bsz, void* stream) {
+    LV_LAUNCH(row_keep_scale_kernel, dim3((unsigned)M), dim3(256), 0, stream, C, keep, kscale, r.rz, r.drec, r.corr, r.W, r.ldw, r.ids,
+              r.ids_stride, r.tgt_off, V, M, N, Bsz);
+    LV_CHECK_LAUNCH();
+    return LV_OK;
+}
+
 static int gemm_b16_launch(int tile, int transA, int M, int N, int K, float alpha,
                            const uint16_t* A, long lda, const uint16_t* B, long ldb,
                            float* C, long ldc, int accumulate,
                            const float* add1, long ld1, int mod1,
                            const float* add2, long ld2, int mod2,
                            float* ws, long ws_floats, void* stream, const uint8_t* keep, float kscale, int Bsz,
-                           float* sq = nullptr, int sq_only = 0, int f16 = 0, float* C2 = nullptr, long ldc2 = 0, int nsplit = 0) {
+                           float* sq = nullptr, int sq_only = 0, int f16 = 0, float* C2 = nullptr, long ldc2 = 0, int nsplit = 0,
+                           const RowScale* rs = nullptr) {
     if (tile != 0 && tile != 128 && (tile < 256 || tile > 258)) return LV_ERR_ARG;
+    const float* rs_rz = rs ? rs->rz : nullptr;
+    if (rs_rz && (!rs->drec || !rs->corr || !rs->W || !rs->ids || transA || sq || f16 || C2 || accumulate || add1 || add2 || ldc != N)) return LV_ERR_ARG;
     if (f16) {
         if (transA || keep || sq || !LV_B16_GLDS) return LV_ERR_UNSUPPORTED;
         tile = 128;
@@ -1814,7 +1914,7 @@
         if (t256_wanted(tile, M, N, K) || !ws) return LV_ERR_UNSUPPORTED;
     }
     if (sq && (!t256_wanted(tile, M, N, K) || accumulate || add1 || add2 || keep)) return LV_ERR_ARG;
-    bool keep_pending = keep != nullptr;
+    bool keep_pending = keep != nullptr, rs_pending = rs_rz != nullptr;
     const int nk = lv_cdiv(K > 0 ? K : 1, BK);
     if (t256_wanted(tile, M, N, K)) {
         p.tilesM = lv_cdiv(M, BT2); p.tilesN = lv_cdiv(N, BT2);
@@ -1822,6 +1922,11 @@
         const Tail256 q = t256_plan((long)p.tilesM * p.tilesN, nk, ws ? ws_floats : 0);
         const long tail = (long)p.tilesM * p.tilesN - q.full;
         if (keep && q.full == 0 && q.tail_s > 1) { p.keep = keep; p.kscale = kscale; p.keepT = M / p.Bsz; keep_pending = false; }
+        if (rs_rz && q.full == 0 && q.tail_s > 1) {
+            p.rs_rz = rs_rz; p.rs_drec = rs->drec; p.rs_corr = rs->corr; p.rs_W = rs->W; p.rs_ldw = rs->ldw;
+            p.ids = rs->ids; p.ids_stride = rs->ids_stride; p.tgt_off = rs->tgt_off;
+            rs_pending = false;
+        }
         dim3 grid((unsigned)(q.full + tail * q.tail_s)), block(512);
         const int sched = t256_sched(tile, q.tail_s > 1 && q.full == 0 ? q.kt_per_piece : nk);
         if (sched == 2) {
@@ -1834,6 +1939,7 @@
         else LV_LAUNCH((lv_gemm_b16_t256_kernel<false, false>), grid, block, 0, stream, p, q);
         if (q.tail_s > 1) LV_LAUNCH(tail_reduce_t256_kernel, dim3((unsigned)(tail * TR_WGS)), dim3(256), 0, stream, p, q);
         LV_CHECK_LAUNCH();
+        if (rs_pending) return row_keep_scale_launch(C, keep_pending ? keep : nullptr, kscale, *rs, M, N, K, p.Bsz, stream);
         if (keep_pending) return lv_keep_scale_f32(C, keep, kscale, M / p.Bsz, p.Bsz, N, stream);
         return LV_OK;
     }
@@ -1858,7 +1964,7 @@
     p.kt_per_split = lv_cdiv(nk, splits);
     splits = lv_cdiv(nk, p.kt_per_split);
     p.splits = splits;
-    if (keep && splits > 1) { p.keep = keep; p.kscale = kscale; p.keepT = M / p.Bsz; keep_pending = false; }
+    if (keep && splits > 1 && !rs_rz) { p.keep = keep; p.kscale = kscale; p.keepT = M / p.Bsz; keep_pending = false; }
     dim3 grid((unsigned)tiles, (unsigned)splits), block(256);
     if (transA && LV_B16_GLDS == 1 && p.kt_per_split > 32) LV_LAUNCH((lv_gemm_b16_nt_glds_kernel<false, false, true>), grid, block, 0, stream, p);
     else if (transA && LV_B16_GLDS) LV_LAUNCH((lv_gemm_b16_nt_glds_kernel<true, false, true>), grid, block, 0, stream, p);
@@ -1876,6 +1982,7 @@
         else LV_LAUNCH(splitk_reduce_b16_kernel, dim3((unsigned)lv_cdiv((long)M * N, 256)), dim3(256), 0, stream, p);
     }
     LV_CHECK_LAUNCH();
+    if (rs_pending) return row_keep_scale_launch(C, keep_pending ? keep : nullptr, kscale, *rs, M, N, K, p.Bsz, stream);
     if (keep_pending) return lv_keep_scale_f32(C, keep, kscale, M / p.Bsz, p.Bsz, N, stream);
     return LV_OK;
 }
@@ -1996,6 +2103,24 @@
     return gemm_b16_launch(0, 0, M, N, K, 1.f, A, lda, B, ldb, C, N, 0, nullptr, 0, 1, nullptr, 0, 1, ws, ws_floats, stream, keep, kscale, Bsz);
 }
 
+extern "C" int lv_gemm_b16_keep_rs_tile(int tile, int M, int N, int K, const uint16_t* A, long lda, const uint16_t* B, long ldb, float* C,
+                                        const uint8_t* keep, float kscale, int Bsz, const float* rz, const float* drec, const float* corr,
+                                        const float* W, long ldw, const int64_t* ids, long ids_stride, int tgt_off,
+                                        float* ws, long ws_floats, void* stream) {
+    if (!rz || !drec || !corr || !W || !ids || Bsz <= 0 || M % Bsz != 0 || ldw < N) return LV_ERR_ARG;
+    const RowScale rs{rz, drec, corr, W, ldw, ids, ids_stride, tgt_off};
+    return gemm_b16_launch(tile, 0, M, N, K, 1.f, A, lda, B, ldb, C, N, 0, nullptr, 0, 1, nullptr, 0, 1, ws, ws_floats, stream, keep, kscale, Bsz,
+                           nullptr, 0, 0, nullptr, 0, 0, &rs);
+}
+
+extern "C" int lv_gemm_b16_keep_rs(int M, int N, int K, const uint16_t* A, long lda, const uint16_t* B, long ldb, float* C,
+                                   const uint8_t* keep, float kscale, int Bsz, const float* rz, const float* drec, const float* corr,
+                                   const float* W, long ldw, const int64_t* ids, long ids_stride, int tgt_off,
+                                   float* ws, long ws_floats, void* stream) {
+    return lv_gemm_b16_keep_rs_tile(0, M, N, K, A, lda, B, ldb, C, keep, kscale, Bsz, rz, drec, corr, W, ldw, ids, ids_stride, tgt_off, ws,
+                                    ws_floats, stream);
+}
+
 extern "C" int lv_gemm_b16_sumsq_parts(int M, int N, int K, long ws_floats) {
     if (M <= 0 || N <= 0 || K <= 0 || !t256_wanted(0, M, N, K)) return 0;
     const long tiles = (long)lv_cdiv(M, BT2) * lv_cdiv(N, BT2);
@@ -2046,6 +2171,17 @@
     if (R == 0 || C == 0) return LV_OK;
     cvt_launch(stream, src, lds, (int)R, C,
               dst, ldd, dstT, ldt, 0, keep, kscale, Bsz, (const int64_t*)nullptr, 0L, 0, 0);
+    LV_CHECK_LAUNCH();
+    return LV_OK;
+}
+
+extern "C" int lv_cvt_bf16_keep_rs_f32(const float* src, long lds, int T, int Bsz, int C, const uint8_t* keep, float kscale,
+                                       const float* kappa, const float* drec, uint16_t* dstT, long ldt, void* stream) {
+    if (!src || !kappa || !drec || !dstT) return LV_ERR_ARG;
+    const long R = (long)T * Bsz;
+    if (T < 0 || Bsz <= 0 || C < 0 || lds < C || ldt < R) return LV_ERR_SHAPE;
+    if (R == 0 || C == 0) return LV_OK;
+    cvt_launch(stream, src, lds, (int)R, C, (uint16_t*)nullptr, 0L, dstT, ldt, 0, keep, kscale, Bsz, (const int64_t*)nullptr, 0L, 0, 0, kappa, drec);
     LV_CHECK_LAUNCH();
     return LV_OK;
 }
@@ -2144,3 +2280,40 @@
                                float* part, float* tgt_logit, void* stream) {
     return lv_gemm_b16_nll_tile(0, M, N, K, A, lda, B, ldb, logits16, ldl16, ids, ids_stride, tgt_off, Bsz, part, tgt_logit, stream);
 }
+
+extern "C" int lv_gemm_b16_nll_exp_supported(int M, int N, int K) { return M > 0 && N > 0 && K > 0 && t256_wanted(0, M, N, K) ? 1 : 0; }
+
+extern "C" int lv_gemm_b16_nll_exp_tile(int tile, int M, int N, int K, const uint16_t* A, long lda, const uint16_t* B, long ldb,
+                                        uint16_t* expimg, long lde, float* part, void* stream) {
+    if (tile != 0 && (tile < 256 || tile > 258)) return LV_ERR_ARG;
+    if (M < 0 || N <= 0 || K <= 0) return LV_ERR_SHAPE;
+    if (!t256_wanted(tile, M, N, K)) return LV_ERR_UNSUPPORTED;
+    if (M == 0) return LV_OK;
+    if (!A || !B || !expimg || !part) return LV_ERR_ARG;
+    if (lda < K || ldb < K || lde < N) return LV_ERR_SHAPE;
+    if (lda % 8 != 0 || ldb % 8 != 0 || lde % 8 != 0 || (((uintptr_t)A) & 15) != 0 || (((uintptr_t)B) & 15) != 0 ||
+        (((uintptr_t)expimg) & 15) != 0 || (((uintptr_t)part) & 7) != 0)
+        return LV_ERR_ALIGN;
+    GemmQ p{};
+    p.A = A; p.B = B; p.C = nullptr; p.M = M; p.N = N; p.K = K;
+    p.lda = lda; p.ldb = ldb; p.ldc = 0; p.alpha = 1.f; p.accumulate = 0;
+    p.add1 = nullptr; p.add2 = nullptr; p.mod1 = p.mod2 = 1; p.ws = nullptr;
+    p.splits = 1; p.kt_per_split = lv_cdiv(K, BK);
+    p.C16 = expimg; p.ldc16 = lde; p.Bsz = 1;
+    p.part = reinterpret_cast<float2*>(part); p.nparts = lv_gemm_b16_nll_parts(N);
+    p.tilesM = lv_cdiv(M, BT2); p.tilesN = lv_cdiv(N, BT2);
+    Tail256 q;
+    const long tiles = (long)p.tilesM * p.tilesN;
+    q.full = (int)(tiles / 256 * 256); q.tail = (int)(tiles - q.full); q.tail_s = 1; q.kt_per_piece = p.kt_per_split;
+    const int sched = t256_sched(tile, p.kt_per_split);
+    if (sched == 2) LV_LAUNCH((lv_gemm_b16_t256q_kernel<2, false>), dim3((unsigned)tiles), dim3(512), 0, stream, p, q);
+    else if (sched == 1) LV_LAUNCH((lv_gemm_b16_t256_kernel<2, false, true>), dim3((unsigned)tiles), dim3(512), 0, stream, p, q);
+    else LV_LAUNCH((lv_gemm_b16_t256_kernel<2, false>), dim3((unsigned)tiles), dim3(512), 0, stream, p, q);
+    LV_CHECK_LAUNCH();
+    return LV_OK;
+}
+
+extern "C" int lv_gemm_b16_nll_exp(int M, int N, int K, const uint16_t* A, long lda, const uint16_t* B, long ldb,
+                                   uint16_t* expimg, long lde, float* part, void* stream) {
+    return lv_gemm_b16_nll_exp_tile(0, M, N, K, A, lda, B, ldb, expimg, lde, part, stream);
+}
diff --git a/vae_lagging_encoder_amd/csrc/lv_loss.hip b/vae_lagging_encoder_amd/csrc/lv_loss.hip
--- a/vae_lagging_encoder_amd/csrc/lv_loss.hip
+++ b/vae_lagging_encoder_amd/csrc/lv_loss.hip
@@ -187,6 +187,64 @@
     }
 }
 
+__global__ __launch_bounds__(256) void softmax_nll_merge_exp_kernel(const float2* __restrict__ part, int nparts,
+                                                                    const uint16_t* __restrict__ A, long lda,
+                                                                    const uint16_t* __restrict__ W, long ldw, int K,
+                                                                    const int64_t* __restrict__ ids, long ids_stride, int tgt_off, int Bsz,
+                                                                    uint16_t* __restrict__ E, long lde, int V, float* __restrict__ lse,
+                                                                    float* __restrict__ nll, float* __restrict__ kappa,
+                                                                    float* __restrict__ rz, float* __restrict__ corr,
+                                                                    int* __restrict__ status, int R) {
+    const int r = (int)blockIdx.x * 4 + ((int)threadIdx.x >> 6);
+    const int l = (int)threadIdx.x & 63;
+    if (r >= R) return;
+    long tg = ids[(long)(r % Bsz) * ids_stride + r / Bsz + tgt_off];
+    if (tg < 0) tg = 0;
+    if (tg >= V) tg = V - 1;
+    float z = 0.f;
+    for (int i0 = l; i0 < nparts; i0 += 512) {
+        float2 q[8];
+#pragma unroll
+        for (int u = 0; u < 8; ++u) q[u] = part[(long)r * nparts + (i0 + 64 * u < nparts ? i0 + 64 * u : nparts - 1)];
+#pragma unroll
+        for (int u = 0; u < 8; ++u)
+            if (i0 + 64 * u < nparts) z += q[u].y;
+    }
+    const uint16_t* a = A + (long)r * lda;
+    const uint16_t* wv = W + tg * ldw;
+    float dot = 0.f;
+    for (int k0 = 8 * l; k0 < K; k0 += 512) {
+        const uint4 qa = *reinterpret_cast<const uint4*>(a + k0), qw = *reinterpret_cast<const uint4*>(wv + k0);
+        const uint32_t ua[4] = {qa.x, qa.y, qa.z, qa.w}, uw[4] = {qw.x, qw.y, qw.z, qw.w};
+#pragma unroll
+        for (int h = 0; h < 4; ++h) {
+            if (k0 + 2 * h < K) dot += lv_bf16_bits_to_f32(ua[h] & 0xFFFFu) * lv_bf16_bits_to_f32(uw[h] & 0xFFFFu);
+            if (k0 + 2 * h + 1 < K) dot += lv_bf16_bits_to_f32(ua[h] >> 16) * lv_bf16_bits_to_f32(uw[h] >> 16);
+        }
+    }
+#pragma unroll
+    for (int d = 32; d >= 1; d >>= 1) {
+        z += __shfl_xor(z, d, 64);
+        dot += __shfl_xor(dot, d, 64);
+    }
+    if (l == 0) {
+        const float L = logf(z);
+        lse[r] = L;
+        nll[r] = L - dot;
+        const float dd = expf(dot) - z;
+        const uint32_t qb = lv_f32_to_bf16_bits(dd);
+        const float qf = lv_bf16_bits_to_f32(qb);
+        const float ratio = dd == 0.f ? 1.f : dd / qf;
+        const float kp = ratio / z;
+        E[(long)r * lde + tg] = (uint16_t)qb;
+        kappa[r] = kp;
+        rz[r] = 1.f / z;
+        corr[r] = (dd - qf) / z;
+        const bool ok = z >= 5.42101086e-20f && z <= 1.26765060e30f && ratio - ratio == 0.f;
+        if (!ok) atomicCAS(status, 0, 400);
+    }
+}
+
 __global__ __launch_bounds__(256) void softmax_nll_bwd_h16_kernel(const uint16_t* __restrict__ logits16, long ldl,
                                                                   const float* __restrict__ lse, const int64_t* __restrict__ ids,
                                                                   long ids_stride, int tgt_off, const float* __restrict__ rowscale,
@@ -456,6 +514,20 @@
     return LV_OK;
 }
 
+extern "C" int lv_softmax_nll_merge_exp_f32(const float* part, int nparts, const uint16_t* A, long lda, const uint16_t* W, long ldw, int K,
+                                            const int64_t* ids, long ids_stride, int tgt_off, int Bsz, uint16_t* expimg, long lde, int V,
+                                            float* lse, float* nll, float* kappa, float* rz, float* corr, int* status, int R,
+                                            void* stream) {
+    if (!part || !A || !W || !ids || !expimg || !lse || !nll || !kappa || !rz || !corr || !status) return LV_ERR_ARG;
+    if (R < 0 || nparts <= 0 || K <= 0 || V <= 0 || Bsz <= 0 || lda < K || ldw < K || lde < V) return LV_ERR_SHAPE;
+    if (lda % 8 != 0 || ldw % 8 != 0 || (((uintptr_t)A) & 15) != 0 || (((uintptr_t)W) & 15) != 0) return LV_ERR_ALIGN;
+    if (R == 0) return LV_OK;
+    LV_LAUNCH(softmax_nll_merge_exp_kernel, dim3((unsigned)lv_cdiv(R, 4)), dim3(256), 0, stream, reinterpret_cast<const float2*>(part),
+              nparts, A, lda, W, ldw, K, ids, ids_stride, tgt_off, Bsz, expimg, lde, V, lse, nll, kappa, rz, corr, status, R);
+    LV_CHECK_LAUNCH();
+    return LV_OK;
+}
+
 extern "C" int lv_softmax_nll_bwd_h16(const uint16_t* logits16, long ldl, const float* lse, const int64_t* ids, long ids_stride,
                                       int tgt_off, const float* rowscale, uint16_t* dlogits, long ldo, int T, int B, int V,
                                       void* stream) {
diff --git a/vae_lagging_encoder_amd/engine.py b/vae_lagging_encoder_amd/engine.py
--- a/vae_lagging_encoder_amd/engine.py
+++ b/vae_lagging_encoder_amd/engine.py
@@ -199,6 +199,16 @@
     pass
 
 
+class _B16WS(_NS):
+
+    @property
+    def l16(self):
+        if self._l16 is None:
+            self._l16 = self._alloc()
+            self._grew(self._l16.numel() * self._l16.element_size())
+        return self._l16
+
+
 class _DecWS(_NS):
 
     @property
@@ -330,6 +340,7 @@
         eng.status.zero_()
 
 
+NLL_EXP_STATUS = 400
 PERSIST_RUNGS = ("persistent, XCD-local hand-off", "persistent, write-through hand-off", "launch-per-timestep kernels")
 
 
@@ -930,6 +941,10 @@
         self.fold = None
         self.cache_weight_images = True
         self.fused_nll = True
+        self.nll_route = "exp"
+        self.nll_gated = False
+        self.nll_tile = 0
+        self.last_nll_route = None
         self.wgen = 0
         self._wimg = None
         self._side = None
@@ -1064,19 +1079,33 @@
             return None
         c = self.wsc
 
+        key = ("b16", Bd, Td) if ns == 1 else ("b16", Bd // ns, ns, Td)
+
         def build():
-            b = _NS()
+            b = _B16WS()
             b.ldr = _round_up(Td * Bd, 8)
             b.ldv = _round_up(V, 32)
             b.O = c.i16(Td * Bd, H)
             b.OT = c.i16(H, b.ldr)
             b.dl = c.i16(Td * Bd, b.ldv)
-            b.l16 = c.i16(Td * Bd, b.ldv)
+            b._l16 = None
+            b._alloc = lambda: c.i16(Td * Bd, b.ldv)
+            b._grew = lambda nb: c.grew(key, nb)
+            b.kappa = c.f32(Td * Bd)
+            b.rz = c.f32(Td * Bd)
+            b.corr = c.f32(Td * Bd)
             b.nparts = self.lib.lv_gemm_b16_nll_parts(V)
             b.part = c.f32(Td * Bd, 2 * b.nparts)
             b.tgt = c.f32(Td * Bd)
             return b
-        return c.get(("b16", Bd, Td) if ns == 1 else ("b16", Bd // ns, ns, Td), build)
+        return c.get(key, build)
+
+    def _exp_route(self, b16, late_mask, M, V, H):
+        if b16 is None or not self.fused_nll or self.nll_route != "exp" or not self.nll_gated:
+            return False
+        if self.nll_tile:
+            return self.nll_tile >= 256
+        return bool(late_mask) and bool(self.lib.lv_gemm_b16_nll_exp_supported(M, V, H))
 
     def refresh_weight_images(self, B, device):
         V, ni, H, nz = self.dims()
@@ -1164,15 +1193,23 @@
                 _lstm_forward(self, lib, s, img, w, P(w.Gx), P(v["lstm.weight_hh_l0"]), None, 1.0, None, Td, Bd, H, x.device)
             else:
                 _lstm_forward(self, lib, s, img, w, P(w.Gx), P(v["lstm.weight_hh_l0"]), P(mask_out), sc_out, P(w.O), Td, Bd, H, x.device)
+        exp_route = self._exp_route(b16, late_mask, Td * Bd, V, H)
+        self.last_nll_route = ("exp" if exp_route else "logits") if (b16 is not None and self.fused_nll) else None
         if b16 is not None:
+            OT = None if exp_route else P(b16.OT)
             if late_mask and mask_out is not None:
-                lib.lv_cvt_bf16_keep_f32(P(w.hs, Bd * H), H, Td, Bd, H, P(mask_out), sc_out, P(b16.O), H, P(b16.OT), b16.ldr, s)
+                lib.lv_cvt_bf16_keep_f32(P(w.hs, Bd * H), H, Td, Bd, H, P(mask_out), sc_out, P(b16.O), H, OT, b16.ldr, s)
             elif late_mask:
-                lib.lv_cvt_bf16_f32(P(w.hs, Bd * H), H, Td * Bd, H, P(b16.O), H, P(b16.OT), b16.ldr, s)
+                lib.lv_cvt_bf16_f32(P(w.hs, Bd * H), H, Td * Bd, H, P(b16.O), H, OT, b16.ldr, s)
             else:
-                lib.lv_cvt_bf16_f32(P(w.O), H, Td * Bd, H, P(b16.O), H, P(b16.OT), b16.ldr, s)
+                lib.lv_cvt_bf16_f32(P(w.O), H, Td * Bd, H, P(b16.O), H, OT, b16.ldr, s)
             wi = self.refresh_weight_images(Bd, x.device)
-            if self.fused_nll:
+            if exp_route:
+                with _prof("gemm_bf16", 2.0 * Td * Bd * V * H):
+                    lib.lv_gemm_b16_nll_exp_tile(self.nll_tile, Td * Bd, V, H, P(b16.O), H, P(wi.pred), H, P(b16.dl), b16.ldv, P(b16.part), s)
+                lib.lv_softmax_nll_merge_exp_f32(P(b16.part), b16.nparts, P(b16.O), H, P(wi.pred), H, H, P(ids), T, 1, Bd, P(b16.dl), b16.ldv,
+                                                 V, P(w.lse), P(w.nll), P(b16.kappa), P(b16.rz), P(b16.corr), P(self.status), Td * Bd, s)
+            elif self.fused_nll:
                 with _prof("gemm_bf16", 2.0 * Td * Bd * V * H):
                     lib.lv_gemm_b16_nll(Td * Bd, V, H, P(b16.O), H, P(wi.pred), H, P(b16.l16), b16.ldv, P(ids), T, 1, Bd,
                                         P(b16.part), P(b16.tgt), s)
@@ -1188,6 +1225,7 @@
         self.gen += 1
         self.last = (x, z2, mask_in, mask_out, sc_in, sc_out, B, T, self.gen)
         self.last_ns = ns
+        self._last_exp = (exp_route, late_mask)
         return w.rec
 
     def cond_ll_supported(self, T):
@@ -1237,7 +1275,13 @@
         gwih = gv["lstm.weight_ih_l0"]
         dev = x.device
         b16 = self._b16(Bd, Td, ns)
-        if b16 is not None and self.fused_nll:
+        exp_route, fwd_late = self._last_exp
+        if exp_route:
+            if fwd_late:
+                lib.lv_cvt_bf16_keep_rs_f32(P(w.hs, Bd * H), H, Td, Bd, H, P(mask_out), sc_out, P(b16.kappa), P(drec), P(b16.OT), b16.ldr, s)
+            else:
+                lib.lv_cvt_bf16_keep_rs_f32(P(w.O), H, Td, Bd, H, None, 1.0, P(b16.kappa), P(drec), P(b16.OT), b16.ldr, s)
+        elif b16 is not None and self.fused_nll:
             lib.lv_softmax_nll_bwd_h16(P(b16.l16), b16.ldv, P(w.lse), P(ids), T, 1, P(drec), P(b16.dl), b16.ldv, Td, Bd, V, s)
         elif b16 is not None:
             lib.lv_softmax_nll_bwd_b16(P(w.logits), w.ldl, P(w.lse), P(ids), T, 1, P(drec), P(b16.dl), b16.ldv, Td, Bd, V, s)
@@ -1261,7 +1305,13 @@
                        self.precision, ws=sws)
         img = self._lstm_images(Bd, Td, ns)
         late_mask = _persistent_ok(self, img, Bd, H, dev, _PERSIST_BWD_MAX_B)
-        if b16 is not None and late_mask and mask_out is not None:
+        if exp_route:
+            gws = _gemm_ws(lib, s)
+            with _prof("gemm_bf16", 2.0 * Td * Bd * H * V):
+                lib.lv_gemm_b16_keep_rs(Td * Bd, H, V, P(b16.dl), b16.ldv, P(self._wimg.predT), b16.ldv, P(w.dO),
+                                        P(mask_out) if late_mask else None, sc_out, Bd, P(b16.rz), P(drec), P(b16.corr),
+                                        P(v["pred_linear.weight"]), H, P(ids), T, 1, P(gws), gws.numel(), s)
+        elif b16 is not None and late_mask and mask_out is not None:
             gws = _gemm_ws(lib, s)
             with _prof("gemm_bf16", 2.0 * Td * Bd * H * V):
                 lib.lv_gemm_b16_keep(Td * Bd, H, V, P(b16.dl), b16.ldv, P(self._wimg.predT), b16.ldv, P(w.dO), P(mask_out), sc_out, Bd,
diff --git a/vae_lagging_encoder_amd/trainer.py b/vae_lagging_encoder_amd/trainer.py
--- a/vae_lagging_encoder_amd/trainer.py
+++ b/vae_lagging_encoder_amd/trainer.py
@@ -161,21 +161,22 @@
         while v[8] != 0.0:
             done = int(round(v[9] - self._committed_base))
             redo = self._journal[done:]
-            if all(_eng.persist_rung(e) == 2 for e in (self.enc, self.dec)):
-                raise _eng._lib.LvaeError("a step was voided although both engines run the launch-per-timestep kernels (status words "
-                                          "%s / %s)" % (self.enc.status.tolist(), self.dec.status.tolist()))
-            for e in (self.enc, self.dec):
-                if _eng.persist_rung(e) < 2:
-                    _eng.demote_persistent(e)
-                else:
-                    _eng.reset_persistent_status(e)
+            if int(self.dec.status.item()) == _eng.NLL_EXP_STATUS:
+                self.dec.nll_route = "logits"
+                _eng.reset_persistent_status(self.dec)
+                moved = int(self.enc.status.item()) != 0
+                if moved:
+                    self._demote(self.enc)
+            else:
+                moved = True
+                self._demote_both()
             self.recoveries += 1
             for st in self.static.values():
                 st.graphs = {}
             self.scal[8:13] = 0
             self._committed_base = 0.0
             self._journal = []
-            if self.on_demote is not None:
+            if moved and self.on_demote is not None:
                 self.on_demote(max(_eng.persist_rung(self.enc), _eng.persist_rung(self.dec)))
             for x, klw, noise, update in redo:
                 self._queue_step(x, klw, noise, update)
@@ -187,6 +188,20 @@
             self.scal[9] = 0
             self._committed_base = 0.0
         return v
+
+    @staticmethod
+    def _demote(e):
+        if _eng.persist_rung(e) < 2:
+            _eng.demote_persistent(e)
+        else:
+            _eng.reset_persistent_status(e)
+
+    def _demote_both(self):
+        if all(_eng.persist_rung(e) == 2 for e in (self.enc, self.dec)):
+            raise _eng._lib.LvaeError("a step was voided although both engines run the launch-per-timestep kernels (status words "
+                                      "%s / %s)" % (self.enc.status.tolist(), self.dec.status.tolist()))
+        for e in (self.enc, self.dec):
+            self._demote(e)
 
     def reset_stats(self):
         self.scal[5:8] = 0
@@ -530,6 +545,7 @@
                 st.m_in.copy_(m_in)
             if m_out is not None:
                 st.m_out.copy_(m_out)
+        self.dec.nll_gated = self.grad_sync is None
         try:
             if not self.use_graph:
                 self._run(st, update, draw)
@@ -550,6 +566,7 @@
             for part in g:
                 part()
         finally:
+            self.dec.nll_gated = False
             if update in ("encoder", "both"):
                 self.enc.wgen += 1
             if update in ("decoder", "both"):
```

Result: faster. 11560 (median of 6 runs) (+2.0%).
